# lvxianwei/DeepMerge

Hardware: AMD Instinct MI355X
Metric: superpixel-pairs/sec (train step) (higher is better)
Workload: dtype bf16; 1 GPU; ShfitScaleFormer_v3 depth [3, 2, 1], scales [32, 64, 128, 256] x 4ch (256x256x4 patches), 32 pairs/GPU/step, fwd+loss+bwd+allreduce+Adam (BASELINE configs[1]); pairs_per_gpu=32, global_batch=32, parallelism=dp1

## Files before the change

deepmerge_amd/_lib.py:

```python
from __future__ import annotations

import ctypes as C
import os
import re
import threading

HERE = os.path.dirname(os.path.abspath(__file__))
ROOT = os.path.dirname(HERE)
LIB_PATH = os.path.join(HERE, "libdeepmerge_hip.so")
HEADER_PATH = os.path.join(ROOT, "include", "deepmerge_hip.h")

DM_F32, DM_BF16 = 0, 1
DM_NT, DM_NN, DM_TN = 0, 1, 2
DM_BF16_PAIR = 2
DM_F64 = 3
DM_EPI_NONE, DM_EPI_GELU, DM_EPI_DGELU, DM_EPI_GELU_GRAD, DM_EPI_MUL = 0, 1, 2, 3, 4

_STATUS = {-1: "bad shape", -2: "bad dtype", -3: "bad alignment", -4: "workspace", -5: "HIP error", -6: "unsupported"}


class DeepMergeLibraryError(RuntimeError):
    pass


class DmGemmArgs(C.Structure):
    _fields_ = [
        ("layout", C.c_int32), ("ab_dtype", C.c_int32), ("c_dtype", C.c_int32), ("aux_dtype", C.c_int32),
        ("M", C.c_int32), ("N", C.c_int32), ("K", C.c_int32),
        ("epilogue", C.c_int32), ("accumulate", C.c_int32), ("split_k", C.c_int32),
        ("A", C.c_void_p), ("lda", C.c_int64),
        ("B", C.c_void_p), ("ldb", C.c_int64),
        ("C", C.c_void_p), ("ldc", C.c_int64),
        ("bias", C.c_void_p),
        ("residual", C.c_void_p), ("ldr", C.c_int64),
        ("aux", C.c_void_p), ("ldaux", C.c_int64),
        ("rows_per_group", C.c_int32), ("group_stride", C.c_int64),
        ("workspace", C.c_void_p), ("workspace_bytes", C.c_int64),
        ("colsum_a", C.c_void_p), ("colsum_accumulate", C.c_int32),
        ("k_fold", C.c_int32), ("a_fold", C.c_int64 * 3), ("b_fold", C.c_int64 * 3),
        ("c_plane", C.c_int64),
    ]


class DmReduceItem(C.Structure):
    _fields_ = [("partial", C.c_void_p), ("out0", C.c_void_p), ("out1", C.c_void_p),
                ("nrows", C.c_int32), ("width", C.c_int32), ("split", C.c_int32), ("accumulate", C.c_int32)]


class DmPairDraw(C.Structure):
    _fields_ = [("pairs", C.c_void_p), ("pair_flag", C.c_void_p), ("poly_off", C.c_void_p), ("poly_pts", C.c_void_p),
                ("pt_tile", C.c_void_p), ("pt_xy", C.c_void_p), ("pt_inner", C.c_void_p), ("pt_obj", C.c_void_p),
                ("pt_region", C.c_void_p),
                ("tile_id", C.c_void_p), ("xy", C.c_void_p), ("inner", C.c_void_p), ("obj", C.c_void_p),
                ("region", C.c_void_p), ("flag", C.c_void_p),
                ("point_id", C.c_void_p),
                ("seed", C.c_uint64),
                ("n_pairs", C.c_int32), ("n_poly", C.c_int32), ("n_poly_pts", C.c_int32), ("n_pts", C.c_int32),
                ("epoch", C.c_int32), ("batch", C.c_int32)]


class DmMergeFold(C.Structure):
    _fields_ = [("ptr", C.c_void_p), ("idx", C.c_void_p), ("edges", C.c_void_p), ("root", C.c_void_p), ("pick", C.c_void_p),
                ("rep", C.c_void_p), ("region_of", C.c_void_p),
                ("simi", C.c_void_p), ("weights", C.c_void_p),
                ("count", C.c_void_p), ("sum", C.c_void_p), ("sumsq", C.c_void_p), ("bbox", C.c_void_p), ("peri", C.c_void_p),
                ("new_id", C.c_void_p), ("hist_rank", C.c_void_p), ("new_ptr", C.c_void_p), ("new_idx", C.c_void_p),
                ("new_rep", C.c_void_p), ("new_region_of", C.c_void_p), ("n_regions", C.c_void_p),
                ("new_count", C.c_void_p), ("new_sum", C.c_void_p), ("new_sumsq", C.c_void_p), ("new_bbox", C.c_void_p),
                ("new_peri", C.c_void_p),
                ("history", C.c_void_p), ("history_simi", C.c_void_p),
                ("C", C.c_int32), ("P", C.c_int32), ("E", C.c_int32), ("S0", C.c_int32), ("bands", C.c_int32), ("round", C.c_int32),
                ("hist_base", C.c_int32), ("hist_cap", C.c_int32)]


class DmVectorTrace(C.Structure):
    _fields_ = [("dart", C.c_void_p), ("next", C.c_void_p), ("lab", C.c_void_p), ("other", C.c_void_p), ("flags", C.c_void_p),
                ("key", C.c_void_p), ("sum", C.c_void_p), ("ring_of_slot", C.c_void_p), ("ring_ptr", C.c_void_p),
                ("arc_base", C.c_void_p), ("xy", C.c_void_p), ("area2", C.c_void_p),
                ("arc_first", C.c_void_p), ("arc_left", C.c_void_p), ("arc_right", C.c_void_p), ("arc_vstart", C.c_void_p),
                ("arc_count", C.c_void_p), ("arc_pos", C.c_void_p), ("arc_ptr", C.c_void_p), ("arc_xy", C.c_void_p),
                ("W", C.c_int32), ("D", C.c_int32), ("R", C.c_int32), ("n_arcs", C.c_int32)]


class DmSceneVectorTrace(C.Structure):
    _fields_ = [("dart", C.c_void_p), ("next", C.c_void_p), ("lab", C.c_void_p), ("other", C.c_void_p), ("flags", C.c_void_p),
                ("key", C.c_void_p), ("sum", C.c_void_p), ("ring_of_slot", C.c_void_p), ("ring_ptr", C.c_void_p),
                ("arc_base", C.c_void_p), ("xy", C.c_void_p), ("area2", C.c_void_p),
                ("arc_first", C.c_void_p), ("arc_left", C.c_void_p), ("arc_right", C.c_void_p), ("arc_vstart", C.c_void_p),
                ("arc_count", C.c_void_p), ("arc_pos", C.c_void_p), ("arc_ptr", C.c_void_p), ("arc_xy", C.c_void_p),
                ("W", C.c_int64), ("D", C.c_int32), ("R", C.c_int32), ("n_arcs", C.c_int32)]


class DmSceneSimplifyRings(C.Structure):
    _fields_ = [("xy", C.c_void_p), ("ring_ptr", C.c_void_p), ("vert_ring", C.c_void_p), ("node_row", C.c_void_p), ("node_col", C.c_void_p),
                ("kept_row", C.c_void_p), ("status", C.c_void_p),
                ("n_nodes", C.c_int64), ("n_kept", C.c_int64), ("scene_h", C.c_int64), ("scene_w", C.c_int64),
                ("V", C.c_int32), ("R", C.c_int32)]


class DmSimplifyTopology(C.Structure):
    _fields_ = [("arc_xy", C.c_void_p), ("arc_ptr", C.c_void_p), ("new_ptr", C.c_void_p), ("keep", C.c_void_p),
                ("point_count", C.c_void_p), ("point_fill", C.c_void_p), ("point_ptr", C.c_void_p), ("point_xy", C.c_void_p),
                ("seg", C.c_void_p), ("kind", C.c_void_p), ("cell_count", C.c_void_p), ("cell_fill", C.c_void_p),
                ("cell_ptr", C.c_void_p), ("cell_seg", C.c_void_p), ("stack", C.c_void_p), ("status", C.c_void_p),
                ("Va", C.c_int64), ("cap", C.c_int64), ("A", C.c_int32), ("H", C.c_int32), ("W", C.c_int32), ("q", C.c_int32)]


class DmSceneSimplifyTopology(C.Structure):
    _fields_ = [("arc_xy", C.c_void_p), ("arc_ptr", C.c_void_p), ("new_ptr", C.c_void_p), ("arc_keep", C.c_void_p),
                ("point_count", C.c_void_p), ("point_fill", C.c_void_p), ("point_ptr", C.c_void_p), ("point_xy", C.c_void_p),
                ("seg", C.c_void_p), ("kind", C.c_void_p), ("cell_count", C.c_void_p), ("cell_fill", C.c_void_p),
                ("cell_ptr", C.c_void_p), ("cell_seg", C.c_void_p), ("stack", C.c_void_p), ("status", C.c_void_p),
                ("Va", C.c_int64), ("cap", C.c_int64), ("A", C.c_int32), ("H", C.c_int32), ("W", C.c_int32), ("q", C.c_int32),
                ("cell_log2", C.c_int32)]


class DmProfRow(C.Structure):
    _fields_ = [("name", C.c_char * 64), ("launches", C.c_int64), ("total_ms", C.c_double),
                ("total_flops", C.c_double), ("total_bytes", C.c_double)]


_P, _I, _L, _F, _D = C.c_void_p, C.c_int32, C.c_int64, C.c_float, C.c_double

SIGNATURES = {
    "dm_abi_version": (_I, []),
    "dm_last_error": (C.c_char_p, []),
    "dm_arch": (C.c_char_p, []),
    "dm_gemm": (_I, [C.POINTER(DmGemmArgs), _P]),
    "dm_gemm_workspace_bytes": (_L, [_I, _I, _I, _I]),
    "dm_gemm_grouped": (_I, [C.POINTER(DmGemmArgs), _I, _P]),
    "dm_attention_fwd": (_I, [_P, _P, _P, _P, _I, _I, _I, _I, _F, _I, _P]),
    "dm_attention_relpos_inkernel": (_I, [_I, _I, _I, _I, _I, _I, _I, _I]),
    "dm_attention_fwd_relpos": (_I, [_P, _P, _I, _I, _I, _P, _P, _I, _I, _I, _I, _F, _I, _P]),
    "dm_attention_split_ok": (_I, [_I, _I, _I, _I, _I, _I, _I, _I]),
    "dm_attention_split_fwd": (_I, [_P, _P, _P, _P, _I, _I, _I, _P, _P, _I, _I, _I, _I, _F, _P]),
    "dm_attention_split_fwd_pair": (_I, [_P, _P, _P, _P, _I, _I, _I, _P, _P, _P, _I, _I, _I, _I, _F, _P]),
    "dm_attention_split_bwd_chunks": (_I, [_I, _I, _I]),
    "dm_attention_split_bwd": (_I, [_P, _P, _P, _I, _I, _I, _P, _P, _P, _P, _P, _P, _P, _P, _I, _I, _I, _I, _F, _P]),
    "dm_attention_split_bwd_pair": (_I, [_P, _P, _P, _I, _I, _I, _P, _P, _P, _P, _P, _P, _P, _P, _I, _I, _I, _I, _F, _P]),
    "dm_attention_bwd_relpos": (_I, [_P, _P, _I, _I, _I, _P, _P, _P, _P, _P, _P, _P, _P, _I, _I, _I, _I, _F, _I, _P]),
    "dm_attention_bwd": (_I, [_P, _P, _P, _P, _P, _P, _P, _P, _P, _I, _I, _I, _I, _F, _I, _P]),
    "dm_attention_bwd_batch_chunks": (_I, [_I, _I, _I, _I]),
    "dm_relpos_bias_gather": (_I, [_P, _P, _P, _P, _I, _I, _I, _P]),
    "dm_relpos_bias_reduce": (_I, [_P, _P, _P, _P, _I, _I, _I, _I, _I, _P]),
    "dm_layernorm_fwd": (_I, [_P, _P, _P, _P, _I, _P, _P, _I, _I, _F, _P]),
    "dm_layernorm_bwd": (_I, [_P, _I, _P, _P, _P, _P, _P, _P, _P, _P, _P, _I, _P, _I, _I, _P]),
    "dm_layernorm_bwd_partials": (_I, [_P, _I, _P, _P, _P, _P, _P, _P, _P, _P, _I, _I, C.POINTER(C.c_int32), _P]),
    "dm_layernorm_bwd_partials_pair": (_I, [_P, _I, _P, _P, _P, _P, _P, _P, _P, _P, _I, _I, C.POINTER(C.c_int32), _P]),
    "dm_layernorm_bwd_partials_regroup": (_I, [_P, _I, _P, _P, _P, _P, _P, _P, _P, _P, _I, _I, _I, _I, C.POINTER(C.c_int32), _P]),
    "dm_pool_layernorm_ok": (_I, [_I]),
    "dm_pool_layernorm_fwd": (_I, [_P, _P, _P, _P, _P, _P, _P, _I, _I, _I, _I, _F, _P]),
    "dm_pool_layernorm_bwd": (_I, [_P, _P, _P, _P, _P, _P, _P, _P, _P, _I, _P, C.POINTER(C.c_int32), _I, _I, _I, _I, _P]),
    "dm_partial_reduce_batch": (_I, [C.POINTER(DmReduceItem), _I, _P]),
    "dm_layernorm_bwd_partial_floats": (_L, [_I]),
    "dm_token_pool_fwd": (_I, [_P, _P, _I, _I, _I, _I, _P]),
    "dm_token_pool_bwd": (_I, [_P, _P, _I, _I, _I, _I, _P]),
    "dm_group_mean_fwd": (_I, [_P, _P, _I, _I, _I, _P]),
    "dm_group_mean_bwd": (_I, [_P, _P, _I, _I, _I, _P]),
    "dm_colsum": (_I, [_P, _I, _L, _P, _I, _I, _I, _P, _P]),
    "dm_colsum_partial_floats": (_L, [_I]),
    "dm_cast": (_I, [_P, _P, _I, _L, _P]),
    "dm_split_bf16": (_I, [_P, _L, _L, _L, _P, _I, _I, _P]),
    "dm_split_colsum_partial_floats": (_L, [_L, _L]),
    "dm_split_bf16_colsum": (_I, [_P, _L, _L, _L, _P, _I, _I, _P, _P, _P]),
    "dm_split_bf16_planes": (_I, [_P, _L, _L, _L, _P, _P, _P, _P]),
    "dm_patchify": (_I, [_P, _P, _I, _I, _I, _I, _I, _P]),
    "dm_contrastive_loss": (_I, [_P, _P, _P, _F, _F, _P, _P, _P, _I, _I, _P]),
    "dm_cross_entropy": (_I, [_P, _P, _P, _F, _P, _P, _I, _I, _P]),
    "dm_batchnorm_workspace_bytes": (_L, [_I, _I]),
    "dm_batchnorm_fwd": (_I, [_P, _P, _P, _P, _P, _P, _I, _P, _P, _P, _I, _I, _F, _F, _I, _I, _P, _P]),
    "dm_batchnorm_bwd": (_I, [_P, _P, _P, _P, _P, _I, _P, _P, _P, _P, _P, _I, _I, _I, _I, _I, _P, _P]),
    "dm_adam_step": (_I, [_P, _P, _P, _P, _P, _L, _I, _D, _D, _D, _D, _D, _P]),
    "dm_adam_hyper": (_I, [_I, _D, _D, _D, _P]),
    "dm_adam_step_dev": (_I, [_P, _P, _P, _P, _P, _L, _P, _D, _D, _D, _D, _P]),
    "dm_adam_step_dev_pair": (_I, [_P, _P, _P, _P, _P, _P, _L, _P, _D, _D, _D, _D, _P]),
    "dm_segment_mean": (_I, [_P, _P, _P, _P, _I, _I, _P]),
    "dm_edge_similarity": (_I, [_P, _P, _P, _P, _I, _I, _F, _P]),
    "dm_pairwise_distance": (_I, [_P, _P, _P, _I, _I, _I, _I, _P]),
    "dm_patch_pyramid": (_I, [_P, _I, _I, _I, _P, _P, _I, _I, _I, _I, _P, _P]),
    "dm_patch_pyramid_cols": (_I, [_P, _I, _I, _I, _P, _P, _I, _I, _I, _I, _I, _P, _I, _P]),
    "dm_pair_batch_gather": (_I, [_P, _I, _I, _I, _I, _P, _P, _P, _P, _I, _I, _I, _I, _I, _I, _P, _I, _P, _P, _P, _P]),
    "dm_pair_batch_gather_oriented": (_I, [_P, _I, _I, _I, _I, _P, _P, _P, _P, _P, _I, _I, _I, _I, _I, _I, _P, _I, _P, _P, _P, _P]),
    "dm_pair_batch_gather_augmented": (_I, [_P, _I, _I, _I, _I, _P, _P, _P, _P, _P, _P, _I, _I, _I, _I, _I, _I, _P, _I, _P, _P, _P, _P]),
    "dm_pair_epoch_draw": (_I, [C.POINTER(DmPairDraw), _P]),
    "dm_pair_epoch_orient": (_I, [C.c_uint64, _I, _I, _I, _I, _P, _P]),
    "dm_pair_epoch_radiometric": (_I, [C.c_uint64, _I, _I, _I, _I, _I, _I, _I, _P, _P]),
    "dm_contrastive_terms": (_I, [_P, _P, _P, _F, _P, _P, _I, _I, _P]),
    "dm_pair_eval_workspace_bytes": (_L, [_L, _I]),
    "dm_pair_eval_summary": (_I, [_P, _P, _P, _L, _P, _I, _P, _P, _P, _P, _P]),
    "dm_label_stats": (_I, [_P, _P, _I, _I, _I, _I, _P, _P, _P, _P, _P, _P]),
    "dm_label_features": (_I, [_P, _P, _P, _P, _P, _I, _I, _P, _P]),
    "dm_rag_edges": (_I, [_P, _I, _I, _I, _P, _P, _I, _P, _P, _I, _P, _P, _P]),
    "dm_seam_stitch": (_I, [_P, _P, _L, _L, _P, _P, _P, _I, _P, _P, _I, _P, _P, _P]),
    "dm_merge_round": (_I, [_P, _P, _I, _I, _P, _P, _I, _P]),
    "dm_merge_best": (_I, [_P, _P, _I, _I, _F, _P, _P]),
    "dm_merge_best_small": (_I, [_P, _P, _I, _I, _P, _L, _P, _P]),
    "dm_merge_accept": (_I, [_P, _P, _I, _I, _P, _L, _P, _P]),
    "dm_merge_match": (_I, [_P, _P, _I, _I, _P, _P, _P, _P, _P]),
    "dm_merge_fold_regions": (_I, [C.POINTER(DmMergeFold), _P]),
    "dm_merge_edge_keys": (_I, [_P, _P, _P, _I, _I, _P, _P]),
    "dm_merge_fold_edges": (_I, [_P, _P, _P, _I, _P, _P, _P, _P]),
    "dm_relabel_raster": (_I, [_P, _P, _P, _L, _I, _P]),
    "dm_region_merge_cost": (_I, [_P, _P, _P, _P, _P, _P, _P, _I, _I, _I, _D, _D, _D, _D, _D, _P, _P]),
    "dm_pixel_regions": (_I, [_P, _I, _I, _I, _P, _P, _P, _P, _P, _P, _P, _P]),
    "dm_label_clearance": (_I, [_P, _I, _I, _I, _P, _P, _P, _P]),
    "dm_point_select_round": (_I, [_P, _P, _I, _I, _I, _I, _I, _P, _P, _P, _P, _P, _P]),
    "dm_point_emit": (_I, [_P, _P, _P, _P, _I, _I, _I, _I, _P, _P, _P, _P, _P, _P, _P]),
    "dm_scene_point_init": (_I, [_P, _P, _P, _I, _P]),
    "dm_scene_point_select": (_I, [_P, _P, _I, _I, _I, _I, _I, _I, _L, _L, _L, _L, _I, _I, _I, _P, _P, _P, _P, _P]),
    "dm_scene_point_commit": (_I, [_P, _L, _L, _I, _I, _P, _P, _P, _P]),
    "dm_label_overlap": (_I, [_P, _P, _I, _I, _L, _L, _P, _P, _I, _P, _P, _I, _P, _P, _P]),
    "dm_overlap_reduce": (_I, [_P, _P, _I, _L, _L, _P, _P, _P, _P, _P, _P, _P, _P, _P]),
    "dm_pair_flags": (_I, [_P, _I, _P, _P, _P, _I, _I, _P, _P]),
    "dm_boundary_bits": (_I, [_P, _I, _I, _I, _P, _P, _P, _P]),
    "dm_boundary_counts": (_I, [_P, _P, _P, _I, _I, _I, _I, _I, _I, _I, _P, _P]),
    "dm_slic_iterate": (_I, [_P, _I, _I, _I, _I, _I, _I, _P, _P, _P, _P]),
    "dm_connected_labels": (_I, [_P, _I, _I, _I, _I, _P, _P, _P, _P, _P]),
    "dm_label_area": (_I, [_P, _I, _I, _I, _P, _P]),
    "dm_slic_absorb_pick": (_I, [_P, _P, _I, _P, _I, _I, _P, _P, _P, _P]),
    "dm_scene_slic_init": (_I, [_P, _I, _I, _I, _I, _I, _I, _I, _I, _P, _P, _P]),
    "dm_scene_slic_pass": (_I, [_P, _I, _I, _I, _I, _I, _I, _I, _I, _I, _P, _P, _P, _P]),
    "dm_scene_slic_update": (_I, [_I, _P, _P, _P]),
    "dm_vector_count": (_I, [_P, _I, _I, _P, _P, _P, _P]),
    "dm_vector_emit": (_I, [_P, _P, _I, _I, _P, _P, _P]),
    "dm_vector_link": (_I, [_P, _P, _P, _P, _I, _I, _I, _P, _P, _P, _P, _P, _P]),
    "dm_vector_head_round": (_I, [_P, _P, _P, _P, _I, _P, _P]),
    "dm_vector_rank_init": (_I, [_P, _P, _P, _P, _I, _P, _P, _P, _P, _P, _I, _P]),
    "dm_vector_rank_round": (_I, [_P, _P, _P, _P, _I, _P, _P]),
    "dm_vector_ring_emit": (_I, [C.POINTER(DmVectorTrace), _P]),
    "dm_vector_arc_emit": (_I, [C.POINTER(DmVectorTrace), _P]),
    "dm_scene_vector_count": (_I, [_P, _I, _I, _I, _I, _I, _I, _P, _P, _P, _P, _P]),
    "dm_scene_vector_link": (_I, [_P, _P, _P, _I, _I, _I, _L, _L, _L, _L, _P, _P, _P, _P, _P, _P]),
    "dm_scene_vector_ring_emit": (_I, [C.POINTER(DmSceneVectorTrace), _P]),
    "dm_scene_vector_arc_emit": (_I, [C.POINTER(DmSceneVectorTrace), _P]),
    "dm_rasterize_count": (_I, [_P, _P, _P, _I, _I, _I, _I, _P, _P]),
    "dm_rasterize_emit": (_I, [_P, _P, _P, _P, _P, _I, _I, _L, _I, _I, _L, _P, _P]),
    "dm_rasterize_fill": (_I, [_P, _L, _I, _I, _I, _P, _P, _P]),
    "dm_rasterize_count_rows": (_I, [_P, _P, _P, _I, _I, _I, _I, _I, _I, _P, _P]),
    "dm_rasterize_emit_rows": (_I, [_P, _P, _P, _P, _P, _I, _I, _L, _I, _I, _I, _I, _L, _P, _P]),
    "dm_rasterize_fill_window": (_I, [_P, _L, _I, _I, _I, _I, _I, _I, _I, _P, _P, _P]),
    "dm_simplify_nodes": (_I, [_P, _I, _I, _P, _P]),
    "dm_simplify_chains": (_I, [_P, _P, _I, _L, _I, _I, _I, _P, _P, _P]),
    "dm_simplify_arc_count": (_I, [_P, _P, _I, _L, _I, _I, _P, _P, _P]),
    "dm_simplify_arc_emit": (_I, [_P, _P, _P, _I, _L, _L, _I, _I, _P, _P, _P]),
    "dm_simplify_ring_count": (_I, [_P, _P, _P, _I, _I, _I, _I, _P, _P, _P]),
    "dm_simplify_ring_emit": (_I, [_P, _P, _P, _P, _P, _I, _I, _L, _I, _I, _P, _P, _P, _P]),
    "dm_simplify_topology_point_count": (_I, [C.POINTER(DmSimplifyTopology), _P]),
    "dm_simplify_topology_point_fill": (_I, [C.POINTER(DmSimplifyTopology), _P]),
    "dm_simplify_topology_segments": (_I, [C.POINTER(DmSimplifyTopology), _P]),
    "dm_simplify_topology_bin_count": (_I, [C.POINTER(DmSimplifyTopology), _P]),
    "dm_simplify_topology_bin_fill": (_I, [C.POINTER(DmSimplifyTopology), _P]),
    "dm_simplify_topology_pairs": (_I, [C.POINTER(DmSimplifyTopology), _P]),
    "dm_simplify_topology_jumps": (_I, [C.POINTER(DmSimplifyTopology), _P]),
    "dm_simplify_topology_refine": (_I, [C.POINTER(DmSimplifyTopology), _I, _P]),
    "dm_scene_simplify_node_count": (_I, [_P, _I, _I, _I, _I, _I, _I, _L, _L, _L, _L, _P, _P, _P]),
    "dm_scene_simplify_node_emit": (_I, [_P, _I, _I, _I, _I, _I, _I, _L, _L, _L, _L, _P, _I, _P, _P]),
    "dm_scene_simplify_chains": (_I, [_P, _P, _I, _L, _L, _L, _I, _P, _P, _P]),
    "dm_scene_simplify_arc_count": (_I, [_P, _P, _I, _L, _L, _L, _P, _P, _P]),
    "dm_scene_simplify_arc_emit": (_I, [_P, _P, _P, _I, _L, _L, _L, _L, _P, _P, _P]),
    "dm_scene_simplify_ring_count": (_I, [C.POINTER(DmSceneSimplifyRings), _P, _P]),
    "dm_scene_simplify_ring_emit": (_I, [C.POINTER(DmSceneSimplifyRings), _P, _P, _L, _P, _P, _P]),
    "dm_scene_simplify_topology_point_count": (_I, [C.POINTER(DmSceneSimplifyTopology), _P]),
    "dm_scene_simplify_topology_point_fill": (_I, [C.POINTER(DmSceneSimplifyTopology), _P]),
    "dm_scene_simplify_topology_segments": (_I, [C.POINTER(DmSceneSimplifyTopology), _P]),
    "dm_scene_simplify_topology_bin_count": (_I, [C.POINTER(DmSceneSimplifyTopology), _P]),
    "dm_scene_simplify_topology_bin_fill": (_I, [C.POINTER(DmSceneSimplifyTopology), _P]),
    "dm_scene_simplify_topology_pairs": (_I, [C.POINTER(DmSceneSimplifyTopology), _P]),
    "dm_scene_simplify_topology_jumps": (_I, [C.POINTER(DmSceneSimplifyTopology), _P]),
    "dm_scene_simplify_topology_refine": (_I, [C.POINTER(DmSceneSimplifyTopology), _I, _P]),
    "dm_gru_cell_fwd": (_I, [_P, _L, _P, _P, _P, _P, _I, _I, _P]),
    "dm_gru_cell_bwd": (_I, [_P, _P, _P, _P, _P, _P, _I, _I, _P]),
    "dm_prof_enable": (_I, [_I]),
    "dm_prof_collect": (_I, [C.POINTER(DmProfRow), _I]),
}

_lock = threading.Lock()
_lib = None


def declared_symbols(header_path: str = HEADER_PATH):
    text = open(header_path).read()
    text = re.sub(r"/\*.*?\*/", "", text, flags=re.S)
    return sorted(set(re.findall(r"\b(dm_[a-z0-9_]+)\s*\(", text)))


def lib() -> C.CDLL:
    global _lib
    if _lib is not None:
        return _lib
    with _lock:
        if _lib is not None:
            return _lib
        if not os.path.exists(LIB_PATH):
            raise DeepMergeLibraryError(
                f"{LIB_PATH} not found: build the HIP kernels first "
                f"(`python -c 'import __graft_entry__ as g; g.build()'` or `make -C deepmerge_amd/csrc`). "
                f"deepmerge_amd has no CPU fallback.")
        try:
            handle = C.CDLL(LIB_PATH)
        except OSError as e:
            raise DeepMergeLibraryError(f"cannot load {LIB_PATH}: {e}") from e
        for name, (res, args) in SIGNATURES.items():
            try:
                fn = getattr(handle, name)
            except AttributeError as e:
                raise DeepMergeLibraryError(f"{LIB_PATH} does not export {name}") from e
            fn.restype = res
            fn.argtypes = args
        if handle.dm_abi_version() != 7:
            raise DeepMergeLibraryError(f"ABI version mismatch: library {handle.dm_abi_version()} != 7")
        _lib = handle
        return _lib


def check(rc: int, what: str):
    if rc == 0:
        return
    msg = lib().dm_last_error().decode("utf-8", "replace")
    text = f"{what} failed ({_STATUS.get(rc, rc)}): {msg}"
    if rc in (-1, -2, -3, -6):
        raise ValueError(text)
    raise RuntimeError(text)
```

deepmerge_amd/csrc/dm_attention.hip:

```cpp
#include "dm_common.h"
#include "dm_mfma.h"
#include "dm_attention_pipe.h"
#include "dm_attention_x3.h"
#include "dm_prof.h"

namespace {

constexpr int HD = 64;
constexpr int QB = 64;

template <typename T> struct AL {
  static constexpr int RB = HD * (int)sizeof(T);
  static constexpr int CPRW = RB / 16;
  static constexpr int KBD = RB / 64;
  static constexpr int EPC = 16 / (int)sizeof(T);
  static constexpr int TPB = (sizeof(T) == 2) ? 2 : 1;
};

template <typename T> __device__ __forceinline__ int swz(int row);
template <> __device__ __forceinline__ int swz<bf16_t>(int row) {
  const int t0 = (row >> 1) & 1, t1 = (row >> 2) & 1, t2 = (row >> 3) & 1;
  return ((t1 ^ t2) << 2) | (t0 << 1) | t1;
}
template <> __device__ __forceinline__ int swz<float>(int row) { return row & 15; }

template <typename T> __device__ __forceinline__ int img_off(int row, int chunk) {
  return row * AL<T>::RB + ((chunk ^ swz<T>(row)) << 4);
}

template <typename T>
__device__ __forceinline__ void tile_to_lds(char *lds, const T *g, long long ld, int nvalid, int nrows, int t) {
  using L = AL<T>;
  const int c = t % L::CPRW;
  constexpr int RPI = 256 / L::CPRW;
  for (int row = t / L::CPRW; row < nrows; row += RPI) {
    u32x4 v = {0u, 0u, 0u, 0u};
    if (row < nvalid) v = *reinterpret_cast<const u32x4 *>(g + (long long)row * ld + c * L::EPC);
    *reinterpret_cast<u32x4 *>(lds + img_off<T>(row, c)) = v;
  }
}

template <typename T> __device__ __forceinline__ u32x4 frag_row(const char *lds, int row, int kb, int lane) {
  return *reinterpret_cast<const u32x4 *>(lds + img_off<T>(row, kb * 4 + (lane >> 4)));
}
template <typename T> __device__ __forceinline__ u32x4 frag_tr(const char *lds, int d0, int m, int lane);
template <> __device__ __forceinline__ u32x4 frag_tr<bf16_t>(const char *lds, int d0, int m, int lane) {
  const int g = lane >> 4, q = (lane >> 2) & 3, p = lane & 3;
  const int d = d0 + 4 * p;
  u32x4 out;
#pragma unroll
  for (int half = 0; half < 2; ++half) {
    const int k = 32 * m + 4 * g + 16 * half + q;
    const u32x2 w = dm_ds_read_tr16(lds + img_off<bf16_t>(k, d >> 3) + ((d & 7) << 1));
    out[2 * half] = w[0];
    out[2 * half + 1] = w[1];
  }
  return out;
}
template <> __device__ __forceinline__ u32x4 frag_tr<float>(const char *lds, int d0, int m, int lane) {
  const int g = lane >> 4, d = d0 + (lane & 15);
  u32x4 out;
#pragma unroll
  for (int j = 0; j < 4; ++j) {
    const int k = 16 * m + 4 * g + j;
    out[j] = *reinterpret_cast<const unsigned int *>(lds + img_off<float>(k, d >> 2) + ((d & 3) << 2));
  }
  return out;
}
template <typename T> __device__ __forceinline__ u32x4 gl_frag(const T *rowp, bool valid, int kb, int lane) {
  u32x4 v = {0u, 0u, 0u, 0u};
  if (valid) v = *reinterpret_cast<const u32x4 *>(rowp + (kb * 4 + (lane >> 4)) * AL<T>::EPC);
  return v;
}

template <typename T, int NKT> __device__ __forceinline__ u32x4 acc_frag(const f32x4 (&s)[NKT], int m) {
  if constexpr (sizeof(T) == 2) {
    const f32x4 lo = s[2 * m], hi = s[2 * m + 1];
    bf16x8 r = {(bf16_t)lo[0], (bf16_t)lo[1], (bf16_t)lo[2], (bf16_t)lo[3], (bf16_t)hi[0], (bf16_t)hi[1], (bf16_t)hi[2], (bf16_t)hi[3]};
    return __builtin_bit_cast(u32x4, r);
  } else {
    return __builtin_bit_cast(u32x4, s[m]);
  }
}

template <typename T, int NKT>
__device__ __forceinline__ void contract_tokens(f32x4 (&o)[4], const f32x4 (&s)[NKT], const char *img, int lane) {
#pragma unroll
  for (int m = 0; m < NKT / AL<T>::TPB; ++m) {
    const u32x4 fp = acc_frag<T, NKT>(s, m);
#pragma unroll
    for (int dt = 0; dt < 4; ++dt) mma<T>(o[dt], fp, frag_tr<T>(img, dt * 16, m, lane));
    if ((m & 1) == 1) __builtin_amdgcn_sched_barrier(0);
  }
}

__device__ __forceinline__ float row_max(float v) {
  v = fmaxf(v, __shfl_xor(v, 16, 64));
  return fmaxf(v, __shfl_xor(v, 32, 64));
}
__device__ __forceinline__ float row_sum(float v) {
  v += __shfl_xor(v, 16, 64);
  return v + __shfl_xor(v, 32, 64);
}

template <typename T> __device__ __forceinline__ float fast_exp(float x);
template <> __device__ __forceinline__ float fast_exp<float>(float x) { return expf(x); }
template <> __device__ __forceinline__ float fast_exp<bf16_t>(float x) { return __expf(x); }

__device__ __forceinline__ f32x4 load4_guard(const float *p, int i, int n, bool vec) {
  if (vec) return (i < n) ? dm_load4(p + i) : (f32x4){0.f, 0.f, 0.f, 0.f};
  f32x4 r;
#pragma unroll
  for (int e = 0; e < 4; ++e) r[e] = (i + e < n) ? p[i + e] : 0.f;
  return r;
}

struct AttnParams {
  const void *qkv;
  const float *bias;
  const float *bias_t;
  const void *out;
  const void *dout;
  float *lse;
  float *delta;
  void *dqkv;
  float *slab;
  int B, N, H, bchunk;
  float scale;
};

template <bool FAST, bool STRIDED>
__device__ __forceinline__ f32x4 bias_tile(const float *bias_rows, int N, int row, int lane, int kt) {
  const int col = kt * 16 + 4 * (lane >> 4);
  f32x4 bv = {0.f, 0.f, 0.f, 0.f};
  if (bias_rows && row < N) {
    if constexpr (!STRIDED) {
      bv = load4_guard(bias_rows + (long long)row * N, col, N, FAST);
    } else {
#pragma unroll
      for (int r = 0; r < 4; ++r) bv[r] = (col + r < N) ? bias_rows[(long long)(col + r) * N + row] : 0.f;
    }
  }
  return bv;
}
template <typename T>
__device__ __forceinline__ f32x4 score_tile(const u32x4 (&fa)[AL<T>::KBD], const char *img, const f32x4 bv,
                                            int N, int row, float scale, int lane, int kt) {
  using L = AL<T>;
  const int g = lane >> 4, li = lane & 15;
  f32x4 a = {0.f, 0.f, 0.f, 0.f};
#pragma unroll
  for (int kb = 0; kb < L::KBD; ++kb) mma<T>(a, fa[kb], frag_row<T>(img, kt * 16 + li, kb, lane));
  const int col = kt * 16 + 4 * g;
#pragma unroll
  for (int r = 0; r < 4; ++r) a[r] = (row < N && col + r < N) ? a[r] * scale + bv[r] : -INFINITY;
  return a;
}

template <typename T> __device__ __forceinline__ u32x4 pack_tiles(const f32x4 (&tl)[AL<T>::TPB]) {
  if constexpr (sizeof(T) == 2) {
    bf16x8 r = {(bf16_t)tl[0][0], (bf16_t)tl[0][1], (bf16_t)tl[0][2], (bf16_t)tl[0][3],
                (bf16_t)tl[1][0], (bf16_t)tl[1][1], (bf16_t)tl[1][2], (bf16_t)tl[1][3]};
    return __builtin_bit_cast(u32x4, r);
  } else {
    return __builtin_bit_cast(u32x4, tl[0]);
  }
}

template <typename T, int NB>
__device__ __forceinline__ void contract_frags(f32x4 (&o)[4], const u32x4 (&f)[NB], const char *img, int lane) {
#pragma unroll
  for (int m = 0; m < NB; ++m) {
#pragma unroll
    for (int dt = 0; dt < 4; ++dt) mma<T>(o[dt], f[m], frag_tr<T>(img, dt * 16, m, lane));
    if ((m & 1) == 1) __builtin_amdgcn_sched_barrier(0);
  }
}

template <typename T, int NKT, bool FAST>
__global__ __launch_bounds__(256, 2) void attn_fwd_kernel(const AttnParams p) {
  using L = AL<T>;
  constexpr int NK = NKT * 16;
  constexpr int IMG = NK * L::RB;
  __shared__ __attribute__((aligned(16))) char smem[2 * IMG];
  char *kimg = smem, *vimg = smem + IMG;
  const int t = threadIdx.x, lane = t & 63, wave = t >> 6, g = lane >> 4, li = lane & 15;
  const int qblk = blockIdx.x, h = blockIdx.y, b = blockIdx.z;
  const int N = p.N, H = p.H;

  const long long tok_stride = 3LL * H * HD;
  const T *base = reinterpret_cast<const T *>(p.qkv) + (long long)b * N * tok_stride + (long long)h * HD;
  const int q = qblk * QB + wave * 16 + li;

  tile_to_lds<T>(kimg, base + (long long)H * HD, tok_stride, N, NK, t);
  tile_to_lds<T>(vimg, base + 2LL * H * HD, tok_stride, N, NK, t);
  u32x4 fq[L::KBD];
#pragma unroll
  for (int kb = 0; kb < L::KBD; ++kb) fq[kb] = gl_frag<T>(base + (long long)q * tok_stride, q < N, kb, lane);
  __syncthreads();

  f32x4 s[NKT];
  const float *brows = p.bias ? p.bias + (long long)h * N * N : nullptr;
#pragma unroll
  for (int kt = 0; kt < NKT; ++kt) s[kt] = score_tile<T>(fq, kimg, bias_tile<FAST, false>(brows, N, q, lane, kt), N, q, p.scale, lane, kt);

  float m = -INFINITY;
#pragma unroll
  for (int kt = 0; kt < NKT; ++kt)
#pragma unroll
    for (int r = 0; r < 4; ++r) m = fmaxf(m, s[kt][r]);
  m = row_max(m);
  const float msafe = (m == -INFINITY) ? 0.f : m;
  float l = 0.f;
#pragma unroll
  for (int kt = 0; kt < NKT; ++kt)
#pragma unroll
    for (int r = 0; r < 4; ++r) {
      const float e = fast_exp<T>(s[kt][r] - msafe);
      s[kt][r] = e;
      l += e;
    }
  l = row_sum(l);
  const float inv = (l > 0.f) ? 1.f / l : 0.f;
  if (g == 0 && q < N) p.lse[((long long)b * H + h) * N + q] = msafe + logf(l);
#pragma unroll
  for (int kt = 0; kt < NKT; ++kt) s[kt] *= inv;

  f32x4 o[4];
#pragma unroll
  for (int dt = 0; dt < 4; ++dt) o[dt] = (f32x4){0.f, 0.f, 0.f, 0.f};
  contract_tokens<T, NKT>(o, s, vimg, lane);
  if (q < N) {
    T *orow = reinterpret_cast<T *>(const_cast<void *>(p.out)) + ((long long)b * N + q) * H * HD + (long long)h * HD;
#pragma unroll
    for (int dt = 0; dt < 4; ++dt) dm_store4(orow + dt * 16 + 4 * g, o[dt]);
  }
}

template <typename T, int NKT, bool FAST>
__global__ __launch_bounds__(256, 2) void attn_bwd_dq_kernel(const AttnParams p) {
  using L = AL<T>;
  constexpr int NK = NKT * 16;
  constexpr int IMG = NK * L::RB;
  constexpr int NB = NKT / L::TPB;
  __shared__ __attribute__((aligned(16))) char smem[2 * IMG];
  char *kimg = smem, *vimg = smem + IMG;
  const int t = threadIdx.x, lane = t & 63, wave = t >> 6, g = lane >> 4, li = lane & 15;
  const int qblk = blockIdx.x, h = blockIdx.y, chunk = blockIdx.z;
  const int N = p.N, H = p.H;
  const long long tok_stride = 3LL * H * HD;
  const int q = qblk * QB + wave * 16 + li;
  const bool qok = q < N;
  const float *brows = p.bias ? p.bias + (long long)h * N * N : nullptr;
  const bool want_bins = p.slab != nullptr;
  f32x4 hacc[NKT];
#pragma unroll
  for (int kt = 0; kt < NKT; ++kt) hacc[kt] = (f32x4){0.f, 0.f, 0.f, 0.f};

  const int b_end = min(p.B, (chunk + 1) * p.bchunk);
  for (int b = chunk * p.bchunk; b < b_end; ++b) {
    const T *base = reinterpret_cast<const T *>(p.qkv) + (long long)b * N * tok_stride + (long long)h * HD;
    const long long orow = ((long long)b * N + q) * H * HD + (long long)h * HD;
    const T *Og = reinterpret_cast<const T *>(p.out) + orow;
    const T *dOg = reinterpret_cast<const T *>(p.dout) + orow;
    __syncthreads();
    tile_to_lds<T>(kimg, base + (long long)H * HD, tok_stride, N, NK, t);
    tile_to_lds<T>(vimg, base + 2LL * H * HD, tok_stride, N, NK, t);
    u32x4 fq[L::KBD], fdo[L::KBD];
#pragma unroll
    for (int kb = 0; kb < L::KBD; ++kb) {
      fq[kb] = gl_frag<T>(base + (long long)q * tok_stride, qok, kb, lane);
      fdo[kb] = gl_frag<T>(dOg, qok, kb, lane);
    }
    float dl = 0.f;
    if (qok) {
#pragma unroll
      for (int c = 0; c < 4; ++c) {
        const f32x4 a = dm_load4(Og + 16 * g + 4 * c), d = dm_load4(dOg + 16 * g + 4 * c);
        dl += (a[0] * d[0] + a[1] * d[1]) + (a[2] * d[2] + a[3] * d[3]);
      }
    }
    dl = row_sum(dl);
    const long long rowid = ((long long)b * H + h) * N + q;
    if (g == 0 && qok) p.delta[rowid] = dl;
    const float lse = qok ? p.lse[rowid] : 0.f;
    __syncthreads();

    u32x4 fds[NB];
    f32x4 bnext[L::TPB];
#pragma unroll
    for (int u = 0; u < L::TPB; ++u) bnext[u] = bias_tile<FAST, false>(brows, N, q, lane, u);
#pragma unroll
    for (int m = 0; m < NB; ++m) {
      f32x4 bcur[L::TPB];
#pragma unroll
      for (int u = 0; u < L::TPB; ++u) bcur[u] = bnext[u];
      if (m + 1 < NB) {
#pragma unroll
        for (int u = 0; u < L::TPB; ++u) bnext[u] = bias_tile<FAST, false>(brows, N, q, lane, (m + 1) * L::TPB + u);
      }
      f32x4 tl[L::TPB];
#pragma unroll
      for (int u = 0; u < L::TPB; ++u) {
        const int kt = m * L::TPB + u;
        const f32x4 sc = score_tile<T>(fq, kimg, bcur[u], N, q, p.scale, lane, kt);
        f32x4 a = {0.f, 0.f, 0.f, 0.f};
#pragma unroll
        for (int kb = 0; kb < L::KBD; ++kb) mma<T>(a, fdo[kb], frag_row<T>(vimg, kt * 16 + li, kb, lane));
        f32x4 dsv;
#pragma unroll
        for (int r = 0; r < 4; ++r) dsv[r] = fast_exp<T>(sc[r] - lse) * (a[r] - dl);
        if (want_bins) hacc[kt] += dsv;
        tl[u] = dsv;
      }
      fds[m] = pack_tiles<T>(tl);
      asm volatile("" : "+v"(fds[m]));
      __builtin_amdgcn_sched_barrier(0);
    }

    f32x4 o[4];
#pragma unroll
    for (int dt = 0; dt < 4; ++dt) o[dt] = (f32x4){0.f, 0.f, 0.f, 0.f};
    contract_frags<T, NB>(o, fds, kimg, lane);
    if (qok) {
      T *dq = reinterpret_cast<T *>(p.dqkv) + ((long long)b * N + q) * tok_stride + (long long)h * HD;
#pragma unroll
      for (int dt = 0; dt < 4; ++dt) dm_store4(dq + dt * 16 + 4 * g, o[dt] * p.scale);
    }
  }

  if (want_bins && qok) {
    float *srow = p.slab + (((long long)chunk * H + h) * N + q) * N;
#pragma unroll
    for (int kt = 0; kt < NKT; ++kt) {
      const int key = kt * 16 + 4 * g;
      if constexpr (FAST) {
        if (key < N) dm_store4(srow + key, hacc[kt]);
      } else {
#pragma unroll
        for (int r = 0; r < 4; ++r)
          if (key + r < N) srow[key + r] = hacc[kt][r];
      }
    }
  }
}

template <typename T, int NKT, bool FAST>
__global__ __launch_bounds__(256, 2) void attn_bwd_dkv_kernel(const AttnParams p) {
  using L = AL<T>;
  constexpr int NK = NKT * 16;
  constexpr int IMG = NK * L::RB;
  __shared__ __attribute__((aligned(16))) char smem[2 * IMG];
  char *qimg = smem, *doimg = smem + IMG;
  const int t = threadIdx.x, lane = t & 63, wave = t >> 6, g = lane >> 4, li = lane & 15;
  const int kblk = blockIdx.x, h = blockIdx.y, b = blockIdx.z;
  const int N = p.N, H = p.H;

  const long long tok_stride = 3LL * H * HD;
  const T *base = reinterpret_cast<const T *>(p.qkv) + (long long)b * N * tok_stride + (long long)h * HD;
  const long long o_stride = (long long)H * HD;
  const T *dOg = reinterpret_cast<const T *>(p.dout) + (long long)b * N * o_stride + (long long)h * HD;
  const int key = kblk * QB + wave * 16 + li;
  const bool kok = key < N;
  const T *krow = base + (long long)key * tok_stride + (long long)H * HD;
  const T *vrow = krow + (long long)H * HD;
  const float *lse = p.lse + ((long long)b * H + h) * N;
  const float *delta = p.delta + ((long long)b * H + h) * N;

  tile_to_lds<T>(qimg, base, tok_stride, N, NK, t);
  tile_to_lds<T>(doimg, dOg, o_stride, N, NK, t);
  u32x4 fk[L::KBD], fvv[L::KBD];
#pragma unroll
  for (int kb = 0; kb < L::KBD; ++kb) {
    fk[kb] = gl_frag<T>(krow, kok, kb, lane);
    fvv[kb] = gl_frag<T>(vrow, kok, kb, lane);
  }
  __syncthreads();

  constexpr int NB = NKT / L::TPB;
  u32x4 fpt[NB], fds[NB];
  const float *bsrc = FAST ? p.bias_t : p.bias;
  const float *brows = bsrc ? bsrc + (long long)h * N * N : nullptr;
  f32x4 bnext[L::TPB], lnext[L::TPB], dnext[L::TPB];
  auto fetch = [&](int m) {
#pragma unroll
    for (int u = 0; u < L::TPB; ++u) {
      const int qt = m * L::TPB + u;
      bnext[u] = bias_tile<FAST, !FAST>(brows, N, key, lane, qt);
      lnext[u] = load4_guard(lse, qt * 16 + 4 * g, N, FAST);
      dnext[u] = load4_guard(delta, qt * 16 + 4 * g, N, FAST);
    }
  };
  fetch(0);
#pragma unroll
  for (int m = 0; m < NB; ++m) {
    f32x4 bcur[L::TPB], lcur[L::TPB], dcur[L::TPB];
#pragma unroll
    for (int u = 0; u < L::TPB; ++u) { bcur[u] = bnext[u]; lcur[u] = lnext[u]; dcur[u] = dnext[u]; }
    if (m + 1 < NB) fetch(m + 1);
    f32x4 tp[L::TPB], td[L::TPB];
#pragma unroll
    for (int u = 0; u < L::TPB; ++u) {
      const int qt = m * L::TPB + u;
      const int q0 = qt * 16 + 4 * g;
      const f32x4 sc = score_tile<T>(fk, qimg, bcur[u], N, key, p.scale, lane, qt);
      f32x4 a = {0.f, 0.f, 0.f, 0.f};
#pragma unroll
      for (int kb = 0; kb < L::KBD; ++kb) mma<T>(a, fvv[kb], frag_row<T>(doimg, qt * 16 + li, kb, lane));
#pragma unroll
      for (int r = 0; r < 4; ++r) {
        const float pv = (q0 + r < N) ? fast_exp<T>(sc[r] - lcur[u][r]) : 0.f;
        tp[u][r] = pv;
        td[u][r] = pv * (a[r] - dcur[u][r]);
      }
    }
    fpt[m] = pack_tiles<T>(tp);
    fds[m] = pack_tiles<T>(td);
    asm volatile("" : "+v"(fpt[m]), "+v"(fds[m]));
    __builtin_amdgcn_sched_barrier(0);
  }
  f32x4 o[4];
  T *dk = reinterpret_cast<T *>(p.dqkv) + ((long long)b * N + key) * tok_stride + (long long)H * HD + (long long)h * HD;
  T *dvp = dk + (long long)H * HD;
#pragma unroll
  for (int dt = 0; dt < 4; ++dt) o[dt] = (f32x4){0.f, 0.f, 0.f, 0.f};
  contract_frags<T, NB>(o, fpt, doimg, lane);
  if (kok) {
#pragma unroll
    for (int dt = 0; dt < 4; ++dt) dm_store4(dvp + dt * 16 + 4 * g, o[dt]);
  }
#pragma unroll
  for (int dt = 0; dt < 4; ++dt) o[dt] = (f32x4){0.f, 0.f, 0.f, 0.f};
  contract_frags<T, NB>(o, fds, qimg, lane);
  if (kok) {
#pragma unroll
    for (int dt = 0; dt < 4; ++dt) dm_store4(dk + dt * 16 + 4 * g, o[dt] * p.scale);
  }
}

template <typename T, int NKT, bool FAST> void launch3(int which, const AttnParams &p, dim3 grid, hipStream_t s) {
  if (which == 0) hipLaunchKernelGGL((attn_fwd_kernel<T, NKT, FAST>), grid, dim3(256), 0, s, p);
  else if (which == 1) hipLaunchKernelGGL((attn_bwd_dq_kernel<T, NKT, FAST>), grid, dim3(256), 0, s, p);
  else hipLaunchKernelGGL((attn_bwd_dkv_kernel<T, NKT, FAST>), grid, dim3(256), 0, s, p);
}
template <typename T, bool FAST> void dispatch_nkt(int which, const AttnParams &p, hipStream_t s) {
  const dim3 grid((p.N + QB - 1) / QB, p.H, which == 1 ? (p.B + p.bchunk - 1) / p.bchunk : p.B);
  const int nkt = (p.N + 15) / 16;
  if (nkt <= 2) launch3<T, 2, FAST>(which, p, grid, s);
  else if (nkt <= 4) launch3<T, 4, FAST>(which, p, grid, s);
  else if (nkt <= 8) launch3<T, 8, FAST>(which, p, grid, s);
  else if (nkt <= 12) launch3<T, 12, FAST>(which, p, grid, s);
  else if (nkt <= 14) launch3<T, 14, FAST>(which, p, grid, s);
  else launch3<T, 16, FAST>(which, p, grid, s);
}
template <typename T> int dispatch(int which, const AttnParams &p, hipStream_t s) {
  const bool fast = (p.N % 4 == 0) && (which != 2 || p.bias == nullptr || p.bias_t != nullptr);
  if (fast) dispatch_nkt<T, true>(which, p, s);
  else dispatch_nkt<T, false>(which, p, s);
  return 0;
}

int check_common(const char *who, int B, int N, int H, int D, int dtype) {
  DM_REQUIRE(B > 0 && H > 0 && N > 0 && N <= 256, DM_ERR_BAD_SHAPE, "%s: need 0 < N <= 4096 tokens and head dim <= 256 (got N=%d, D=%d, B=%d, H=%d)", who, N, D, B, H);
  DM_REQUIRE(D == HD, DM_ERR_BAD_SHAPE, "%s: head dim must be in 1..256 (got %d)", who, D);
  DM_REQUIRE(dtype == DM_F32 || dtype == DM_BF16, DM_ERR_BAD_DTYPE, "%s: bad dtype %d", who, dtype);
  DM_REQUIRE(H <= 65535 && B <= 65535, DM_ERR_BAD_SHAPE, "%s: grid too large", who);
  return DM_OK;
}

}

static int batch_chunk(int B, int N, int H) {
  const int per_sample = ((N + QB - 1) / QB) * H;
  for (int c = 8; c > 1; c >>= 1)
    if ((long long)per_sample * ((B + c - 1) / c) >= 300) return c;
  return 1;
}

const AttnSwitches &attn_switches() {
// ... 340 lines not shown
```

deepmerge_amd/ops.py:

```python
from __future__ import annotations

import os

import ctypes as C
from dataclasses import dataclass
from typing import Optional, Tuple

import torch

from . import _lib
from ._lib import DM_BF16, DM_EPI_DGELU, DM_EPI_GELU, DM_EPI_GELU_GRAD, DM_EPI_MUL, DM_EPI_NONE, DM_F32, DM_NN, DM_NT, DM_TN, DmGemmArgs, check

_NUMERICS = "bf16"


NUMERICS_MODES = ("bf16", "fp32", "bf16x3")
_FP32_PRODUCTS = "mfma_f32"
_SPLIT_MIN_WORK = 1 << 24
_PAIR_LN_MAX_COLS = 1024


def set_numerics(mode: str) -> None:
    global _NUMERICS
    _NUMERICS = check_numerics(mode)
# ... 158 lines not shown

def _fold_planes(layout: int, A: Planes, B: Planes, M: int, N: int, K: int):
    (a_rows, a_cols), (b_rows, b_cols) = _operand_shapes(layout, M, N, K)
    if (A.rows, A.cols) != (a_rows, a_cols) or (B.rows, B.cols) != (b_rows, b_cols):
        raise ValueError(f"plane pair shapes {(A.rows, A.cols)} / {(B.rows, B.cols)} do not match the product {(a_rows, a_cols)} / {(b_rows, b_cols)}")
    return A.t, B.t, a_cols, b_cols, 3 * K, (K, A.t.stride(0), B.t.stride(0))


def gemm(layout: int, A: torch.Tensor, B: torch.Tensor, C_out: torch.Tensor, M: int, N: int, K: int, *,
         lda: Optional[int] = None, ldb: Optional[int] = None, ldc: Optional[int] = None,
         bias: Optional[torch.Tensor] = None, residual: Optional[torch.Tensor] = None, ldr: Optional[int] = None,
         epilogue: int = DM_EPI_NONE, aux: Optional[torch.Tensor] = None, ldaux: Optional[int] = None,
         accumulate: bool = False, split_k: int = 0, rows_per_group: int = 0, group_stride: int = 0,
         colsum_out: Optional[torch.Tensor] = None, colsum_accumulate: bool = False, ws_slot: str = "gemm") -> torch.Tensor:
    c_pair = C_out if isinstance(C_out, Planes) else None
    if c_pair is not None:
        if (c_pair.rows, c_pair.cols) != (M, N) or ldc not in (None, N):
            raise ValueError("a plane-pair result is a dense [2, M, N] tensor")
        C_out = c_pair.t
    fold = None
    if isinstance(A, Planes) or isinstance(B, Planes) or (
            _FP32_PRODUCTS == "bf16x3" and A.dtype == torch.float32 and M * N * K >= _SPLIT_MIN_WORK and planes_ok(M, K) and planes_ok(N, K)
            and (lda is None or lda % 4 == 0) and (ldb is None or ldb % 4 == 0) and A.data_ptr() % 16 == 0 and B.data_ptr() % 16 == 0):
        (a_rows, a_cols), (b_rows, b_cols) = _operand_shapes(layout, M, N, K)
        if not isinstance(A, Planes):
            A = split_planes(torch.as_strided(A, (a_rows, a_cols), (lda if lda is not None else a_cols, 1)), colsum_out, colsum_accumulate)
            colsum_out = None
        if not isinstance(B, Planes):
            B = split_planes(torch.as_strided(B, (b_rows, b_cols), (ldb if ldb is not None else b_cols, 1)))
        A, B, lda, ldb, K, fold = _fold_planes(layout, A, B, M, N, K)
    _need_cuda(A, B, C_out, bias, residual, aux, colsum_out)
    if A.dtype != B.dtype:
        raise ValueError(f"A/B dtype mismatch: {A.dtype} vs {B.dtype}")
    if lda is None:
        lda = A.stride(-2) if A.dim() >= 2 else K
    if ldb is None:
        ldb = B.stride(-2) if B.dim() >= 2 else K
    if (_FP32_PRODUCTS == "bf16x3" and A.dtype == torch.float32 and M * N * K >= _SPLIT_MIN_WORK
            and M % 8 == 0 and N % 8 == 0 and K % 8 == 0 and lda % 4 == 0 and ldb % 4 == 0):
        (a_rows, a_cols), (b_rows, b_cols) = _operand_shapes(layout, M, N, K)
        a_stack, b_stack = int(layout == DM_TN), int(layout != DM_NT)
        A3 = workspace(6 * a_rows * a_cols, A.device, ws_slot + ".split_a").view(torch.bfloat16)
        B3 = workspace(6 * b_rows * b_cols, A.device, ws_slot + ".split_b").view(torch.bfloat16)
        fused_ok = colsum_out is not None and a_cols % 8 == 0 and A.data_ptr() % 16 == 0 and (a_rows * a_cols) % 8 == 0
        n_part = _lib.lib().dm_split_colsum_partial_floats(a_rows, a_cols) if fused_ok else 0
        if n_part > 0:
            part = workspace(4 * n_part, A.device, ws_slot + ".partial").view(torch.float32)
            rows_out = C.c_int32(0)
            check(_lib.lib().dm_split_bf16_colsum(A.data_ptr(), lda, a_rows, a_cols, A3.data_ptr(), a_stack, 0b100, part.data_ptr(),
                                                  C.byref(rows_out), _stream()), "dm_split_bf16_colsum")
            _reduce(part, colsum_out, colsum_out, rows_out.value, a_cols, a_cols, colsum_accumulate)
        else:
            check(_lib.lib().dm_split_bf16(A.data_ptr(), lda, a_rows, a_cols, A3.data_ptr(), a_stack, 0b100, _stream()), "dm_split_bf16")
            if colsum_out is not None:
                colsum(torch.as_strided(A, (a_rows, a_cols), (lda, 1)), colsum_out, accumulate=colsum_accumulate, ws_slot=ws_slot + ".partial")
        check(_lib.lib().dm_split_bf16(B.data_ptr(), ldb, b_rows, b_cols, B3.data_ptr(), b_stack, 0b010, _stream()), "dm_split_bf16")
        return gemm(layout, A3, B3, C_out, M, N, 3 * K, lda=(a_cols if a_stack else 3 * a_cols), ldb=(b_cols if b_stack else 3 * b_cols),
                    ldc=ldc, bias=bias, residual=residual, ldr=ldr, epilogue=epilogue, aux=aux, ldaux=ldaux, accumulate=accumulate,
                    split_k=split_k, rows_per_group=rows_per_group, group_stride=group_stride, ws_slot=ws_slot)
    a = _gemm_args(layout, A, B, C_out, M, N, K, lda, ldb, ldc, bias, residual, ldr, epilogue, aux, ldaux, accumulate, split_k,
                   rows_per_group, group_stride, colsum_out, colsum_accumulate, ws_slot, c_pair, fold)
    check(_lib.lib().dm_gemm(C.byref(a), _stream()), "dm_gemm")
    return c_pair if c_pair is not None else C_out


def _gemm_args(layout, A, B, C_out, M, N, K, lda, ldb, ldc, bias, residual, ldr, epilogue, aux, ldaux, accumulate, split_k,
               rows_per_group, group_stride, colsum_out, colsum_accumulate, ws_slot, c_pair=None, fold=None, min_slabs: int = 0) -> DmGemmArgs:
    a = DmGemmArgs()
    a.layout, a.ab_dtype, a.c_dtype = layout, _dt(A), _dt(C_out)
    if c_pair is not None:
        if _dt(A) != DM_BF16:
            raise ValueError("a plane-pair result goes with bf16 / folded operands")
        a.c_dtype, a.c_plane = _lib.DM_BF16_PAIR, M * N
    a.aux_dtype = _dt(aux) if aux is not None else DM_F32
    a.M, a.N, a.K = M, N, K
    a.epilogue, a.accumulate, a.split_k = epilogue, int(accumulate), split_k
    a.A, a.lda = A.data_ptr(), lda
    a.B, a.ldb = B.data_ptr(), ldb
    a.C, a.ldc = C_out.data_ptr(), (ldc if ldc is not None else N)
    a.bias = _ptr(bias)
    if bias is not None and (bias.dtype != torch.float32 or bias.numel() < N):
        raise ValueError("bias must be fp32 with >= N elements")
    a.residual, a.ldr = _ptr(residual), (ldr if ldr is not None else N)
    if residual is not None and residual.dtype != torch.float32:
        raise ValueError("residual must be fp32")
    a.aux, a.ldaux = _ptr(aux), (ldaux if ldaux is not None else N)
    a.rows_per_group, a.group_stride = rows_per_group, group_stride
    if colsum_out is not None:
        if colsum_out.dtype != torch.float32 or colsum_out.numel() < M or not colsum_out.is_contiguous():
            raise ValueError("colsum_out must be a contiguous fp32 tensor with >= M elements")
        a.colsum_a, a.colsum_accumulate = colsum_out.data_ptr(), int(colsum_accumulate)
    if fold is not None:
        a.k_fold = fold[0]
        a.a_fold[0], a.a_fold[1], a.a_fold[2] = 0, 0, fold[1]
        a.b_fold[0], a.b_fold[1], a.b_fold[2] = 0, fold[2], 0
    ws_bytes = _lib.lib().dm_gemm_workspace_bytes(layout, M, N, K) if (split_k != 1 or colsum_out is not None) else 0
    if split_k > 1:
        ws_bytes = max(ws_bytes, _lib.lib().dm_gemm_workspace_bytes(layout, M, N, K) + split_k * M * N * 4)
    if min_slabs > 0:
        ws_bytes = max(ws_bytes, _lib.lib().dm_gemm_workspace_bytes(layout, M, N, K) + min_slabs * M * N * 4)
    if ws_bytes > 0:
        ws = workspace(ws_bytes, A.device, ws_slot)
        a.workspace, a.workspace_bytes = ws.data_ptr(), ws.numel()
    return a


def gemm_grouped(calls) -> None:
    if not calls:
        return
    plain = len(calls) > 1
    for args, kw in calls:
        A, B = args[1], args[2]
        pair = isinstance(A, Planes) and isinstance(B, Planes)
        plain = plain and not isinstance(args[3], Planes) and (pair or (not isinstance(A, Planes) and not isinstance(B, Planes) and A.dtype == torch.bfloat16))
    if not plain:
        for args, kw in calls:
            gemm(*args, **kw)
        return
    arr = (DmGemmArgs * len(calls))()
    for i, (args, kw) in enumerate(calls):
        layout, A, B, C_out, M, N, K = args
        lda, ldb, fold = kw.get("lda"), kw.get("ldb"), None
        if isinstance(A, Planes):
            A, B, lda, ldb, K, fold = _fold_planes(layout, A, B, M, N, K)
        _need_cuda(A, B, C_out, kw.get("colsum_out"))
        if A.dtype != B.dtype:
            raise ValueError(f"A/B dtype mismatch: {A.dtype} vs {B.dtype}")
        lda = lda if lda is not None else (A.stride(-2) if A.dim() >= 2 else K)
        ldb = ldb if ldb is not None else (B.stride(-2) if B.dim() >= 2 else K)
        arr[i] = _gemm_args(layout, A, B, C_out, M, N, K, lda, ldb, kw.get("ldc"), kw.get("bias"), kw.get("residual"), kw.get("ldr"),
                            kw.get("epilogue", DM_EPI_NONE), kw.get("aux"), kw.get("ldaux"), kw.get("accumulate", False), kw.get("split_k", 0),
                            kw.get("rows_per_group", 0), kw.get("group_stride", 0), kw.get("colsum_out"), kw.get("colsum_accumulate", False),
                            f"{kw.get('ws_slot', 'gemm')}.g{i}", None, fold, min_slabs=16 if layout == DM_TN else 0)
    check(_lib.lib().dm_gemm_grouped(arr, len(calls), _stream()), "dm_gemm_grouped")


def cast(src: torch.Tensor, dtype: torch.dtype) -> torch.Tensor:
    if src.dtype == dtype:
        return src
    _need_cuda(src)
    if src.dtype != torch.float32:
        raise ValueError("dm_cast source must be fp32")
    src = src.contiguous()
    dst = torch.empty(src.shape, dtype=dtype, device=src.device)
    check(_lib.lib().dm_cast(src.data_ptr(), dst.data_ptr(), _dt(dst), src.numel(), _stream()), "dm_cast")
    return dst


def colsum(X: torch.Tensor, out: torch.Tensor, accumulate: bool = False, ws_slot: str = "partial") -> torch.Tensor:
    _need_cuda(X, out)
    M, N = X.shape
    part = workspace(_lib.lib().dm_colsum_partial_floats(N) * 4, X.device, ws_slot)
    check(_lib.lib().dm_colsum(X.data_ptr(), _dt(X), X.stride(0), out.data_ptr(), M, N, int(accumulate), part.data_ptr(), _stream()), "dm_colsum")
    return out


def layernorm_fwd(x: torch.Tensor, gamma, beta, eps: float, out_dtype: torch.dtype, pair: bool = False):
    _need_cuda(x, gamma, beta)
    rows, cols = x.numel() // x.shape[-1], x.shape[-1]
    mean = torch.empty(rows, dtype=torch.float32, device=x.device)
    rstd = torch.empty(rows, dtype=torch.float32, device=x.device)
    if pair:
        yp = torch.empty((2, rows, cols), dtype=torch.bfloat16, device=x.device)
        check(_lib.lib().dm_layernorm_fwd(x.data_ptr(), gamma.data_ptr(), beta.data_ptr(), yp.data_ptr(), _lib.DM_BF16_PAIR, mean.data_ptr(),
                                          rstd.data_ptr(), rows, cols, eps, _stream()), "dm_layernorm_fwd")
        return Planes(yp), mean, rstd
    y = torch.empty(x.shape, dtype=out_dtype, device=x.device)
    check(_lib.lib().dm_layernorm_fwd(x.data_ptr(), gamma.data_ptr(), beta.data_ptr(), y.data_ptr(), _dt(y), mean.data_ptr(),
                                      rstd.data_ptr(), rows, cols, eps, _stream()), "dm_layernorm_fwd")
    return y, mean, rstd


_pending_reduce = []
_pending_out = set()
_flush_queued = False
_flush_task = -1


def _in_backward() -> bool:
    return torch._C._current_graph_task_id() != -1


def flush_reductions() -> None:
    global _flush_queued
    _flush_queued = False
    if not _pending_reduce:
        return
    items = (_lib.DmReduceItem * len(_pending_reduce))()
    for i, (f, _keep) in enumerate(_pending_reduce):
        items[i].partial, items[i].out0, items[i].out1, items[i].nrows, items[i].width, items[i].split, items[i].accumulate = f
    n = len(_pending_reduce)
    keep = list(_pending_reduce)
    _pending_reduce.clear()
    _pending_out.clear()
    check(_lib.lib().dm_partial_reduce_batch(items, n, _stream()), "dm_partial_reduce_batch")
    del keep


def _queue_reduce(part, out0, out1, nrows, width, split, accumulate) -> None:
    global _flush_queued, _flush_task
    task = torch._C._current_graph_task_id()
    if task != _flush_task:
        _pending_reduce.clear()
        _pending_out.clear()
        _flush_queued = False
        _flush_task = task
    keys = (out0.data_ptr(), out1.data_ptr())
    if keys[0] in _pending_out or keys[1] in _pending_out:
        flush_reductions()
    _pending_reduce.append(((part.data_ptr(), keys[0], keys[1], int(nrows), int(width), int(split), int(bool(accumulate))), (part, out0, out1)))
    _pending_out.update(keys)
    if not _flush_queued:
        torch.autograd.Variable._execution_engine.queue_callback(flush_reductions)
        _flush_queued = True


def _deferred(defer: bool) -> bool:
    return bool(defer and _DEFER_REDUCTIONS and _in_backward())


def _reduce(part, out0, out1, nrows, width, split, accumulate, deferred=False) -> None:
    if deferred:
        _queue_reduce(part, out0, out1, nrows, width, split, accumulate)
        return
    item = (_lib.DmReduceItem * 1)()
    item[0].partial, item[0].out0, item[0].out1 = part.data_ptr(), out0.data_ptr(), out1.data_ptr()
    item[0].nrows, item[0].width, item[0].split, item[0].accumulate = nrows, width, split, int(bool(accumulate))
    check(_lib.lib().dm_partial_reduce_batch(item, 1, _stream()), "dm_partial_reduce_batch")


def _partial_rows(cols: int, device, deferred: bool) -> torch.Tensor:
    n = _lib.lib().dm_layernorm_bwd_partial_floats(cols)
    return torch.empty(n, dtype=torch.float32, device=device) if deferred else workspace(n * 4, device, "partial").view(torch.float32)


def layernorm_bwd(dy, x, gamma, mean, rstd, dres=None, dgamma=None, dbeta=None, accumulate=False, want_lp=False, defer=False, want_pair=False,
                  regroup=None):
    _need_cuda(dy, x)
    if not (dy.is_contiguous() and x.is_contiguous()) or dy.numel() != x.numel():
        raise ValueError("layernorm_bwd: dy and x must be contiguous and of the same size (an expanded gradient has no rows to read)")
    rows, cols = x.numel() // x.shape[-1], x.shape[-1]
    dx = torch.empty(x.shape, dtype=torch.float32, device=x.device)
    if want_pair:
        lp_out = Planes(torch.empty((2, rows, cols), dtype=torch.bfloat16, device=x.device))
    elif regroup is not None:
        S, T = regroup
        if not want_lp or rows % (S * T) or cols > _PAIR_LN_MAX_COLS:
            raise ValueError("layernorm_bwd: regroup needs want_lp, rows in whole (S, T) groups and a register-resident width")
        lp_out = torch.empty((S, rows // (S * T), T, cols), dtype=torch.bfloat16, device=x.device)
    else:
        lp_out = torch.empty(x.shape, dtype=torch.bfloat16, device=x.device) if want_lp else None
    if dgamma is None:
        dgamma = torch.empty(cols, dtype=torch.float32, device=x.device)
        dbeta = torch.empty(cols, dtype=torch.float32, device=x.device)
        accumulate = False
        defer = False
    result = (dx, lp_out, dgamma, dbeta) if (want_lp or want_pair) else (dx, dgamma, dbeta)
    deferred = _deferred(defer)
    part = _partial_rows(cols, x.device, deferred)
    head = (dy.data_ptr(), _dt(dy), x.data_ptr(), gamma.data_ptr(), mean.data_ptr(), rstd.data_ptr(), _ptr(dres), dx.data_ptr())
    if not (want_pair or regroup is not None or deferred):
        check(_lib.lib().dm_layernorm_bwd(*head, _ptr(lp_out), dgamma.data_ptr(), dbeta.data_ptr(), int(accumulate), part.data_ptr(), rows, cols,
                                          _stream()), "dm_layernorm_bwd")
        return result
    n_part = C.c_int32(0)
    if want_pair:
        check(_lib.lib().dm_layernorm_bwd_partials_pair(*head, lp_out.t.data_ptr(), part.data_ptr(), rows, cols, C.byref(n_part), _stream()),
              "dm_layernorm_bwd_partials_pair")
    elif regroup is not None:
        check(_lib.lib().dm_layernorm_bwd_partials_regroup(*head, lp_out.data_ptr(), part.data_ptr(), rows, cols, S, T, C.byref(n_part), _stream()),
              "dm_layernorm_bwd_partials_regroup")
    else:
        check(_lib.lib().dm_layernorm_bwd_partials(*head, _ptr(lp_out), part.data_ptr(), rows, cols, C.byref(n_part), _stream()),
              "dm_layernorm_bwd_partials")
    _reduce(part, dgamma, dbeta, n_part.value, 2 * cols, cols, accumulate, deferred)
    return result


_DEFER_REDUCTIONS = os.environ.get("DM_DEFER_REDUCTIONS", "1") != "0"
_FUSED_GLUE = os.environ.get("DM_FUSED_GLUE", "1") != "0"


def relpos_bias_gather(table: torch.Tensor, index32: torch.Tensor, N: int, transposed: bool = False):
    _need_cuda(table, index32)
    n_bins, H = table.shape
    bias = torch.empty((H, N, N), dtype=torch.float32, device=table.device)
    bias_t = torch.empty_like(bias) if transposed else None
    check(_lib.lib().dm_relpos_bias_gather(table.data_ptr(), index32.data_ptr(), bias.data_ptr(), _ptr(bias_t), N, H, n_bins, _stream()),
          "dm_relpos_bias_gather")
    return (bias, bias_t) if transposed else bias


def attention_fwd(qkv: torch.Tensor, bias: Optional[torch.Tensor], B: int, N: int, H: int, D: int, scale: float):
    _need_cuda(qkv, bias)
    out = torch.empty((B, N, H * D), dtype=qkv.dtype, device=qkv.device)
    lse = torch.empty((B, H, N), dtype=torch.float32, device=qkv.device)
    check(_lib.lib().dm_attention_fwd(qkv.data_ptr(), _ptr(bias), out.data_ptr(), lse.data_ptr(), B, N, H, D, scale, _dt(qkv), _stream()),
          "dm_attention_fwd")
    return out, lse


_SPLIT_ATTENTION = os.environ.get("DM_ATTN_X3", "1") != "0"
_INKERNEL_TABLE = os.environ.get("DM_ATTN_TABLE_IN_KERNEL", "1") != "0"


class _AttnRoute:
    __slots__ = ("kind", "cube")

    def __init__(self, table, index32, dtype, B, N, H, D):
        cube = None if table is None else getattr(index32, "_dm_cube", None)
        self.kind, self.cube = "dense", None
        if (dtype == torch.float32 and _FP32_PRODUCTS == "bf16x3" and _SPLIT_ATTENTION and (table is None or cube is not None)
                and attention_split_ok(B, N, H, D, cube)):
            self.kind, self.cube = "split", cube
        elif cube is not None and _INKERNEL_TABLE and relpos_inkernel(B, N, H, D, cube, dtype):
            self.kind, self.cube = "table", cube


def _attention_forward(qkv, table, index32, route: _AttnRoute, B, N, H, D, scale, out_pair: bool = False):
    table = None if table is None else table.contiguous()
    if route.kind == "split":
        r = attention_fwd_split(qkv, table, route.cube, B, N, H, D, scale, out_pair=out_pair)
        return r[0], r[1], (r[2], r[3]), (r[4] if out_pair else None)
    if route.kind == "table":
        return attention_fwd_relpos(qkv, table, route.cube, B, N, H, D, scale) + ((None, None), None)
    keep = (None, None) if table is None else relpos_bias_gather(table, index32, N, transposed=True)
    return attention_fwd(qkv, keep[0], B, N, H, D, scale) + (keep, None)


def _attention_backward(route: _AttnRoute, qkv, keep, table, out, dout, lse, index32, n_bins, B, N, H, D, scale, pair: bool = False):
    table = None if (table is None or route.kind == "dense") else table.contiguous()
    if route.kind == "split":
        return attention_bwd_split(keep[0], keep[1], table, route.cube, out, dout, lse, B, N, H, D, scale, index32, n_bins or 0, pair=pair)
    return attention_bwd(qkv, keep[0], out, dout, lse, B, N, H, D, scale, index32, n_bins or 0, bias_t=keep[1], table=table, cube=route.cube)


def relpos_inkernel(B: int, N: int, H: int, D: int, cube, dtype: torch.dtype) -> bool:
    if cube is None or len(cube) != 3:
        return False
    return bool(_lib.lib().dm_attention_relpos_inkernel(B, N, H, D, int(cube[0]), int(cube[1]), int(cube[2]),
                                                        DM_BF16 if dtype == torch.bfloat16 else DM_F32))


def attention_fwd_relpos(qkv: torch.Tensor, table: torch.Tensor, cube, B: int, N: int, H: int, D: int, scale: float):
    _need_cuda(qkv, table)
    if table.dtype != torch.float32 or not table.is_contiguous() or tuple(table.shape) != ((2 * cube[0] - 1) * (2 * cube[1] - 1) * (2 * cube[2] - 1), H):
        raise ValueError(f"attention_fwd_relpos: table must be contiguous fp32 [(2s-1)(2h-1)(2w-1), H], got {tuple(table.shape)} {table.dtype}")
    out = torch.empty((B, N, H * D), dtype=qkv.dtype, device=qkv.device)
    lse = torch.empty((B, H, N), dtype=torch.float32, device=qkv.device)
    check(_lib.lib().dm_attention_fwd_relpos(qkv.data_ptr(), table.data_ptr(), int(cube[0]), int(cube[1]), int(cube[2]), out.data_ptr(),
                                             lse.data_ptr(), B, N, H, D, scale, _dt(qkv), _stream()), "dm_attention_fwd_relpos")
    return out, lse


def attention_split_ok(B: int, N: int, H: int, D: int, cube=None) -> bool:
    c = (0, 0, 0) if cube is None else tuple(int(v) for v in cube)
    return bool(_lib.lib().dm_attention_split_ok(B, N, H, D, int(cube is not None), c[0], c[1], c[2]))


def attention_fwd_split(qkv: torch.Tensor, table: Optional[torch.Tensor], cube, B: int, N: int, H: int, D: int, scale: float, out_pair: bool = False):
    if table is not None and (table.dtype != torch.float32 or not table.is_contiguous()):
        raise ValueError("attention_fwd_split: table must be contiguous fp32")
    if isinstance(qkv, Planes):
        _need_cuda(qkv.t, table)
        hi, lo, src, dev = qkv.t[0], qkv.t[1], None, qkv.t.device
    else:
        _need_cuda(qkv, table)
        if qkv.dtype != torch.float32 or not qkv.is_contiguous():
            raise ValueError("attention_fwd_split: qkv must be a contiguous fp32 tensor")
        hi = torch.empty(qkv.shape, dtype=torch.bfloat16, device=qkv.device)
        lo = torch.empty(qkv.shape, dtype=torch.bfloat16, device=qkv.device)
        src, dev = qkv.data_ptr(), qkv.device
    out = torch.empty((B, N, H * D), dtype=torch.float32, device=dev)
    lse = torch.empty((B, H, N), dtype=torch.float32, device=dev)
    c = (0, 0, 0) if cube is None else tuple(int(v) for v in cube)
    if out_pair:
        op = torch.empty((2, B * N, H * D), dtype=torch.bfloat16, device=dev)
        check(_lib.lib().dm_attention_split_fwd_pair(src, hi.data_ptr(), lo.data_ptr(), _ptr(table), c[0], c[1], c[2], out.data_ptr(), op.data_ptr(),
                                                     lse.data_ptr(), B, N, H, D, scale, _stream()), "dm_attention_split_fwd_pair")
        return out, lse, hi, lo, Planes(op)
    check(_lib.lib().dm_attention_split_fwd(src, hi.data_ptr(), lo.data_ptr(), _ptr(table), c[0], c[1], c[2], out.data_ptr(),
                                            lse.data_ptr(), B, N, H, D, scale, _stream()), "dm_attention_split_fwd")
    return out, lse, hi, lo


def attention_bwd_split(hi, lo, table, cube, out, dout, lse, B, N, H, D, scale, index32=None, n_bins=0, pair=False):
    _need_cuda(hi, lo, table, out, dout, lse, index32)
    if out.dtype != torch.float32 or dout.dtype != torch.float32 or not (out.is_contiguous() and dout.is_contiguous()):
        raise ValueError("attention_bwd_split: out / dout must be contiguous fp32")
    dqkv = (torch.empty((2, B * N, 3 * H * D), dtype=torch.bfloat16, device=hi.device) if pair
            else torch.empty(hi.shape, dtype=torch.float32, device=hi.device))
    delta = torch.empty((B, H, N), dtype=torch.float32, device=hi.device)
    dhi = torch.empty(dout.shape, dtype=torch.bfloat16, device=hi.device)
    dlo = torch.empty(dout.shape, dtype=torch.bfloat16, device=hi.device)
    slab, info = None, None
    if index32 is not None and table is not None:
        chunks = _lib.lib().dm_attention_split_bwd_chunks(B, N, H)
        slab = torch.empty((chunks, H, N, N), dtype=torch.float32, device=hi.device)
        info = (chunks, N, relpos_index_csr(index32, n_bins))
    c = (0, 0, 0) if cube is None else tuple(int(v) for v in cube)
    fn = _lib.lib().dm_attention_split_bwd_pair if pair else _lib.lib().dm_attention_split_bwd
    check(fn(hi.data_ptr(), lo.data_ptr(), _ptr(table), c[0], c[1], c[2], out.data_ptr(), dout.data_ptr(),
             dhi.data_ptr(), dlo.data_ptr(), lse.data_ptr(), dqkv.data_ptr(), delta.data_ptr(), _ptr(slab),
             B, N, H, D, scale, _stream()), "dm_attention_split_bwd")
    return (Planes(dqkv) if pair else dqkv), slab, info


def relpos_index_csr(index32: torch.Tensor, n_bins: int):
    key = (index32._version, n_bins)
    hit = getattr(index32, "_dm_csr", None)
    if hit is None or hit[0] != key:
        flat = index32.reshape(-1).to(torch.int64)
        ok = (flat >= 0) & (flat < n_bins)
        where = torch.nonzero(ok).reshape(-1)
        order = torch.argsort(flat[where], stable=True)
        positions = where[order].to(torch.int32).contiguous()
        counts = torch.bincount(flat[where], minlength=n_bins)
        offsets = torch.zeros(n_bins + 1, dtype=torch.int64, device=index32.device)
        offsets[1:] = torch.cumsum(counts, 0)
        hit = index32._dm_csr = (key, positions, offsets.to(torch.int32).contiguous())
    return hit[1], hit[2]


def attention_bwd(qkv, bias, out, dout, lse, B, N, H, D, scale, index32=None, n_bins=0, bias_t=None, table=None, cube=None):
    _need_cuda(qkv, bias, out, dout, lse, index32, bias_t, table)
    dqkv = torch.empty_like(qkv)
    delta = torch.empty((B, H, N), dtype=torch.float32, device=qkv.device)
    slab, info = None, None
    if index32 is not None:
        if D != 64 or N > 256:
            raise ValueError(f"the relative-position bias gradient needs head dim 64 and N <= 256 (got D={D}, N={N})")
        chunks = _lib.lib().dm_attention_bwd_batch_chunks(B, N, H, _dt(qkv))
        slab = torch.empty((chunks, H, N, N), dtype=torch.float32, device=qkv.device)
        info = (chunks, N, relpos_index_csr(index32, n_bins))
    if table is not None and cube is not None:
        check(_lib.lib().dm_attention_bwd_relpos(qkv.data_ptr(), table.data_ptr(), int(cube[0]), int(cube[1]), int(cube[2]), _ptr(bias),
                                                 _ptr(bias_t), out.data_ptr(), dout.data_ptr(), lse.data_ptr(), dqkv.data_ptr(),
                                                 delta.data_ptr(), _ptr(slab), B, N, H, D, scale, _dt(qkv), _stream()),
              "dm_attention_bwd_relpos")
        return dqkv, slab, info
    check(_lib.lib().dm_attention_bwd(qkv.data_ptr(), _ptr(bias), _ptr(bias_t), out.data_ptr(), dout.data_ptr(), lse.data_ptr(), dqkv.data_ptr(),
                                      delta.data_ptr(), _ptr(slab), B, N, H, D, scale, _dt(qkv), _stream()),
          "dm_attention_bwd")
    return dqkv, slab, info


def relpos_bias_scatter(slab, dtable, B, H, info, n_bins, accumulate=False):
    _need_cuda(slab, dtable)
    chunks, N, (positions, offsets) = info
    check(_lib.lib().dm_relpos_bias_reduce(slab.data_ptr(), positions.data_ptr(), offsets.data_ptr(), dtable.data_ptr(), chunks, H, N,
                                           n_bins, int(accumulate), _stream()), "dm_relpos_bias_reduce")
    return dtable


def patchify(x: torch.Tensor, patch: int, dtype: torch.dtype) -> torch.Tensor:
    _need_cuda(x)
    B, Cc, H, W = x.shape
    if H != W:
        raise ValueError("square images only")
    x = x.contiguous()
    g = H // patch
    cols = torch.empty((B * g * g, Cc * patch * patch), dtype=dtype, device=x.device)
    check(_lib.lib().dm_patchify(x.data_ptr(), cols.data_ptr(), _dt(cols), B, Cc, H, patch, _stream()), "dm_patchify")
    return cols


RESIZE_RULES = {"opencv": 0, "exact_area": 1}


def _resize_rule(resize: str) -> int:
    if resize not in RESIZE_RULES:
        raise ValueError(f"resize must be one of {tuple(RESIZE_RULES)}, got {resize!r}")
    return RESIZE_RULES[resize]


def patch_pyramid(tile: torch.Tensor, xy: torch.Tensor, windows: torch.Tensor, target: int, max_window: Optional[int] = None,
                  resize: str = "opencv") -> torch.Tensor:
    _need_cuda(tile, xy, windows)
    if tile.dtype != torch.uint8:
        raise ValueError("tile must be uint8")
    bands, H, W = tile.shape
    P = xy.shape[0]
    if max_window is None:
        max_window = int(windows.max().item())
    out = torch.empty((P, bands, target, target), dtype=torch.float32, device=tile.device)
    check(_lib.lib().dm_patch_pyramid(tile.contiguous().data_ptr(), bands, H, W, xy.to(torch.int32).contiguous().data_ptr(),
                                      windows.to(torch.int32).contiguous().data_ptr(), max_window, P, target, _resize_rule(resize),
                                      out.data_ptr(), _stream()), "dm_patch_pyramid")
    return out


class PatchCols:

    def __init__(self, cols: torch.Tensor, batch: int, side: int, patch: int, bands: int):
        self.cols, self.batch, self.side, self.patch, self.bands = cols, batch, side, patch, bands

    @property
    def shape(self):
        return (self.batch, self.bands, self.side, self.side)

    def __getitem__(self, sl):
        g2 = (self.side // self.patch) ** 2
        if not isinstance(sl, slice) or sl.step not in (None, 1):
            raise TypeError("PatchCols supports contiguous batch slices only")
        a, b, _ = sl.indices(self.batch)
        return PatchCols(self.cols[a * g2:b * g2], b - a, self.side, self.patch, self.bands)

    def to(self, *_a, **_k):
        return self

    @staticmethod
    def cat(a: "PatchCols", b: "PatchCols") -> "PatchCols":
        if (a.side, a.patch, a.bands, a.cols.dtype) != (b.side, b.patch, b.bands, b.cols.dtype):
            raise ValueError("PatchCols.cat: the two sides were built for different scales / dtypes")
        ca, cb = a.cols, b.cols
        if (ca.is_contiguous() and cb.is_contiguous() and ca.untyped_storage().data_ptr() == cb.untyped_storage().data_ptr()
                and cb.data_ptr() == ca.data_ptr() + ca.numel() * ca.element_size()):
            both = ca.as_strided((ca.shape[0] + cb.shape[0], ca.shape[1]), (ca.shape[1], 1), ca.storage_offset())
        else:
            both = torch.cat((ca, cb), 0)
        return PatchCols(both, a.batch + b.batch, a.side, a.patch, a.bands)


def cat_batch(a, b):
    if isinstance(a, PatchCols) or isinstance(b, PatchCols):
        return PatchCols.cat(a, b)
    return torch.cat((a, b), 0)


def pair_batch_gather(tiles: torch.Tensor, tile_id: Optional[torch.Tensor], xy: torch.Tensor, inner: torch.Tensor, obj: torch.Tensor,
                      scale_index: int, target: int, max_window: int, out: torch.Tensor, grid: int = 0, resize: str = "opencv",
                      region_features: Optional[torch.Tensor] = None, designed: Optional[torch.Tensor] = None,
                      error_flag: Optional[torch.Tensor] = None, orient: Optional[torch.Tensor] = None,
                      radio: Optional[torch.Tensor] = None) -> None:
    _need_cuda(tiles, tile_id, xy, inner, obj, out, region_features, designed, error_flag, orient, radio)
    if tiles.dtype != torch.uint8 or tiles.dim() != 4 or not tiles.is_contiguous():
        raise ValueError("tiles must be a contiguous uint8 [T, bands, H, W] tensor")
    for name, t in (("tile_id", tile_id), ("xy", xy), ("inner", inner), ("obj", obj), ("error_flag", error_flag)):
        if t is not None and (t.dtype != torch.int32 or not t.is_contiguous()):
            raise ValueError(f"{name} must be a contiguous int32 tensor (a per-step cast would be a launch of its own)")
    T, bands, H, W = tiles.shape
    P = xy.shape[0]
    if not out.is_contiguous() or out.numel() != P * bands * target * target:
        raise ValueError(f"out must be contiguous with {P * bands * target * target} elements, got {tuple(out.shape)}")
    if (region_features is None) != (designed is None):
        raise ValueError("designed rows need the region features (and vice versa)")
    if designed is not None and (designed.dtype != torch.float32 or designed.numel() != P * 19 or not designed.is_contiguous()
                                 or region_features.dtype != torch.float32 or region_features.numel() != P * 15 or not region_features.is_contiguous()):
        raise ValueError("region_features must be contiguous float32 [P, 15] and designed contiguous float32 [P, 1, 19]")
    if orient is not None and (orient.dtype != torch.int32 or not orient.is_contiguous() or tuple(orient.shape) != (P,)):
        raise ValueError(f"orient must be a contiguous int32 [{P}] tensor, got {orient.dtype} {tuple(orient.shape)}")
    if radio is not None:
        if radio.dtype != torch.int32 or not radio.is_contiguous() or tuple(radio.shape) != (P, bands, 2):
            raise ValueError(f"radio must be a contiguous int32 [{P}, {bands}, 2] tensor, got {radio.dtype} {tuple(radio.shape)}")
        check(_lib.lib().dm_pair_batch_gather_augmented(tiles.data_ptr(), T, bands, H, W, _ptr(tile_id), xy.data_ptr(), inner.data_ptr(),
                                                        obj.data_ptr(), _ptr(orient), radio.data_ptr(), scale_index, max_window, P, target,
                                                        grid, _resize_rule(resize), out.data_ptr(), _dt(out), _ptr(region_features),
                                                        _ptr(designed), _ptr(error_flag), _stream()), "dm_pair_batch_gather_augmented")
        return
    if orient is not None:
        check(_lib.lib().dm_pair_batch_gather_oriented(tiles.data_ptr(), T, bands, H, W, _ptr(tile_id), xy.data_ptr(), inner.data_ptr(),
                                                       obj.data_ptr(), orient.data_ptr(), scale_index, max_window, P, target, grid,
                                                       _resize_rule(resize), out.data_ptr(), _dt(out), _ptr(region_features), _ptr(designed),
                                                       _ptr(error_flag), _stream()), "dm_pair_batch_gather_oriented")
        return
    check(_lib.lib().dm_pair_batch_gather(tiles.data_ptr(), T, bands, H, W, _ptr(tile_id), xy.data_ptr(), inner.data_ptr(), obj.data_ptr(),
                                          scale_index, max_window, P, target, grid, _resize_rule(resize), out.data_ptr(), _dt(out),
                                          _ptr(region_features), _ptr(designed), _ptr(error_flag), _stream()), "dm_pair_batch_gather")


ORIENT_MASKS = {"flips": 3, "d4": 7}


def pair_epoch_orient(seed: int, epoch: int, n_pairs: int, batch: int, mask: int, out: torch.Tensor) -> None:
    _need_cuda(out)
    if out.dtype != torch.int32 or not out.is_contiguous() or out.numel() != 2 * int(n_pairs):
        raise ValueError(f"pair_epoch_orient: out must be a contiguous int32 tensor of {2 * int(n_pairs)} elements, got {out.dtype} {tuple(out.shape)}")
    with torch.cuda.device(out.device):
        check(_lib.lib().dm_pair_epoch_orient(int(seed) & 0xFFFFFFFFFFFFFFFF, int(epoch), int(n_pairs), int(batch), int(mask), out.data_ptr(),
                                              _stream()), "dm_pair_epoch_orient")


@dataclass(frozen=True)
class Radiometric:
    contrast: float = 0.2
    brightness: float = 0.1
    colour: float = 0.05

    def __post_init__(self):
        for name, top in (("contrast", 0.5), ("brightness", 0.25), ("colour", 0.25)):
            v = getattr(self, name)
            if isinstance(v, bool) or not isinstance(v, (int, float)) or not 0.0 <= float(v) <= top:
                raise ValueError(f"Radiometric: {name} must be a number in 0 .. {top}, got {v!r}")

    def spans(self) -> Tuple[int, int, int]:
        return int(round(256 * self.contrast)), int(round(256 * self.colour)), int(round(255 * 256 * self.brightness))

    @staticmethod
    def of(value) -> Optional["Radiometric"]:
        if value is None or isinstance(value, Radiometric):
            return value
        if isinstance(value, (tuple, list)) and len(value) == 3:
            return Radiometric(*value)
        raise ValueError(f"radiometric must be None, an ops.Radiometric or a (contrast, brightness, colour) triple, got {value!r}")


def pair_epoch_radiometric(seed: int, epoch: int, n_pairs: int, batch: int, bands: int, gain_span: int, band_span: int, offset_span: int,
                           out: torch.Tensor) -> None:
    _need_cuda(out)
    if out.dtype != torch.int32 or not out.is_contiguous() or out.numel() != 4 * int(n_pairs) * int(bands):
        raise ValueError(f"pair_epoch_radiometric: out must be a contiguous int32 tensor of {4 * int(n_pairs) * int(bands)} elements "
                         f"([2 n_pairs, bands, 2]), got {out.dtype} {tuple(out.shape)}")
    with torch.cuda.device(out.device):
        check(_lib.lib().dm_pair_epoch_radiometric(int(seed) & 0xFFFFFFFFFFFFFFFF, int(epoch), int(n_pairs), int(batch), int(bands),
                                                   int(gain_span), int(band_span), int(offset_span), out.data_ptr(), _stream()),
              "dm_pair_epoch_radiometric")


def pair_epoch_draw(pairs: torch.Tensor, pair_flag: torch.Tensor, poly_off: torch.Tensor, poly_pts: torch.Tensor, pt_tile: torch.Tensor,
                    pt_xy: torch.Tensor, pt_inner: torch.Tensor, pt_obj: torch.Tensor, pt_region: torch.Tensor, seed: int, epoch: int, batch: int,
                    tile_id: torch.Tensor, xy: torch.Tensor, inner: torch.Tensor, obj: torch.Tensor, region: torch.Tensor, flag: torch.Tensor,
                    point_id: Optional[torch.Tensor] = None) -> None:
    if pairs.dim() != 2 or pairs.shape[1] != 2:
        raise ValueError(f"pair_epoch_draw: pairs must be [N, 2], got {tuple(pairs.shape)}")
    N, n_pts = pairs.shape[0], pt_tile.numel()
    cols = {"pairs": (pairs, torch.int32, 2 * N), "pair_flag": (pair_flag, torch.int32, N), "poly_off": (poly_off, torch.int32, poly_off.numel()),
            "poly_pts": (poly_pts, torch.int32, poly_pts.numel()), "pt_tile": (pt_tile, torch.int32, n_pts), "pt_xy": (pt_xy, torch.int32, 2 * n_pts),
            "pt_inner": (pt_inner, torch.int32, n_pts), "pt_obj": (pt_obj, torch.int32, n_pts), "pt_region": (pt_region, torch.float32, 15 * n_pts),
            "tile_id": (tile_id, torch.int32, 2 * N), "xy": (xy, torch.int32, 4 * N), "inner": (inner, torch.int32, 2 * N),
            "obj": (obj, torch.int32, 2 * N), "region": (region, torch.float32, 30 * N), "flag": (flag, torch.float32, N),
            "point_id": (point_id, torch.int32, 2 * N)}
    _need_cuda(*(t for t, _, _ in cols.values()))
    for name, (t, dtype, numel) in cols.items():
        if t is not None and (t.dtype != dtype or not t.is_contiguous() or t.numel() != numel):
            raise ValueError(f"pair_epoch_draw: {name} must be a contiguous {dtype} tensor of {numel} elements, got {t.dtype} {tuple(t.shape)}")
    a = _lib.DmPairDraw()
    for name, (t, _, _) in cols.items():
        setattr(a, name, _ptr(t))
    a.seed = int(seed) & 0xFFFFFFFFFFFFFFFF
    a.n_pairs, a.n_poly, a.n_poly_pts, a.n_pts = N, poly_off.numel() - 1, poly_pts.numel(), n_pts
    a.epoch, a.batch = int(epoch), int(batch)
    with torch.cuda.device(pairs.device):
        check(_lib.lib().dm_pair_epoch_draw(C.byref(a), _stream()), "dm_pair_epoch_draw")


def patch_pyramid_cols(tile: torch.Tensor, xy: torch.Tensor, windows: torch.Tensor, target: int, grid: int = 8,
                       dtype: torch.dtype = torch.bfloat16, max_window: Optional[int] = None, resize: str = "opencv") -> PatchCols:
    _need_cuda(tile, xy, windows)
    if tile.dtype != torch.uint8:
        raise ValueError("tile must be uint8")
    bands, H, W = tile.shape
    P = xy.shape[0]
    if target % grid:
        raise ValueError(f"target {target} is not a multiple of the token grid {grid}")
    ps = target // grid
    if max_window is None:
        max_window = int(windows.max().item())
    cols = torch.empty((P * grid * grid, bands * ps * ps), dtype=dtype, device=tile.device)
    check(_lib.lib().dm_patch_pyramid_cols(tile.contiguous().data_ptr(), bands, H, W, xy.to(torch.int32).contiguous().data_ptr(),
                                           windows.to(torch.int32).contiguous().data_ptr(), max_window, P, target, grid, _resize_rule(resize),
                                           cols.data_ptr(), _dt(cols), _stream()), "dm_patch_pyramid_cols")
    return PatchCols(cols, P, target, ps, bands)


def adam_step(param, grad, m, v, step, lr=1e-4, beta1=0.9, beta2=0.999, eps=1e-8, grad_scale=1.0, param_lp=None):
    _need_cuda(param, grad, m, v)
    check(_lib.lib().dm_adam_step(param.data_ptr(), grad.data_ptr(), m.data_ptr(), v.data_ptr(), _ptr(param_lp), param.numel(), step,
                                  lr, beta1, beta2, eps, grad_scale, _stream()), "dm_adam_step")


def adam_hyper(step: int, lr: float, beta1: float = 0.9, beta2: float = 0.999) -> torch.Tensor:
    h = torch.empty(2, dtype=torch.float32).pin_memory() if torch.cuda.is_available() else torch.empty(2, dtype=torch.float32)
    check(_lib.lib().dm_adam_hyper(step, lr, beta1, beta2, h.data_ptr()), "dm_adam_hyper")
    return h


def adam_step_dev(param, grad, m, v, hyper_dev, beta1=0.9, beta2=0.999, eps=1e-8, grad_scale=1.0, param_lp=None, param_lo=None):
    _need_cuda(param, grad, m, v, hyper_dev)
    if param_lo is not None:
        check(_lib.lib().dm_adam_step_dev_pair(param.data_ptr(), grad.data_ptr(), m.data_ptr(), v.data_ptr(), param_lp.data_ptr(), param_lo.data_ptr(),
                                               param.numel(), hyper_dev.data_ptr(), beta1, beta2, eps, grad_scale, _stream()), "dm_adam_step_dev_pair")
        return
    check(_lib.lib().dm_adam_step_dev(param.data_ptr(), grad.data_ptr(), m.data_ptr(), v.data_ptr(), _ptr(param_lp), param.numel(),
                                      hyper_dev.data_ptr(), beta1, beta2, eps, grad_scale, _stream()), "dm_adam_step_dev")


def segment_mean(F: torch.Tensor, ptr: torch.Tensor, idx: torch.Tensor, validate: bool = True) -> torch.Tensor:
    _need_cuda(F, ptr, idx)
    S, D = ptr.numel() - 1, F.shape[1]
    if validate and S > 0:
        bad = (ptr[1:] < ptr[:-1]).any() | (ptr[0] != 0) | (ptr[-1] > idx.numel())
        if idx.numel():
            bad = bad | (idx.min() < 0) | (idx.max() >= F.shape[0])
        if bool(bad):
            raise ValueError("segment_mean: ptr must be non-decreasing from 0 to <= len(idx) and idx must index rows of F")
    pooled = torch.empty((S, D), dtype=torch.float32, device=F.device)
    check(_lib.lib().dm_segment_mean(F.data_ptr(), ptr.data_ptr(), idx.data_ptr(), pooled.data_ptr(), S, D, _stream()), "dm_segment_mean")
    return pooled


def edge_similarity(pooled: torch.Tensor, edges: torch.Tensor, margin: float = 1.0, validate: bool = True):
    _need_cuda(pooled, edges)
    E, D = edges.shape[0], pooled.shape[1]
    if validate and E > 0 and int(edges.max()) >= pooled.shape[0]:
        raise ValueError(f"edge_similarity: edge endpoint {int(edges.max())} is not a row of pooled (S = {pooled.shape[0]}); negative ids mean 'no polygon'")
    simi = torch.empty(E, dtype=torch.float32, device=pooled.device)
    merge = torch.empty(E, dtype=torch.uint8, device=pooled.device)
    check(_lib.lib().dm_edge_similarity(pooled.data_ptr(), edges.data_ptr(), simi.data_ptr(), merge.data_ptr(), E, D, margin, _stream()),
          "dm_edge_similarity")
    return simi, merge


def contrastive_terms(a: torch.Tensor, b: torch.Tensor, flag: torch.Tensor, margin: float = 1.0,
                      d2: Optional[torch.Tensor] = None, term: Optional[torch.Tensor] = None):
    _need_cuda(a, b, flag, d2, term)
    if a.dim() != 2 or tuple(a.shape) != tuple(b.shape) or a.shape[0] < 1 or a.shape[1] < 1:
        raise ValueError(f"contrastive_terms: a and b must be the same non-empty [B, D], got {tuple(a.shape)} and {tuple(b.shape)}")
    B = a.shape[0]
    for name, t, shape in (("a", a, tuple(a.shape)), ("b", b, tuple(a.shape)), ("flag", flag, (B,)), ("d2", d2, (B,)), ("term", term, (B,))):
        if t is not None and (t.dtype != torch.float32 or not t.is_contiguous() or tuple(t.shape) != shape):
            raise ValueError(f"contrastive_terms: {name} must be a contiguous float32 tensor of shape {shape}, got {t.dtype} {tuple(t.shape)}")
    d2 = torch.empty(B, dtype=torch.float32, device=a.device) if d2 is None else d2
    term = torch.empty(B, dtype=torch.float32, device=a.device) if term is None else term
    with torch.cuda.device(a.device):
        check(_lib.lib().dm_contrastive_terms(a.data_ptr(), b.data_ptr(), flag.data_ptr(), float(margin), d2.data_ptr(), term.data_ptr(),
                                              B, a.shape[1], _stream()), "dm_contrastive_terms")
    return d2, term


PAIR_EVAL_MAX_THRESHOLDS = 1024


def pair_eval_summary(term: torch.Tensor, simi: torch.Tensor, flag: torch.Tensor, thresholds: torch.Tensor, validate: bool = True,
                      out: Optional[torch.Tensor] = None) -> torch.Tensor:
    _need_cuda(term, simi, flag, thresholds, out)
    N = term.numel()
    for name, t in (("term", term), ("simi", simi), ("flag", flag)):
        if t.dtype != torch.float32 or not t.is_contiguous() or t.dim() != 1 or t.numel() != N:
            raise ValueError(f"pair_eval_summary: {name} must be a contiguous float32 [N] tensor (N = {N}), got {t.dtype} {tuple(t.shape)}")
    if not 1 <= N <= 2 ** 31 - 1:
        raise ValueError(f"pair_eval_summary: N = {N} pairs (1 .. 2^31 - 1)")
    T = thresholds.numel()
    if thresholds.dtype != torch.float32 or not thresholds.is_contiguous() or thresholds.dim() != 1 or not 1 <= T <= PAIR_EVAL_MAX_THRESHOLDS:
        raise ValueError(f"pair_eval_summary: thresholds must be a contiguous float32 [T] tensor with 1 <= T <= {PAIR_EVAL_MAX_THRESHOLDS}, "
                         f"got {thresholds.dtype} {tuple(thresholds.shape)}")
    if validate:
        th = thresholds.cpu()
        if not bool(torch.isfinite(th).all()) or (T > 1 and not bool((th[1:] > th[:-1]).all())):
            raise ValueError("pair_eval_summary: thresholds must be finite and strictly ascending")
    if out is None:
        out = torch.empty(2 * T + 2, dtype=torch.int64, device=term.device)
    elif out.dtype != torch.int64 or not out.is_contiguous() or out.numel() != 2 * T + 2:
        raise ValueError(f"pair_eval_summary: out must be a contiguous int64 tensor of {2 * T + 2} elements")
    lib = _lib.lib()
    ws = workspace(lib.dm_pair_eval_workspace_bytes(N, T), term.device, slot="eval")
    with torch.cuda.device(term.device):
        check(lib.dm_pair_eval_summary(term.data_ptr(), simi.data_ptr(), flag.data_ptr(), N, thresholds.data_ptr(), T, ws.data_ptr(),
                                       out.data_ptr(), out.data_ptr() + 16, out.data_ptr() + 8, _stream()), "dm_pair_eval_summary")
    return out


_DIST_DTYPES = {torch.float32: DM_F32, torch.float64: _lib.DM_F64}


def pairwise_distance(X: torch.Tensor, Y: torch.Tensor) -> torch.Tensor:
    _need_cuda(X, Y)
    if X.dim() != 2 or Y.dim() != 2:
        raise ValueError(f"pairwise_distance: X and Y must be 2-D, got {tuple(X.shape)} and {tuple(Y.shape)}")
    if X.shape[1] != Y.shape[1]:
        raise ValueError(f"pairwise_distance: feature widths differ ({X.shape[1]} != {Y.shape[1]})")
    if X.dtype != Y.dtype or X.dtype not in _DIST_DTYPES:
        raise ValueError(f"pairwise_distance: X and Y must both be float32 or float64, got {X.dtype} and {Y.dtype}")
    if X.device != Y.device:
        raise ValueError(f"pairwise_distance: X on {X.device}, Y on {Y.device}")
    n, m, p = X.shape[0], Y.shape[0], X.shape[1]
    if n == 0 or m == 0:
        return torch.empty((n, m), dtype=X.dtype, device=X.device)
    if p == 0:
        return torch.zeros((n, m), dtype=X.dtype, device=X.device)
    X, Y = X.detach().contiguous(), Y.detach().contiguous()
    D = torch.empty((n, m), dtype=X.dtype, device=X.device)
    with torch.cuda.device(X.device):
        check(_lib.lib().dm_pairwise_distance(X.data_ptr(), Y.data_ptr(), D.data_ptr(), n, m, p, _DIST_DTYPES[X.dtype], _stream()),
              "dm_pairwise_distance")
    return D


def _as_operand(t: torch.Tensor, dtype: torch.dtype) -> torch.Tensor:
    t = t.contiguous()
    if t.dtype == dtype:
        return t
    if t.dtype == torch.float32:
        return cast(t, dtype)
    raise ValueError(f"cannot use a {t.dtype} gradient with {dtype} operands")


class _GradSlot:
    __slots__ = ("param", "out", "direct")

    def __init__(self, param, shape, device, use_sink: bool = True):
        sink = getattr(param, "_dm_grad_sink", None) if use_sink else None
        self.param, self.direct = param, sink is not None
        self.out = sink.view(shape) if self.direct else torch.empty(shape, dtype=torch.float32, device=device)

    def acc(self) -> bool:
        if not self.direct:
            return False
        st = getattr(self.param, "_dm_gw", None)
        if st is None or st[0]:
            return True
        st[0] = True
        return False

    def grad(self):
        if self.direct:
            return None
        return self.out if self.out.shape == self.param.shape else self.out.view(self.param.shape)


def _norm_slots(gamma, beta, cols: int, device, need: bool = True):
    g = _GradSlot(gamma, (cols,), device, use_sink=need)
    b = _GradSlot(beta, (cols,), device, use_sink=g.direct)
    if b.direct != g.direct:
        g = _GradSlot(gamma, (cols,), device, use_sink=False)
    acc = g.acc()
    b.acc()
    return g, b, acc


def attach(g: torch.Tensor, name: str, payload, *extra) -> None:
    setattr(g, name, (payload, _grad_tag(g)) + extra)


def attached(g: torch.Tensor, name: str, *extra):
    rider = getattr(g, name, None)
    if rider is None or rider[1] != _grad_tag(g) or tuple(rider[2:]) != extra:
        return None
    return rider[0]


def _linear_backward(x, w, dy, need_dx, need_dw, need_db, wparam, bparam):
    M, K = x.shape
    N = w.shape[0]
    dx = None
    if need_dx:
        dx = torch.empty((M, K), dtype=x.dtype, device=x.device)
        gemm(DM_NN, dy, w, dx, M, K, N, lda=N, ldb=K, ldc=K)
    bs = _GradSlot(bparam, (N,), x.device) if need_db else None
    ws = _GradSlot(wparam, (N, K), x.device) if need_dw else None
    if need_dw:
        gemm(DM_TN, dy, x, ws.out, N, K, M, lda=N, ldb=K, ldc=K, accumulate=ws.acc(),
             colsum_out=bs.out if need_db else None, colsum_accumulate=bs.acc() if need_db else False)
    elif need_db:
        colsum(dy, bs.out, accumulate=bs.acc())
    return dx, (ws.grad() if need_dw else None), (bs.grad() if need_db else None)


class LinearFn(torch.autograd.Function):

    @staticmethod
    def forward(ctx, x, weight, bias, residual, out_dtype):
        _save_products(ctx)
        x = x.contiguous()
        M, K = x.shape
        N = weight.shape[0]
        w = lp_weight(weight, x.dtype, (N, K))
        y = torch.empty((M, N), dtype=out_dtype, device=x.device)
        gemm(DM_NT, x, w, y, M, N, K, lda=K, ldb=K, ldc=N, bias=bias,
             residual=None if residual is None else residual.contiguous())
        ctx.save_for_backward(x, w)
        ctx.has_bias = bias is not None
        ctx.params = (weight, bias)
        return y

    @staticmethod
    @_replay_products
    def backward(ctx, dy):
        x, w = ctx.saved_tensors
        dres = dy if ctx.needs_input_grad[3] else None
        dyo = _as_operand(dy, x.dtype)
        dx, dw, db = _linear_backward(x, w, dyo, ctx.needs_input_grad[0], ctx.needs_input_grad[1],
                                      ctx.has_bias and ctx.needs_input_grad[2], *ctx.params)
        return dx, dw, db, dres, None


class PatchEmbedCatFn(torch.autograd.Function):

    @staticmethod
    def forward(ctx, S, T, *args):
        _save_products(ctx)
        cols, weights, biases = args[:S], args[S:2 * S], args[2 * S:3 * S]
        B = cols[0].shape[0] // T
        Cc = weights[0].shape[0]
        cube = torch.empty((B, S * T, Cc), dtype=torch.float32, device=cols[0].device)
        flat = cube.view(-1)
        ws = []
        for i in range(S):
            c = cols[i].contiguous()
            K = c.shape[1]
            w = lp_weight(weights[i], c.dtype, (Cc, K))
            ws.append(w)
            gemm(DM_NT, c, w, flat[i * T * Cc:], B * T, Cc, K, lda=K, ldb=K, ldc=Cc, bias=biases[i], rows_per_group=T, group_stride=S * T * Cc)
        ctx.save_for_backward(*cols, *ws)
        ctx.cfg = (S, T, B, Cc)
        ctx.params = (weights, biases)
        if _FUSED_GLUE:
            cube._dm_lp_rows = (S, T)
        return cube

    @staticmethod
    @_replay_products
    def backward(ctx, dcube):
        S, T, B, Cc = ctx.cfg
        saved = ctx.saved_tensors
        cols, ws = saved[:S], saved[S:]
        weights, biases = ctx.params
        grads_w, grads_b = [], []
        same = all(c.dtype == cols[0].dtype for c in cols)
        rg = attached(dcube, "_dm_lp_regrouped", (S, T))
        if rg is not None and same and rg.dtype == cols[0].dtype and tuple(rg.shape) == (S, B, T, Cc) and tuple(dcube.shape) == (B, S * T, Cc):
            dys = rg
        else:
            dys = torch.empty((S, B, T, Cc), dtype=cols[0].dtype, device=dcube.device).copy_(dcube.contiguous().view(B, S, T, Cc).transpose(0, 1)) if same else None
        for i in range(S):
            c = cols[i]
            K = c.shape[1]
            dy = dys[i].view(B * T, Cc) if same else dcube[:, i * T:(i + 1) * T, :].to(c.dtype).reshape(B * T, Cc)
            need_w, need_b = ctx.needs_input_grad[2 + S + i], ctx.needs_input_grad[2 + 2 * S + i]
            _, dw, db = _linear_backward(c, ws[i], dy, False, need_w, need_b and biases[i] is not None, weights[i], biases[i])
            grads_w.append(dw)
            grads_b.append(db)
        return (None, None) + (None,) * S + tuple(grads_w) + tuple(grads_b)


class MlpFn(torch.autograd.Function):

    @staticmethod
    def forward(ctx, x, w1, b1, w2, b2, residual, out_dtype):
        _save_products(ctx)
        x = x.contiguous()
        M, K = x.shape
        Hd, N = w1.shape[0], w2.shape[0]
        w1c = cast(w1.reshape(Hd, K), x.dtype)
        w2c = cast(w2.reshape(N, Hd), x.dtype)
        pre = torch.empty((M, Hd), dtype=x.dtype, device=x.device)
        h = torch.empty((M, Hd), dtype=x.dtype, device=x.device)
        gemm(DM_NT, x, w1c, h, M, Hd, K, lda=K, ldb=K, ldc=Hd, bias=b1, epilogue=DM_EPI_GELU_GRAD, aux=pre, ldaux=Hd)
        y = torch.empty((M, N), dtype=out_dtype, device=x.device)
        gemm(DM_NT, h, w2c, y, M, N, Hd, lda=Hd, ldb=Hd, ldc=N, bias=b2,
             residual=None if residual is None else residual.contiguous())
        ctx.save_for_backward(x, w1c, w2c, pre, h)
        ctx.params = (w1, b1, w2, b2)
        return y

    @staticmethod
    @_replay_products
    def backward(ctx, dy):
        x, w1c, w2c, pre, h = ctx.saved_tensors
        M, K = x.shape
        Hd, N = w1c.shape[0], w2c.shape[0]
        need = ctx.needs_input_grad
        dres = dy if need[5] else None
        dyo = _as_operand(dy, x.dtype)
        w1, b1, w2, b2 = ctx.params
        _, dw2, db2 = _linear_backward(h, w2c, dyo, False, need[3], need[4], w2, b2)
        dpre = torch.empty((M, Hd), dtype=x.dtype, device=x.device)
        gemm(DM_NN, dyo, w2c, dpre, M, Hd, N, lda=N, ldb=Hd, ldc=Hd, epilogue=DM_EPI_MUL, aux=pre, ldaux=Hd)
        dx, dw1, db1 = _linear_backward(x, w1c, dpre, need[0], need[1], need[2], w1, b1)
        return dx, dw1, db1, dw2, db2, dres, None


class LayerNormFn(torch.autograd.Function):

    @staticmethod
    def forward(ctx, x, gamma, beta, eps, out_dtype, grad_lp=None):
        x = x.contiguous()
        y, mean, rstd = layernorm_fwd(x, gamma, beta, eps, out_dtype)
        ctx.save_for_backward(x, gamma, mean, rstd)
        ctx.params = (gamma, beta)
        ctx.want_lp = grad_lp == torch.bfloat16 and _FUSED_GLUE
        return y

    @staticmethod
    def backward(ctx, dy):
        x, gamma, mean, rstd = ctx.saved_tensors
        g, b, acc = _norm_slots(*ctx.params, gamma.numel(), x.device, need=ctx.needs_input_grad[1] and ctx.needs_input_grad[2])
        r = layernorm_bwd(dy.contiguous(), x, gamma, mean, rstd, dgamma=g.out, dbeta=b.out, accumulate=acc, want_lp=ctx.want_lp)
        dx = r[0]
        if ctx.want_lp:
            attach(dx, "_dm_lp_copy", r[1])
        return dx, g.grad(), b.grad(), None, None, None


class AttentionFn(torch.autograd.Function):

    @staticmethod
    def forward(ctx, qkv, table, index32, B, N, H, D, scale):
        qkv = qkv.contiguous()
        route = _AttnRoute(table, index32, qkv.dtype, B, N, H, D)
        out, lse, keep, _ = _attention_forward(qkv, table, index32, route, B, N, H, D, scale)
        ctx.save_for_backward(None if route.kind == "split" else qkv, out, lse, *keep, index32, None if route.kind == "dense" else table)
        ctx.dims = (B, N, H, D, scale, None if table is None else table.shape[0])
        ctx.route = route
        return out

    @staticmethod
    def backward(ctx, dout):
        B, N, H, D, scale, n_bins = ctx.dims
        qkv, out, lse, k0, k1, index32, table = ctx.saved_tensors
        want_table = n_bins is not None and ctx.needs_input_grad[1]
        dout = dout.contiguous().float() if ctx.route.kind == "split" else _as_operand(dout, qkv.dtype)
        dqkv, slab, info = _attention_backward(ctx.route, qkv, (k0, k1), table, out, dout, lse, index32 if want_table else None, n_bins,
                                               B, N, H, D, scale)
        dtable = None
        if want_table:
            dtable = torch.empty((n_bins, H), dtype=torch.float32, device=out.device)
            relpos_bias_scatter(slab, dtable, B, H, info, n_bins)
        return dqkv, dtable, None, None, None, None, None, None


class GRUCellFn(torch.autograd.Function):

    @staticmethod
    def forward(ctx, gi, gh, h):
        _need_cuda(gi, gh, h)
        B, H = h.shape
        if gi.shape != (B, 3 * H) or gh.shape != (B, 3 * H) or gi.stride(1) != 1:
            raise ValueError(f"GRUCellFn: gi {tuple(gi.shape)} / gh {tuple(gh.shape)} do not fit h {tuple(h.shape)}")
        gh, h = gh.contiguous(), h.contiguous()
        h_new = torch.empty_like(h)
        saved = torch.empty((B, 4 * H), dtype=torch.float32, device=h.device)
        check(_lib.lib().dm_gru_cell_fwd(gi.data_ptr(), gi.stride(0), gh.data_ptr(), h.data_ptr(), h_new.data_ptr(), saved.data_ptr(), B, H,
                                         _stream()), "dm_gru_cell_fwd")
        ctx.save_for_backward(saved, h)
        return h_new

    @staticmethod
    def backward(ctx, dh_new):
        saved, h = ctx.saved_tensors
        B, H = h.shape
        dh_new = dh_new.contiguous()
        dgi = torch.empty((B, 3 * H), dtype=torch.float32, device=h.device)
        dgh, dh = torch.empty_like(dgi), torch.empty_like(h)
        check(_lib.lib().dm_gru_cell_bwd(dh_new.data_ptr(), saved.data_ptr(), h.data_ptr(), dgi.data_ptr(), dgh.data_ptr(), dh.data_ptr(), B, H,
                                         _stream()), "dm_gru_cell_bwd")
        return dgi, dgh, dh


class BatchNormReluFn(torch.autograd.Function):

    @staticmethod
    def forward(ctx, x, gamma, beta, running_mean, running_var, mask, rows_per_sample, eps, momentum, training, relu):
        _need_cuda(x, gamma, beta, running_mean, running_var, mask)
        x = x.float().contiguous()
        M, Cc = x.shape
        if training and M <= 1:
            raise ValueError(f"Expected more than 1 value per channel when training, got input size {tuple(x.shape)}")
        y = torch.empty_like(x)
        mean = torch.empty(Cc, dtype=torch.float32, device=x.device)
        rstd = torch.empty(Cc, dtype=torch.float32, device=x.device)
        if mask is not None:
            mask = mask.float().contiguous()
            if mask.shape != (M // rows_per_sample, Cc):
                raise ValueError(f"mask must be [samples, C] = {(M // rows_per_sample, Cc)}, got {tuple(mask.shape)}")
        ws = workspace(_lib.lib().dm_batchnorm_workspace_bytes(M, Cc), x.device, "bn")
        check(_lib.lib().dm_batchnorm_fwd(x.data_ptr(), gamma.data_ptr(), beta.data_ptr(), _ptr(running_mean), _ptr(running_var), _ptr(mask),
                                          rows_per_sample, y.data_ptr(), mean.data_ptr(), rstd.data_ptr(), M, Cc, eps, momentum, int(training),
                                          int(relu), ws.data_ptr(), _stream()), "dm_batchnorm_fwd")
        ctx.save_for_backward(x, y, gamma, mask, mean, rstd)
        ctx.cfg = (rows_per_sample, bool(training), bool(relu))
        ctx.params = (gamma, beta)
        return y

    @staticmethod
    def backward(ctx, dy):
        x, y, gamma, mask, mean, rstd = ctx.saved_tensors
        rows_per_sample, training, relu = ctx.cfg
        M, Cc = x.shape
        dx = torch.empty_like(x)
        g, b, acc = _norm_slots(*ctx.params, Cc, x.device)
        ws = workspace(_lib.lib().dm_batchnorm_workspace_bytes(M, Cc), x.device, "bn")
        check(_lib.lib().dm_batchnorm_bwd(dy.float().contiguous().data_ptr(), x.data_ptr(), y.data_ptr(), gamma.data_ptr(), _ptr(mask), rows_per_sample,
                                          mean.data_ptr(), rstd.data_ptr(), dx.data_ptr(), g.out.data_ptr(), b.out.data_ptr(), int(acc), M, Cc,
                                          int(training), int(relu), ws.data_ptr(), _stream()), "dm_batchnorm_bwd")
        return dx, g.grad(), b.grad(), None, None, None, None, None, None, None, None


class TokenPoolFn(torch.autograd.Function):

    @staticmethod
    def forward(ctx, x, S, side):
        x = x.contiguous()
        B, N, Cc = x.shape
        y = torch.empty((B, S * (side // 2) ** 2, Cc), dtype=torch.float32, device=x.device)
        check(_lib.lib().dm_token_pool_fwd(x.data_ptr(), y.data_ptr(), B, S, side, Cc, _stream()), "dm_token_pool_fwd")
        ctx.dims = (B, S, side, Cc)
        return y

    @staticmethod
    def backward(ctx, dy):
        B, S, side, Cc = ctx.dims
        dy = dy.contiguous()
        dx = torch.empty((B, S * side * side, Cc), dtype=torch.float32, device=dy.device)
        check(_lib.lib().dm_token_pool_bwd(dy.data_ptr(), dx.data_ptr(), B, S, side, Cc, _stream()), "dm_token_pool_bwd")
        return dx, None, None


def pool_norm_fused(x: torch.Tensor, numerics: str) -> bool:
    return (_FUSED_GLUE and numerics != "bf16x3" and x.is_cuda and x.dtype == torch.float32
            and bool(_lib.lib().dm_pool_layernorm_ok(x.shape[-1])))


def pool_norm(x, gamma, beta, eps, S, side, numerics):
    if pool_norm_fused(x, numerics):
        return PoolNormFn.apply(x, gamma, beta, eps, S, side, act_dtype(numerics))
    return LayerNormFn.apply(TokenPoolFn.apply(x, S, side), gamma, beta, eps, torch.float32)


class PoolNormFn(torch.autograd.Function):

    @staticmethod
    def forward(ctx, x, gamma, beta, eps, S, side, grad_lp):
        x = x.contiguous()
        B, N, Cc = x.shape
        if N != S * side * side:
            raise ValueError(f"PoolNormFn: {N} tokens are not {S} scales of {side} x {side}")
        n = S * (side // 2) ** 2
        pooled = torch.empty((B, n, Cc), dtype=torch.float32, device=x.device)
        y = torch.empty((B, n, Cc), dtype=torch.float32, device=x.device)
        mean = torch.empty(B * n, dtype=torch.float32, device=x.device)
        rstd = torch.empty(B * n, dtype=torch.float32, device=x.device)
        check(_lib.lib().dm_pool_layernorm_fwd(x.data_ptr(), gamma.data_ptr(), beta.data_ptr(), pooled.data_ptr(), y.data_ptr(), mean.data_ptr(),
                                               rstd.data_ptr(), B, S, side, Cc, eps, _stream()), "dm_pool_layernorm_fwd")
        ctx.save_for_backward(pooled, gamma, mean, rstd)
        ctx.dims = (B, S, side, Cc)
        ctx.params = (gamma, beta)
        ctx.want_lp = grad_lp == torch.bfloat16
        return y

    @staticmethod
    def backward(ctx, dy):
        pooled, gamma, mean, rstd = ctx.saved_tensors
        B, S, side, Cc = ctx.dims
        dy = dy.contiguous()
        if dy.dtype != torch.float32 or dy.numel() != pooled.numel():
            raise ValueError("PoolNormFn.backward: the gradient must be fp32 and of the pooled rows' size")
        dev = dy.device
        dx = torch.empty((B, S * side * side, Cc), dtype=torch.float32, device=dev)
        dx_lp = torch.empty(dx.shape, dtype=torch.bfloat16, device=dev) if ctx.want_lp else None
        g, b, acc = _norm_slots(*ctx.params, Cc, dev, need=ctx.needs_input_grad[1] and ctx.needs_input_grad[2])
        deferred = _deferred(g.direct)
        part = _partial_rows(Cc, dev, deferred)
        n_part = C.c_int32(0)
        sums = (None, None, 0, part.data_ptr(), C.byref(n_part)) if deferred else (g.out.data_ptr(), b.out.data_ptr(), int(acc), part.data_ptr(), None)
        check(_lib.lib().dm_pool_layernorm_bwd(dy.data_ptr(), pooled.data_ptr(), gamma.data_ptr(), mean.data_ptr(), rstd.data_ptr(), dx.data_ptr(),
                                               _ptr(dx_lp), *sums, B, S, side, Cc, _stream()), "dm_pool_layernorm_bwd")
        if deferred:
            _reduce(part, g.out, b.out, n_part.value, 2 * Cc, Cc, acc, deferred)
        if dx_lp is not None:
            attach(dx, "_dm_lp_copy", dx_lp)
        return dx, g.grad(), b.grad(), None, None, None, None


class GroupMeanFn(torch.autograd.Function):

    @staticmethod
    def forward(ctx, x, g):
        x = x.contiguous()
        rows, Cc = x.numel() // (x.shape[-1] * g), x.shape[-1]
        y = torch.empty((rows, Cc), dtype=torch.float32, device=x.device)
        check(_lib.lib().dm_group_mean_fwd(x.data_ptr(), y.data_ptr(), rows, g, Cc, _stream()), "dm_group_mean_fwd")
        ctx.dims = (rows, g, Cc, x.shape)
        return y

    @staticmethod
    def backward(ctx, dy):
        rows, g, Cc, xshape = ctx.dims
        dy = dy.contiguous()
        dx = torch.empty(xshape, dtype=torch.float32, device=dy.device)
        check(_lib.lib().dm_group_mean_bwd(dy.data_ptr(), dx.data_ptr(), rows, g, Cc, _stream()), "dm_group_mean_bwd")
        return dx, None


class ContrastiveLossFn(torch.autograd.Function):

    @staticmethod
    def forward(ctx, a, b, flag, margin):
        a, b = a.contiguous(), b.contiguous()
        B, D = a.shape
        flag = flag.to(torch.float32).contiguous()
        loss = torch.empty(1, dtype=torch.float32, device=a.device)
        da, db = torch.empty_like(a), torch.empty_like(b)
        check(_lib.lib().dm_contrastive_loss(a.data_ptr(), b.data_ptr(), flag.data_ptr(), margin, 1.0, loss.data_ptr(),
                                             da.data_ptr(), db.data_ptr(), B, D, _stream()), "dm_contrastive_loss")
        ctx.save_for_backward(da, db)
        return loss.reshape(())

    @staticmethod
    def backward(ctx, g):
        da, db = ctx.saved_tensors
        if is_unit_grad(g):
            return da, db, None, None
        return da * g, db * g, None, None


_unit_grads = {}


def unit_grad(device) -> torch.Tensor:
    key = torch.device(device)
    t = _unit_grads.get(key)
    if t is None:
        t = _unit_grads[key] = torch.ones((), dtype=torch.float32, device=key)
    return t


def is_unit_grad(g: torch.Tensor) -> bool:
    t = _unit_grads.get(g.device)
    return t is not None and g.data_ptr() == t.data_ptr() and g.dim() == 0


def split_halves(f: torch.Tensor):
    B = f.shape[0] // 2
    a, b = f[:B], f[B:]
    a._dm_pair, b._dm_pair = f, f
    return a, b


def stacked_halves(a: torch.Tensor, b: torch.Tensor):
    f = getattr(a, "_dm_pair", None)
    if f is None or f is not getattr(b, "_dm_pair", None) or f.dim() != 2 or not f.is_contiguous() or a.shape != b.shape:
        return None
    B, D = a.shape
    if tuple(f.shape) != (2 * B, D) or a.data_ptr() != f.data_ptr() or b.data_ptr() != f.data_ptr() + B * D * f.element_size():
        return None
    return f


class ContrastivePairLossFn(torch.autograd.Function):

    @staticmethod
    def forward(ctx, both, flag, margin):
        B, D = both.shape[0] // 2, both.shape[1]
        flag = flag.to(torch.float32).contiguous()
        loss = torch.empty(1, dtype=torch.float32, device=both.device)
        d = torch.empty_like(both)
        check(_lib.lib().dm_contrastive_loss(both.data_ptr(), both[B:].data_ptr(), flag.data_ptr(), margin, 1.0, loss.data_ptr(),
                                             d.data_ptr(), d[B:].data_ptr(), B, D, _stream()), "dm_contrastive_loss")
        ctx.save_for_backward(d)
        return loss.reshape(())

    @staticmethod
    def backward(ctx, g):
        d, = ctx.saved_tensors
        return (d if is_unit_grad(g) else d * g), None, None


def contrastive_loss(a: torch.Tensor, b: torch.Tensor, flag: torch.Tensor, margin: float) -> torch.Tensor:
    both = stacked_halves(a, b) if (a.dtype == torch.float32 and b.dtype == torch.float32) else None
    if both is not None:
        return ContrastivePairLossFn.apply(both, flag, margin)
    return ContrastiveLossFn.apply(a, b, flag, margin)


class CrossEntropyFn(torch.autograd.Function):

    @staticmethod
    def forward(ctx, logits, target):
        _need_cuda(logits, target)
        x = logits.float().contiguous()
        B, K = x.shape
        loss = torch.empty(1, dtype=torch.float32, device=x.device)
        dl = torch.empty_like(x)
        if target.dtype.is_floating_point:
            if target.shape != x.shape:
                raise ValueError(f"probability targets must be [B,K] = {tuple(x.shape)}, got {tuple(target.shape)}")
            t = target.float().contiguous()
            ti, tp = 0, t.data_ptr()
        else:
            if target.shape != (B,):
                raise ValueError(f"index targets must be [B] = ({B},), got {tuple(target.shape)}")
            t = target.to(torch.int64).contiguous()
            if B and (int(t.min()) < 0 or int(t.max()) >= K):
                raise IndexError(f"Target {int(t.max())} is out of bounds.")
            ti, tp = t.data_ptr(), 0
        check(_lib.lib().dm_cross_entropy(x.data_ptr(), ti, tp, 1.0, loss.data_ptr(), dl.data_ptr(), B, K, _stream()), "dm_cross_entropy")
        ctx.save_for_backward(dl)
        return loss.reshape(())

    @staticmethod
    def backward(ctx, g):
        (dl,) = ctx.saved_tensors
        return dl * g, None




def lp_weight(weight: torch.Tensor, dtype: torch.dtype, shape2d) -> torch.Tensor:
    if dtype == torch.float32:
        return weight.reshape(shape2d)
    lp = getattr(weight, "_dm_lp", None)
    if lp is not None and lp.dtype == dtype:
        return lp.reshape(shape2d)
    return cast(weight.reshape(shape2d), dtype)


def pair_weight(weight: torch.Tensor, w2d: torch.Tensor) -> Planes:
    src = getattr(weight, "_dm_pair_src", None)
    if src is not None and _PLANES:
        flat, off = src
        rows, cols = w2d.shape
        if rows * cols == weight.numel() and off % 8 == 0 and flat.shape[1] % 8 == 0:
            return Planes(torch.as_strided(flat, (2, rows, cols), (flat.shape[1], cols, 1), off))
    return split_planes(w2d)


def _grad_tag(g: torch.Tensor):
    return (g.data_ptr(), g._version)


def _operand_grad(dy: torch.Tensor, dtype: torch.dtype, lp: Optional[torch.Tensor] = None) -> torch.Tensor:
    if dy.dtype == dtype and dy.is_contiguous():
        return dy
    if lp is not None and lp.dtype == dtype and lp.numel() == dy.numel():
        return lp.reshape(dy.shape)
    return _as_operand(dy, dtype)


_WGRAD_GROUP_TOKENS = int(os.environ.get("DM_WGRAD_GROUP", "12288"))
_WGRAD_PAIR = os.environ.get("DM_WGRAD_PAIR", "1") != "0"


class _WgradQueue:

    def __init__(self, fused: bool, M: int):
        self.grouped = [] if (fused and 0 < M <= _WGRAD_GROUP_TOKENS) else None
        self.late = [] if (self.grouped is None and fused and _WGRAD_PAIR) else None

    def add(self, *a, pair: bool = False, **kw) -> None:
        if self.grouped is not None:
            self.grouped.append((a, kw))
        elif self.late is not None and pair:
            self.late.append((a, kw))
        else:
            gemm(*a, **kw)

    def flush(self) -> None:
        for calls in (self.grouped, self.late):
            if calls:
                gemm_grouped(calls)


class BlockFn(torch.autograd.Function):

    @staticmethod
    def forward(ctx, x, n1w, n1b, table, index32, qkv_w, qkv_b, proj_w, proj_b, n2w, n2b, fc1_w, fc1_b, fc2_w, fc2_b,
                heads, eps, scale, dtype):
        _save_products(ctx)
        lp_rows = getattr(x, "_dm_lp_rows", None)
        ctx.lp_rows = lp_rows if (lp_rows is not None and x.dim() == 3 and lp_rows[0] * lp_rows[1] == x.shape[1]) else None
        x = x.contiguous()
        B, N, Cc = x.shape
        M, Hd, D = B * N, fc1_w.shape[0], Cc // heads
        dev = x.device
        wq, wp = lp_weight(qkv_w, dtype, (3 * Cc, Cc)), lp_weight(proj_w, dtype, (Cc, Cc))
        w1, w2 = lp_weight(fc1_w, dtype, (Hd, Cc)), lp_weight(fc2_w, dtype, (Cc, Hd))
        x2d = x.view(M, Cc)
        planes = (dtype == torch.float32 and _FP32_PRODUCTS == "bf16x3" and planes_ok(M, Cc) and planes_ok(M, Hd) and planes_ok(Hd, Cc)
                  and Cc <= _PAIR_LN_MAX_COLS and M * Cc * Cc >= _SPLIT_MIN_WORK)
        if planes:
            wq, wp, w1, w2 = (pair_weight(P, w) for P, w in ((qkv_w, wq), (proj_w, wp), (fc1_w, w1), (fc2_w, w2)))
        y1, mean1, rstd1 = layernorm_fwd(x2d, n1w, n1b, eps, dtype, pair=planes)
        route = _AttnRoute(table, index32, dtype, B, N, heads, D)
        split = route.kind == "split"
        qkv = (Planes(torch.empty((2, M, 3 * Cc), dtype=torch.bfloat16, device=dev)) if (planes and split)
               else torch.empty((M, 3 * Cc), dtype=dtype, device=dev))
        gemm(DM_NT, y1, wq, qkv, M, 3 * Cc, Cc, lda=Cc, ldb=Cc, ldc=3 * Cc, bias=qkv_b)
        o, lse, keep, o_op = _attention_forward(qkv, table, index32, route, B, N, heads, D, scale, out_pair=planes and split)
        bias, bias_t = (None, None) if split else keep
        x1 = torch.empty((M, Cc), dtype=torch.float32, device=dev)
        if o_op is None:
            o_op = split_planes(o.view(M, Cc)) if planes else o.view(M, Cc)
        gemm(DM_NT, o_op, wp, x1, M, Cc, Cc, lda=Cc, ldb=Cc, ldc=Cc, bias=proj_b, residual=x2d)
        y2, mean2, rstd2 = layernorm_fwd(x1, n2w, n2b, eps, dtype, pair=planes)
        h = Planes(torch.empty((2, M, Hd), dtype=torch.bfloat16, device=dev)) if planes else torch.empty((M, Hd), dtype=dtype, device=dev)
        if any(ctx.needs_input_grad):
            pre = torch.empty((M, Hd), dtype=dtype, device=dev)
            gemm(DM_NT, y2, w1, h, M, Hd, Cc, lda=Cc, ldb=Cc, ldc=Hd, bias=fc1_b, epilogue=DM_EPI_GELU_GRAD, aux=pre, ldaux=Hd)
        else:
            pre = None
            gemm(DM_NT, y2, w1, h, M, Hd, Cc, lda=Cc, ldb=Cc, ldc=Hd, bias=fc1_b, epilogue=DM_EPI_GELU)
        x2 = torch.empty((M, Cc), dtype=torch.float32, device=dev)
        gemm(DM_NT, h, w2, x2, M, Cc, Hd, lda=Hd, ldb=Hd, ldc=Cc, bias=fc2_b, residual=x1)
        if planes:
            y1, y2, h, wq, wp, w1, w2, o_op = y1.t, y2.t, h.t, wq.t, wp.t, w1.t, w2.t, o_op.t
            if isinstance(qkv, Planes):
                qkv = qkv.t
        ctx.planes = planes
        ctx.save_for_backward(x2d, mean1, rstd1, y1, qkv, o, lse, bias, bias_t, index32, x1, mean2, rstd2, y2, pre, h,
                              wq, wp, w1, w2, n1w, n2w, o_op if planes else None)
        ctx.dims = (B, N, Cc, heads, D, Hd, scale, None if table is None else table.shape[0])
        ctx.route = route
        ctx.split_imgs = keep if split else None
        ctx.params = (n1w, n1b, table, qkv_w, qkv_b, proj_w, proj_b, n2w, n2b, fc1_w, fc1_b, fc2_w, fc2_b)
        return x2.view(B, N, Cc)

    _PARAMS = ("n1w", "n1b", "table", "qkv_w", "qkv_b", "proj_w", "proj_b", "n2w", "n2b", "fc1_w", "fc1_b", "fc2_w", "fc2_b")

    @staticmethod
    @_replay_products
    def backward(ctx, dx2):
        (x, mean1, rstd1, y1, qkv, o, lse, bias, bias_t, index32, x1, mean2, rstd2, y2, pre, h,
         wq, wp, w1, w2, n1w, n2w, o_op) = ctx.saved_tensors
        planes = ctx.planes
        if planes:
            y1, y2, h, wq, wp, w1, w2, o_op = (Planes(t_) for t_ in (y1, y2, h, wq, wp, w1, w2, o_op))
        P = dict(zip(BlockFn._PARAMS, ctx.params))
        B, N, Cc, heads, D, Hd, scale, n_bins = ctx.dims
        M = B * N
        dtype, dev = (torch.float32 if planes else y1.dtype), x.device
        lp = dtype != torch.float32
        slots = {}
        wgrads = _WgradQueue(lp or planes, M)

        def linear_grads(name, g2d, inp, n_out, n_in, pair=False):
            w = slots[name + "_w"] = _GradSlot(P[name + "_w"], (n_out, n_in), dev)
            b = slots[name + "_b"] = _GradSlot(P[name + "_b"], (n_out,), dev)
            if planes and not isinstance(g2d, Planes):
                g2d = split_planes(g2d)
            wgrads.add(DM_TN, g2d, inp, w.out, n_out, n_in, M, lda=n_out, ldb=n_in, ldc=n_in, accumulate=w.acc(),
                       colsum_out=b.out, colsum_accumulate=b.acc(), pair=pair)
            return g2d

        def norm_grads(name, dy_, x_, gamma, mean, rstd, dres, regroup=None):
            g, b, acc = _norm_slots(P[name + "w"], P[name + "b"], Cc, dev)
            slots[name + "w"], slots[name + "b"] = g, b
            return layernorm_bwd(dy_, x_, gamma, mean, rstd, dres=dres, dgamma=g.out, dbeta=b.out, accumulate=acc, want_lp=lp, defer=g.direct,
                                 want_pair=planes, regroup=regroup)

        lp_copy, dy_pair = attached(dx2, "_dm_lp_copy"), attached(dx2, "_dm_planes")
        dx2 = dx2.contiguous().view(M, Cc)
        dy = _operand_grad(dx2, dtype, lp_copy)
        if planes and isinstance(dy_pair, Planes) and (dy_pair.rows, dy_pair.cols) == (M, Cc):
            dy = dy_pair
        dy = linear_grads("fc2", dy, h, Cc, Hd)
        dpre = Planes(torch.empty((2, M, Hd), dtype=torch.bfloat16, device=dev)) if planes else torch.empty((M, Hd), dtype=dtype, device=dev)
        gemm(DM_NN, dy, w2, dpre, M, Hd, Cc, lda=Cc, ldb=Hd, ldc=None if planes else Hd, epilogue=DM_EPI_MUL, aux=pre, ldaux=Hd)
        dpre = linear_grads("fc1", dpre, y2, Hd, Cc)
        dy2 = torch.empty((M, Cc), dtype=dtype, device=dev)
        gemm(DM_NN, dpre, w1, dy2, M, Cc, Hd, lda=Hd, ldb=Cc, ldc=Cc)
        r = norm_grads("n2", dy2, x1, n2w, mean2, rstd2, dx2)
        dx1, dx1_op = r[0], (r[1] if (lp or planes) else r[0])
        dx1_op = linear_grads("proj", dx1_op, o_op if planes else o.view(M, Cc), Cc, Cc, pair=True)
        do = torch.empty((M, Cc), dtype=dtype, device=dev)
        gemm(DM_NN, dx1_op, wp, do, M, Cc, Cc, lda=Cc, ldb=Cc, ldc=Cc)
        keep = ctx.split_imgs if ctx.route.kind == "split" else (bias, bias_t)
        ctx.split_imgs = None
        want_table = P["table"] is not None
        dqkv, slab, info = _attention_backward(ctx.route, qkv, keep, P["table"].detach() if want_table else None, o, do.view(B, N, Cc), lse,
                                               index32 if want_table else None, n_bins, B, N, heads, D, scale, pair=planes)
        if want_table:
            t = slots["table"] = _GradSlot(P["table"], (n_bins, heads), dev)
            relpos_bias_scatter(slab, t.out, B, heads, info, n_bins, accumulate=t.acc())
        dqkv = linear_grads("qkv", dqkv if isinstance(dqkv, Planes) else dqkv.view(M, 3 * Cc), y1, 3 * Cc, Cc, pair=True)
        dy1 = torch.empty((M, Cc), dtype=dtype, device=dev)
        gemm(DM_NN, dqkv, wq, dy1, M, Cc, 3 * Cc, lda=3 * Cc, ldb=Cc, ldc=Cc)
        regroup = ctx.lp_rows if (lp and dtype == torch.bfloat16 and _FUSED_GLUE and Cc <= _PAIR_LN_MAX_COLS) else None
        r = norm_grads("n1", dy1, x, n1w, mean1, rstd1, dx1, regroup=regroup)
        wgrads.flush()
        dx = r[0].view(B, N, Cc)
        if regroup is not None:
            attach(dx, "_dm_lp_regrouped", r[1], regroup)
        elif lp:
            attach(dx, "_dm_lp_copy", r[1])
        if planes:
            attach(dx, "_dm_planes", r[1])
        grads = [slots[n].grad() if n in slots else None for n in BlockFn._PARAMS]
        return (dx, *grads[:3], None, *grads[3:], None, None, None, None)
```

include/deepmerge_hip.h:

```cpp
#ifndef DEEPMERGE_HIP_H
#define DEEPMERGE_HIP_H

#include <stdint.h>

#ifdef __cplusplus
extern "C" {
#endif

typedef enum { DM_F32 = 0, DM_BF16 = 1,
               DM_BF16_PAIR = 2,
               DM_F64 = 3
} DmDtype;

typedef enum {
  DM_OK = 0,
  DM_ERR_BAD_SHAPE = -1,
  DM_ERR_BAD_DTYPE = -2,
  DM_ERR_BAD_ALIGN = -3,
  DM_ERR_WORKSPACE = -4,
  DM_ERR_HIP = -5,
  DM_ERR_UNSUPPORTED = -6
} DmStatus;

int dm_abi_version(void);
const char *dm_last_error(void);
const char *dm_arch(void);

typedef enum { DM_NT = 0, DM_NN = 1, DM_TN = 2 } DmGemmLayout;
typedef enum { DM_EPI_NONE = 0, DM_EPI_GELU = 1, DM_EPI_DGELU = 2, DM_EPI_GELU_GRAD = 3, DM_EPI_MUL = 4 } DmEpilogue;

typedef struct {
  int32_t layout;
  int32_t ab_dtype;
  int32_t c_dtype;
  int32_t aux_dtype;
  int32_t M, N, K;
  int32_t epilogue;
  int32_t accumulate;
  int32_t split_k;
  const void *A; int64_t lda;
  const void *B; int64_t ldb;
  void *C; int64_t ldc;
  const float *bias;
  const float *residual; int64_t ldr;
  void *aux; int64_t ldaux;
  int32_t rows_per_group; int64_t group_stride;
  void *workspace; int64_t workspace_bytes;
  float *colsum_a; int32_t colsum_accumulate;
  int32_t k_fold;
  int64_t a_fold[3], b_fold[3];
  int64_t c_plane;
} DmGemmArgs;

int dm_gemm(const DmGemmArgs *args, void *stream);
int64_t dm_gemm_workspace_bytes(int32_t layout, int32_t M, int32_t N, int32_t K);
int dm_gemm_grouped(const DmGemmArgs *args, int32_t n, void *stream);

int dm_attention_fwd(const void *qkv, const float *bias, void *out, float *lse,
                     int32_t B, int32_t N, int32_t H, int32_t D, float scale, int32_t dtype, void *stream);
int32_t dm_attention_relpos_inkernel(int32_t B, int32_t N, int32_t H, int32_t D, int32_t cube_s, int32_t cube_h,
                                     int32_t cube_w, int32_t dtype);
int dm_attention_fwd_relpos(const void *qkv, const float *table, int32_t cube_s, int32_t cube_h, int32_t cube_w,
                            void *out, float *lse, int32_t B, int32_t N, int32_t H, int32_t D, float scale,
                            int32_t dtype, void *stream);
int dm_attention_bwd(const void *qkv, const float *bias, const float *bias_t, const void *out, const void *dout,
                     const float *lse, void *dqkv, float *delta, float *dbias_slab, int32_t B, int32_t N, int32_t H,
                     int32_t D, float scale, int32_t dtype, void *stream);
int dm_attention_bwd_relpos(const void *qkv, const float *table, int32_t cube_s, int32_t cube_h, int32_t cube_w,
                            const float *bias, const float *bias_t, const void *out, const void *dout, const float *lse,
                            void *dqkv, float *delta, float *dbias_slab, int32_t B, int32_t N, int32_t H, int32_t D,
                            float scale, int32_t dtype, void *stream);
int32_t dm_attention_split_ok(int32_t B, int32_t N, int32_t H, int32_t D, int32_t has_table, int32_t cube_s, int32_t cube_h,
                              int32_t cube_w);
int dm_attention_split_fwd(const float *qkv, void *qkv_hi, void *qkv_lo, const float *table, int32_t cube_s, int32_t cube_h,
                           int32_t cube_w, float *out, float *lse, int32_t B, int32_t N, int32_t H, int32_t D, float scale,
                           void *stream);
int dm_attention_split_fwd_pair(const float *qkv, void *qkv_hi, void *qkv_lo, const float *table, int32_t cube_s, int32_t cube_h,
                                int32_t cube_w, float *out, void *out_pair, float *lse, int32_t B, int32_t N, int32_t H, int32_t D,
                                float scale, void *stream);
int32_t dm_attention_split_bwd_chunks(int32_t B, int32_t N, int32_t H);
int dm_attention_split_bwd(const void *qkv_hi, const void *qkv_lo, const float *table, int32_t cube_s, int32_t cube_h,
                           int32_t cube_w, const float *out, const float *dout, void *dout_hi, void *dout_lo,
                           const float *lse, float *dqkv, float *delta, float *dbias_slab, int32_t B, int32_t N,
                           int32_t H, int32_t D, float scale, void *stream);
int dm_attention_split_bwd_pair(const void *qkv_hi, const void *qkv_lo, const float *table, int32_t cube_s, int32_t cube_h,
                                int32_t cube_w, const float *out, const float *dout, void *dout_hi, void *dout_lo,
                                const float *lse, void *dqkv_pair, float *delta, float *dbias_slab, int32_t B, int32_t N,
                                int32_t H, int32_t D, float scale, void *stream);
int32_t dm_attention_bwd_batch_chunks(int32_t B, int32_t N, int32_t H, int32_t dtype);

int dm_relpos_bias_gather(const float *table, const int32_t *index, float *bias, float *bias_t,
                          int32_t N, int32_t H, int32_t n_bins, void *stream);
int dm_relpos_bias_reduce(float *dbias_slab, const int32_t *positions, const int32_t *offsets, float *dtable,
                          int32_t chunks, int32_t H, int32_t N, int32_t n_bins, int32_t accumulate, void *stream);

int dm_layernorm_fwd(const float *x, const float *gamma, const float *beta, void *y, int32_t y_dtype,
                     float *mean, float *rstd, int32_t rows, int32_t cols, float eps, void *stream);
int dm_layernorm_bwd(const void *dy, int32_t dy_dtype, const float *x, const float *gamma,
                     const float *mean, const float *rstd, const float *dres, float *dx, void *dx_lp,
                     float *dgamma, float *dbeta, int32_t accumulate_params, float *partial,
                     int32_t rows, int32_t cols, void *stream);
int64_t dm_layernorm_bwd_partial_floats(int32_t cols);
int dm_layernorm_bwd_partials(const void *dy, int32_t dy_dtype, const float *x, const float *gamma,
                              const float *mean, const float *rstd, const float *dres, float *dx, void *dx_lp,
                              float *partial, int32_t rows, int32_t cols, int32_t *n_partial, void *stream);
int dm_layernorm_bwd_partials_pair(const void *dy, int32_t dy_dtype, const float *x, const float *gamma,
                                   const float *mean, const float *rstd, const float *dres, float *dx, void *dx_pair, float *partial,
                                   int32_t rows, int32_t cols, int32_t *n_partial, void *stream);
int dm_layernorm_bwd_partials_regroup(const void *dy, int32_t dy_dtype, const float *x, const float *gamma,
                                      const float *mean, const float *rstd, const float *dres, float *dx, void *dx_lp, float *partial,
                                      int32_t rows, int32_t cols, int32_t S, int32_t T, int32_t *n_partial, void *stream);
typedef struct DmReduceItem {
  const float *partial;
  float *out0, *out1;
  int32_t nrows, width, split, accumulate;
} DmReduceItem;
int dm_partial_reduce_batch(const DmReduceItem *items, int32_t n, void *stream);

int dm_token_pool_fwd(const float *x, float *y, int32_t B, int32_t S, int32_t side, int32_t C, void *stream);
int dm_token_pool_bwd(const float *dy, float *dx, int32_t B, int32_t S, int32_t side, int32_t C, void *stream);
int dm_pool_layernorm_ok(int32_t C);
int dm_pool_layernorm_fwd(const float *x, const float *gamma, const float *beta, float *pooled, float *y, float *mean, float *rstd,
                          int32_t B, int32_t S, int32_t side, int32_t C, float eps, void *stream);
int dm_pool_layernorm_bwd(const float *dy, const float *pooled, const float *gamma, const float *mean, const float *rstd, float *dx,
                          void *dx_lp, float *dgamma, float *dbeta, int32_t accumulate_params, float *partial, int32_t *n_partial,
                          int32_t B, int32_t S, int32_t side, int32_t C, void *stream);
int dm_group_mean_fwd(const float *x, float *y, int32_t rows, int32_t g, int32_t C, void *stream);
int dm_group_mean_bwd(const float *dy, float *dx, int32_t rows, int32_t g, int32_t C, void *stream);

int dm_colsum(const void *X, int32_t dtype, int64_t ldx, float *out, int32_t M, int32_t N,
              int32_t accumulate, float *partial, void *stream);
int64_t dm_colsum_partial_floats(int32_t N);

int dm_cast(const float *src, void *dst, int32_t dst_dtype, int64_t n, void *stream);

int dm_split_bf16(const float *src, int64_t ld, int64_t rows, int64_t cols, void *dst, int32_t stack, int32_t pattern, void *stream);
int64_t dm_split_colsum_partial_floats(int64_t rows, int64_t cols);
int dm_split_bf16_planes(const float *src, int64_t ld, int64_t rows, int64_t cols, void *dst, float *partial, int32_t *n_partial, void *stream);
int dm_split_bf16_colsum(const float *src, int64_t ld, int64_t rows, int64_t cols, void *dst, int32_t stack, int32_t pattern,
                         float *partial, int32_t *n_partial, void *stream);

int dm_patchify(const float *x, void *cols, int32_t dtype, int32_t B, int32_t C, int32_t side, int32_t p, void *stream);

int dm_contrastive_loss(const float *a, const float *b, const float *flag, float margin, float upstream,
                        float *loss, float *da, float *db, int32_t B, int32_t D, void *stream);

int dm_cross_entropy(const float *logits, const int64_t *target_index, const float *target_prob, float upstream,
                     float *loss, float *dlogits, int32_t B, int32_t K, void *stream);

int dm_adam_step(float *param, const float *grad, float *m, float *v, void *param_lp, int64_t n,
                 int32_t step, double lr, double beta1, double beta2, double eps, double grad_scale, void *stream);

int dm_adam_hyper(int32_t step, double lr, double beta1, double beta2, float *hyper_host);
int dm_adam_step_dev(float *param, const float *grad, float *m, float *v, void *param_lp, int64_t n, const float *hyper_dev,
                     double beta1, double beta2, double eps, double grad_scale, void *stream);
int dm_adam_step_dev_pair(float *param, const float *grad, float *m, float *v, void *param_hi, void *param_lo, int64_t n,
                          const float *hyper_dev, double beta1, double beta2, double eps, double grad_scale, void *stream);

int dm_segment_mean(const float *F, const int32_t *ptr, const int32_t *idx, float *pooled,
                    int32_t S, int32_t D, void *stream);
int dm_edge_similarity(const float *pooled, const int32_t *edges, float *simi, uint8_t *merge,
                       int32_t E, int32_t D, float margin, void *stream);
int dm_pairwise_distance(const void *X, const void *Y, void *D, int32_t n, int32_t m, int32_t p, int32_t dtype, void *stream);

#define DM_RESIZE_OPENCV 0
#define DM_RESIZE_EXACT_AREA 1
int dm_patch_pyramid(const uint8_t *tile, int32_t bands, int32_t H, int32_t W, const int32_t *xy, const int32_t *windows,
                     int32_t max_window, int32_t P, int32_t target, int32_t resize_rule, float *out, void *stream);
int dm_patch_pyramid_cols(const uint8_t *tile, int32_t bands, int32_t H, int32_t W, const int32_t *xy, const int32_t *windows,
                          int32_t max_window, int32_t P, int32_t target, int32_t grid, int32_t resize_rule, void *cols, int32_t dtype,
                          void *stream);

int dm_pair_batch_gather(const uint8_t *tiles, int32_t n_tiles, int32_t bands, int32_t H, int32_t W, const int32_t *tile_id,
                         const int32_t *xy, const int32_t *inner, const int32_t *obj, int32_t scale_index, int32_t max_window,
                         int32_t P, int32_t target, int32_t grid, int32_t resize_rule, void *out, int32_t dtype,
                         const float *region_features, float *designed, int32_t *error_flag, void *stream);
int dm_pair_batch_gather_oriented(const uint8_t *tiles, int32_t n_tiles, int32_t bands, int32_t H, int32_t W, const int32_t *tile_id,
                                  const int32_t *xy, const int32_t *inner, const int32_t *obj, const int32_t *orient, int32_t scale_index,
                                  int32_t max_window, int32_t P, int32_t target, int32_t grid, int32_t resize_rule, void *out,
                                  int32_t dtype, const float *region_features, float *designed, int32_t *error_flag, void *stream);
int dm_pair_batch_gather_augmented(const uint8_t *tiles, int32_t n_tiles, int32_t bands, int32_t H, int32_t W, const int32_t *tile_id,
                                   const int32_t *xy, const int32_t *inner, const int32_t *obj, const int32_t *orient,
                                   const int32_t *radio, int32_t scale_index, int32_t max_window, int32_t P, int32_t target, int32_t grid,
                                   int32_t resize_rule, void *out, int32_t dtype, const float *region_features, float *designed,
                                   int32_t *error_flag, void *stream);

typedef struct {
  const int32_t *pairs, *pair_flag, *poly_off, *poly_pts;
  const int32_t *pt_tile, *pt_xy, *pt_inner, *pt_obj;
  const float *pt_region;
  int32_t *tile_id, *xy, *inner, *obj;
  float *region, *flag;
  int32_t *point_id;
  uint64_t seed;
  int32_t n_pairs, n_poly, n_poly_pts, n_pts, epoch, batch;
} DmPairDraw;
int dm_pair_epoch_draw(const DmPairDraw *args, void *stream);
int dm_pair_epoch_orient(uint64_t seed, int32_t epoch, int32_t n_pairs, int32_t batch, int32_t mask, int32_t *orient, void *stream);
#define DM_RADIO_MAX_GAIN_SPAN 128
#define DM_RADIO_MAX_BAND_SPAN 64
#define DM_RADIO_MAX_OFFSET_SPAN 16320
int dm_pair_epoch_radiometric(uint64_t seed, int32_t epoch, int32_t n_pairs, int32_t batch, int32_t bands, int32_t gain_span,
                              int32_t band_span, int32_t offset_span, int32_t *radio, void *stream);

int dm_contrastive_terms(const float *a, const float *b, const float *flag, float margin, float *d2, float *term, int32_t B, int32_t D,
                         void *stream);
int64_t dm_pair_eval_workspace_bytes(int64_t N, int32_t T);
int dm_pair_eval_summary(const float *term, const float *simi, const float *flag, int64_t N, const float *thresholds, int32_t T,
                         void *workspace, double *loss_sum, int64_t *merged, int64_t *n_pos, void *stream);

int dm_label_stats(const int32_t *labels, const uint8_t *tile, int32_t bands, int32_t H, int32_t W, int32_t S,
                   int64_t *count, int64_t *sum, int64_t *sumsq, int32_t *bbox, int64_t *peri, void *stream);
int dm_label_features(const int64_t *count, const int64_t *sum, const int64_t *sumsq, const int32_t *bbox, const int64_t *peri,
                      int32_t S, int32_t bands, float *features, void *stream);
int dm_rag_edges(const int32_t *labels, int32_t H, int32_t W, int32_t S, int64_t *table_keys, int32_t *table_counts,
                 int32_t capacity_log2, int64_t *edge_keys, int32_t *edge_counts, int32_t max_edges, int32_t *n_edges,
                 int32_t *overflow, void *stream);

int dm_seam_stitch(const int32_t *a, const int32_t *b, int64_t n, int64_t S, int64_t *peri, int64_t *table_keys,
                   int32_t *table_counts, int32_t capacity_log2, int64_t *edge_keys, int32_t *edge_counts, int32_t max_edges,
                   int32_t *n_edges, int32_t *overflow, void *stream);

int dm_merge_round(const int32_t *edges, const uint8_t *merge, int32_t E, int32_t S, int32_t *parent, int32_t *changed,
                   int32_t init, void *stream);

typedef struct {
  const int32_t *ptr, *idx, *edges, *root, *pick, *rep, *region_of;
  const float *simi;
  const int32_t *weights;
  const int64_t *count, *sum, *sumsq;
  const int32_t *bbox;
  const int64_t *peri;
  int32_t *new_id, *hist_rank, *new_ptr, *new_idx, *new_rep, *new_region_of, *n_regions;
  int64_t *new_count, *new_sum, *new_sumsq;
  int32_t *new_bbox;
  int64_t *new_peri;
  int32_t *history;
  float *history_simi;
  int32_t C, P, E, S0, bands, round, hist_base, hist_cap;
} DmMergeFold;
int dm_merge_best(const int32_t *edges, const float *simi, int32_t E, int32_t C, float margin, uint64_t *best, void *stream);
int dm_merge_best_small(const int32_t *edges, const float *simi, int32_t E, int32_t C, const int64_t *count, int64_t min_area,
                        uint64_t *best, void *stream);
int dm_merge_accept(const int32_t *edges, const float *simi, int32_t E, int32_t C, const int64_t *count, int64_t min_area,
                    uint64_t *best, void *stream);
int dm_merge_match(const int32_t *edges, const uint64_t *best, int32_t E, int32_t C, uint8_t *picked, int32_t *root, int32_t *pick,
                   int32_t *n_picked, void *stream);
int dm_merge_fold_regions(const DmMergeFold *args, void *stream);
int dm_merge_edge_keys(const int32_t *edges, const int32_t *root, const int32_t *new_id, int32_t E, int32_t C, int64_t *keys,
                       void *stream);
int dm_merge_fold_edges(const int64_t *sorted_keys, const int64_t *order, const int32_t *weights, int32_t E, int32_t *new_edges,
                        int32_t *new_weights, int32_t *n_edges, void *stream);
int dm_relabel_raster(const int32_t *labels, const int32_t *map, int32_t *out, int64_t n, int32_t S, void *stream);

int dm_region_merge_cost(const int64_t *count, const int64_t *sum, const int64_t *sumsq, const int32_t *bbox, const int64_t *peri,
                         const int32_t *edges, const int32_t *weights, int32_t E, int32_t C, int32_t bands, double bw0, double bw1,
                         double bw2, double shape, double compactness, float *cost, void *stream);
int dm_pixel_regions(const uint8_t *tile, int32_t bands, int32_t H, int32_t W, int64_t *count, int64_t *sum, int64_t *sumsq,
                     int32_t *bbox, int64_t *peri, int32_t *edges, int32_t *weights, void *stream);

int dm_label_clearance(const int32_t *labels, int32_t H, int32_t W, int32_t max_window, uint64_t *bits, uint8_t *row_dist,
                       uint16_t *clearance, void *stream);
int dm_point_select_round(const int32_t *labels, const uint16_t *clearance, int32_t H, int32_t W, int32_t S, int32_t k, int32_t round,
                          uint64_t *best, int32_t *points, int32_t *point_clearance, int32_t *counts, int32_t *bbox, void *stream);
int dm_point_emit(const int32_t *counts, const int32_t *points, const int32_t *point_clearance, const int32_t *bbox, int32_t S, int32_t k,
                  int32_t max_window, int32_t capacity, int32_t *ptr, int32_t *xy, int32_t *label, int32_t *inner, int32_t *obj,
                  int32_t *round, void *stream);

#define DM_SCENE_POINTS_MAX_PIXELS (1LL << 48)
int dm_scene_point_init(uint64_t *best, int32_t *counts, int32_t *bbox, int32_t S, void *stream);
int dm_scene_point_select(const int32_t *labels, const uint16_t *clearance, int32_t wh, int32_t ww, int32_t cy0, int32_t cy1,
                          int32_t cx0, int32_t cx1, int64_t oy, int64_t ox, int64_t scene_h, int64_t scene_w, int32_t S, int32_t k,
                          int32_t round, const int32_t *points, const int32_t *counts, uint64_t *best, int32_t *bbox, void *stream);
int dm_scene_point_commit(uint64_t *best, int64_t scene_h, int64_t scene_w, int32_t S, int32_t k, int32_t *points,
                          int32_t *point_clearance, int32_t *counts, void *stream);

int dm_label_overlap(const int32_t *labels, const int32_t *truth, int32_t H, int32_t W, int64_t S, int64_t G, int64_t *table_keys,
                     int32_t *table_counts, int32_t capacity_log2, int64_t *cell_keys, int32_t *cell_counts, int32_t max_cells,
                     int32_t *n_cells, int32_t *overflow, void *stream);
int dm_overlap_reduce(const int64_t *cell_keys, const int32_t *cell_counts, int32_t K, int64_t S, int64_t G, uint64_t *row_best,
                      int64_t *row_labelled, int64_t *area, int32_t *owner, int32_t *owner_count, int64_t *size, int32_t *cover,
                      int64_t *summary, void *stream);
int dm_pair_flags(const int32_t *edges, int32_t E, const int64_t *area, const int32_t *owner, const int32_t *owner_count, int32_t S,
                  int32_t purity_pm, int8_t *flags, void *stream);

#define DM_BOUNDARY_MAX_TOLERANCE 64
int dm_boundary_bits(const int32_t *raster, int32_t H, int32_t W, int32_t n_ids, const int32_t *mapping, uint64_t *edge,
                     uint64_t *valid, void *stream);
int dm_boundary_counts(const uint64_t *label_edge, const uint64_t *truth_edge, const uint64_t *truth_valid, int32_t H, int32_t W,
                       int32_t d, int32_t y0, int32_t y1, int32_t x0, int32_t x1, int64_t *counts, void *stream);

int dm_slic_iterate(const uint8_t *tile, int32_t bands, int32_t H, int32_t W, int32_t cell, int32_t compactness, int32_t iters,
                    int32_t *centres, int64_t *sums, int32_t *labels, void *stream);
int dm_connected_labels(const int32_t *raster, int32_t H, int32_t W, int32_t use_background, int32_t background, int32_t *parent,
                        int32_t *chunk_counts, int32_t *labels, int32_t *n_labels, void *stream);
int dm_label_area(const int32_t *labels, int32_t H, int32_t W, int32_t S, int32_t *area, void *stream);
int dm_slic_absorb_pick(const int32_t *edges, const int32_t *weights, int32_t E, const int32_t *area, int32_t S, int32_t min_size,
                        uint64_t *best, uint8_t *merge, int32_t *n_picked, void *stream);

int dm_scene_slic_init(const uint8_t *core, int32_t bands, int32_t h, int32_t w, int32_t y0, int32_t x0, int32_t H, int32_t W,
                       int32_t cell, int32_t *centres, int64_t *sums, void *stream);
int dm_scene_slic_pass(const uint8_t *core, int32_t bands, int32_t h, int32_t w, int32_t y0, int32_t x0, int32_t H, int32_t W,
                       int32_t cell, int32_t compactness, const int32_t *centres, int64_t *sums, int32_t *labels, void *stream);
int dm_scene_slic_update(int32_t K, int32_t *centres, int64_t *sums, void *stream);

typedef struct DmVectorTrace {
  const int32_t *dart, *next, *lab, *other;
  const uint8_t *flags;
  const int64_t *key, *sum;
  const int32_t *ring_of_slot;
  const int64_t *ring_ptr;
  const int32_t *arc_base;
  int32_t *xy;
  int64_t *area2;
  int32_t *arc_first, *arc_left, *arc_right, *arc_vstart, *arc_count;
  const int32_t *arc_pos;
  const int64_t *arc_ptr;
  int32_t *arc_xy;
  int32_t W, D, R, n_arcs;
} DmVectorTrace;
int dm_vector_count(const int32_t *labels, int32_t H, int32_t W, uint8_t *mask, int32_t *tile_off, int32_t *n_darts, void *stream);
int dm_vector_emit(const uint8_t *mask, const int32_t *tile_off, int32_t H, int32_t W, int32_t *first_slot, int32_t *dart, void *stream);
int dm_vector_link(const int32_t *labels, const uint8_t *mask, const int32_t *first_slot, const int32_t *dart, int32_t H, int32_t W,
                   int32_t D, int32_t *next, int32_t *lab, int32_t *other, uint8_t *flags, int64_t *key, void *stream);
int dm_vector_head_round(const int64_t *key_in, const int32_t *jump_in, int64_t *key_out, int32_t *jump_out, int32_t D, int32_t *changed,
                         void *stream);
int dm_vector_rank_init(const int64_t *key, const int32_t *next, const uint8_t *flags, const int32_t *lab, int32_t D, int64_t *sum,
                        int32_t *nxt, int64_t *ring_key, int32_t *ring_slot, int32_t *n_rings, int32_t max_rings, void *stream);
int dm_vector_rank_round(const int64_t *sum_in, const int32_t *nxt_in, int64_t *sum_out, int32_t *nxt_out, int32_t D, int32_t *changed,
                         void *stream);
int dm_vector_ring_emit(const DmVectorTrace *t, void *stream);
int dm_vector_arc_emit(const DmVectorTrace *t, void *stream);

#define DM_SCENE_VECTOR_MAX_SIDE 2147483647LL
#define DM_SCENE_VECTOR_MAX_PIXELS (1LL << 60)
typedef struct DmSceneVectorTrace {
  const int64_t *dart;
  const int32_t *next, *lab, *other;
  const uint8_t *flags;
  const int64_t *key, *sum;
  const int32_t *ring_of_slot;
  const int64_t *ring_ptr;
  const int32_t *arc_base;
  int32_t *xy;
  int64_t *area2;
  int32_t *arc_first, *arc_left, *arc_right, *arc_vstart, *arc_count;
  const int32_t *arc_pos;
  const int64_t *arc_ptr;
  int32_t *arc_xy;
  int64_t W;
  int32_t D, R, n_arcs;
} DmSceneVectorTrace;
int dm_scene_vector_count(const int32_t *labels, int32_t H, int32_t W, int32_t cy0, int32_t cy1, int32_t cx0, int32_t cx1, uint8_t *mask,
                          uint8_t *core_mask, int32_t *tile_off, int32_t *n_darts, void *stream);
int dm_scene_vector_link(const int32_t *labels, const uint8_t *mask, const int32_t *dart, int32_t H, int32_t W, int32_t D, int64_t oy,
                         int64_t ox, int64_t scene_h, int64_t scene_w, int64_t *id, int64_t *succ, int32_t *lab, int32_t *other,
                         uint8_t *succ_flags, void *stream);
int dm_scene_vector_ring_emit(const DmSceneVectorTrace *t, void *stream);
int dm_scene_vector_arc_emit(const DmSceneVectorTrace *t, void *stream);

#define DM_RASTERIZE_SUBPIXEL 256
int dm_rasterize_count(const int32_t *xy, const int64_t *ring_ptr, const int32_t *vert_ring, int32_t V, int32_t R, int32_t H, int32_t W,
                       int32_t *count, void *stream);
int dm_rasterize_emit(const int32_t *xy, const int64_t *ring_ptr, const int32_t *vert_ring, const int32_t *ring_label, const int64_t *scan,
                      int32_t V, int32_t R, int64_t N, int32_t H, int32_t W, int64_t n_labels, int64_t *keys, void *stream);
int dm_rasterize_fill(const int64_t *keys, int64_t N, int32_t H, int32_t W, int32_t fill, int32_t *out, int32_t *error, void *stream);

int dm_rasterize_count_rows(const int32_t *xy, const int64_t *ring_ptr, const int32_t *vert_ring, int32_t V, int32_t R, int32_t H, int32_t W,
                            int32_t r0, int32_t r1, int32_t *count, void *stream);
int dm_rasterize_emit_rows(const int32_t *xy, const int64_t *ring_ptr, const int32_t *vert_ring, const int32_t *ring_label,
                           const int64_t *scan, int32_t V, int32_t R, int64_t N, int32_t H, int32_t W, int32_t r0, int32_t r1,
                           int64_t n_labels, int64_t *keys, void *stream);
int dm_rasterize_fill_window(const int64_t *keys, int64_t N, int32_t H, int32_t W, int32_t r0, int32_t r1, int32_t x0, int32_t x1,
                             int32_t fill, int32_t *out, int32_t *error, void *stream);

#define DM_SIMPLIFY_MAX_SIDE 32768
#define DM_SIMPLIFY_MAX_Q (1 << 20)
int dm_simplify_nodes(const int32_t *labels, int32_t H, int32_t W, uint8_t *keep, void *stream);
int dm_simplify_chains(const int32_t *arc_xy, const int64_t *arc_ptr, int32_t A, int64_t Va, int32_t H, int32_t W, int32_t q, uint8_t *keep,
                       int64_t *stack, void *stream);
int dm_simplify_arc_count(const int32_t *arc_xy, const int64_t *arc_ptr, int32_t A, int64_t Va, int32_t H, int32_t W, const uint8_t *keep,
                          int32_t *count, void *stream);
int dm_simplify_arc_emit(const int32_t *arc_xy, const int64_t *arc_ptr, const int64_t *new_ptr, int32_t A, int64_t Va, int64_t Vn, int32_t H,
                         int32_t W, const uint8_t *keep, int32_t *out_xy, void *stream);
int dm_simplify_ring_count(const int32_t *xy, const int64_t *ring_ptr, const int32_t *vert_ring, int32_t V, int32_t R, int32_t H, int32_t W,
                           const uint8_t *keep, int32_t *count, void *stream);
int dm_simplify_ring_emit(const int32_t *xy, const int64_t *ring_ptr, const int32_t *vert_ring, const int64_t *scan, const int64_t *new_ring_ptr,
                          int32_t V, int32_t R, int64_t Vn, int32_t H, int32_t W, const uint8_t *keep, int32_t *out_xy, int64_t *area2,
                          void *stream);

#define DM_SIMPLIFY_TOPOLOGY_CELL_LOG2 5
typedef struct DmSimplifyTopology {
  const int32_t *arc_xy;
// ... 106 lines not shown
```

Measured before the change: 6563 pairs/s.

## Add fused small-token attention kernels with in-kernel relpos bias and table grads

```diff
diff --git a/deepmerge_amd/_lib.py b/deepmerge_amd/_lib.py
--- a/deepmerge_amd/_lib.py
+++ b/deepmerge_amd/_lib.py
@@ -141,6 +141,10 @@
     "dm_attention_bwd_relpos": (_I, [_P, _P, _I, _I, _I, _P, _P, _P, _P, _P, _P, _P, _P, _I, _I, _I, _I, _F, _I, _P]),
     "dm_attention_bwd": (_I, [_P, _P, _P, _P, _P, _P, _P, _P, _P, _I, _I, _I, _I, _F, _I, _P]),
     "dm_attention_bwd_batch_chunks": (_I, [_I, _I, _I, _I]),
+    "dm_attention_small_ok": (_I, [_I, _I, _I, _I, _I, _I]),
+    "dm_attention_small_chunks": (_I, [_I, _I, _I]),
+    "dm_attention_small_fwd": (_I, [_P, _P, _P, _P, _P, _I, _I, _I, _I, _I, _F, _P]),
+    "dm_attention_small_bwd": (_I, [_P, _P, _P, _P, _P, _P, _P, _P, _P, _P, _P, _I, _I, _I, _I, _I, _I, _F, _P]),
     "dm_relpos_bias_gather": (_I, [_P, _P, _P, _P, _I, _I, _I, _P]),
     "dm_relpos_bias_reduce": (_I, [_P, _P, _P, _P, _I, _I, _I, _I, _I, _P]),
     "dm_layernorm_fwd": (_I, [_P, _P, _P, _P, _I, _P, _P, _I, _I, _F, _P]),
diff --git a/deepmerge_amd/csrc/dm_attention.hip b/deepmerge_amd/csrc/dm_attention.hip
--- a/deepmerge_amd/csrc/dm_attention.hip
+++ b/deepmerge_amd/csrc/dm_attention.hip
@@ -1,119 +1,11 @@
 #include "dm_common.h"
 #include "dm_mfma.h"
+#include "dm_attention_reg.h"
 #include "dm_attention_pipe.h"
 #include "dm_attention_x3.h"
 #include "dm_prof.h"
 
 namespace {
-
-constexpr int HD = 64;
-constexpr int QB = 64;
-
-template <typename T> struct AL {
-  static constexpr int RB = HD * (int)sizeof(T);
-  static constexpr int CPRW = RB / 16;
-  static constexpr int KBD = RB / 64;
-  static constexpr int EPC = 16 / (int)sizeof(T);
-  static constexpr int TPB = (sizeof(T) == 2) ? 2 : 1;
-};
-
-template <typename T> __device__ __forceinline__ int swz(int row);
-template <> __device__ __forceinline__ int swz<bf16_t>(int row) {
-  const int t0 = (row >> 1) & 1, t1 = (row >> 2) & 1, t2 = (row >> 3) & 1;
-  return ((t1 ^ t2) << 2) | (t0 << 1) | t1;
-}
-template <> __device__ __forceinline__ int swz<float>(int row) { return row & 15; }
-
-template <typename T> __device__ __forceinline__ int img_off(int row, int chunk) {
-  return row * AL<T>::RB + ((chunk ^ swz<T>(row)) << 4);
-}
-
-template <typename T>
-__device__ __forceinline__ void tile_to_lds(char *lds, const T *g, long long ld, int nvalid, int nrows, int t) {
-  using L = AL<T>;
-  const int c = t % L::CPRW;
-  constexpr int RPI = 256 / L::CPRW;
-  for (int row = t / L::CPRW; row < nrows; row += RPI) {
-    u32x4 v = {0u, 0u, 0u, 0u};
-    if (row < nvalid) v = *reinterpret_cast<const u32x4 *>(g + (long long)row * ld + c * L::EPC);
-    *reinterpret_cast<u32x4 *>(lds + img_off<T>(row, c)) = v;
-  }
-}
-
-template <typename T> __device__ __forceinline__ u32x4 frag_row(const char *lds, int row, int kb, int lane) {
-  return *reinterpret_cast<const u32x4 *>(lds + img_off<T>(row, kb * 4 + (lane >> 4)));
-}
-template <typename T> __device__ __forceinline__ u32x4 frag_tr(const char *lds, int d0, int m, int lane);
-template <> __device__ __forceinline__ u32x4 frag_tr<bf16_t>(const char *lds, int d0, int m, int lane) {
-  const int g = lane >> 4, q = (lane >> 2) & 3, p = lane & 3;
-  const int d = d0 + 4 * p;
-  u32x4 out;
-#pragma unroll
-  for (int half = 0; half < 2; ++half) {
-    const int k = 32 * m + 4 * g + 16 * half + q;
-    const u32x2 w = dm_ds_read_tr16(lds + img_off<bf16_t>(k, d >> 3) + ((d & 7) << 1));
-    out[2 * half] = w[0];
-    out[2 * half + 1] = w[1];
-  }
-  return out;
-}
-template <> __device__ __forceinline__ u32x4 frag_tr<float>(const char *lds, int d0, int m, int lane) {
-  const int g = lane >> 4, d = d0 + (lane & 15);
-  u32x4 out;
-#pragma unroll
-  for (int j = 0; j < 4; ++j) {
-    const int k = 16 * m + 4 * g + j;
-    out[j] = *reinterpret_cast<const unsigned int *>(lds + img_off<float>(k, d >> 2) + ((d & 3) << 2));
-  }
-  return out;
-}
-template <typename T> __device__ __forceinline__ u32x4 gl_frag(const T *rowp, bool valid, int kb, int lane) {
-  u32x4 v = {0u, 0u, 0u, 0u};
-  if (valid) v = *reinterpret_cast<const u32x4 *>(rowp + (kb * 4 + (lane >> 4)) * AL<T>::EPC);
-  return v;
-}
-
-template <typename T, int NKT> __device__ __forceinline__ u32x4 acc_frag(const f32x4 (&s)[NKT], int m) {
-  if constexpr (sizeof(T) == 2) {
-    const f32x4 lo = s[2 * m], hi = s[2 * m + 1];
-    bf16x8 r = {(bf16_t)lo[0], (bf16_t)lo[1], (bf16_t)lo[2], (bf16_t)lo[3], (bf16_t)hi[0], (bf16_t)hi[1], (bf16_t)hi[2], (bf16_t)hi[3]};
-    return __builtin_bit_cast(u32x4, r);
-  } else {
-    return __builtin_bit_cast(u32x4, s[m]);
-  }
-}
-
-template <typename T, int NKT>
-__device__ __forceinline__ void contract_tokens(f32x4 (&o)[4], const f32x4 (&s)[NKT], const char *img, int lane) {
-#pragma unroll
-  for (int m = 0; m < NKT / AL<T>::TPB; ++m) {
-    const u32x4 fp = acc_frag<T, NKT>(s, m);
-#pragma unroll
-    for (int dt = 0; dt < 4; ++dt) mma<T>(o[dt], fp, frag_tr<T>(img, dt * 16, m, lane));
-    if ((m & 1) == 1) __builtin_amdgcn_sched_barrier(0);
-  }
-}
-
-__device__ __forceinline__ float row_max(float v) {
-  v = fmaxf(v, __shfl_xor(v, 16, 64));
-  return fmaxf(v, __shfl_xor(v, 32, 64));
-}
-__device__ __forceinline__ float row_sum(float v) {
-  v += __shfl_xor(v, 16, 64);
-  return v + __shfl_xor(v, 32, 64);
-}
-
-template <typename T> __device__ __forceinline__ float fast_exp(float x);
-template <> __device__ __forceinline__ float fast_exp<float>(float x) { return expf(x); }
-template <> __device__ __forceinline__ float fast_exp<bf16_t>(float x) { return __expf(x); }
-
-__device__ __forceinline__ f32x4 load4_guard(const float *p, int i, int n, bool vec) {
-  if (vec) return (i < n) ? dm_load4(p + i) : (f32x4){0.f, 0.f, 0.f, 0.f};
-  f32x4 r;
-#pragma unroll
-  for (int e = 0; e < 4; ++e) r[e] = (i + e < n) ? p[i + e] : 0.f;
-  return r;
-}
 
 struct AttnParams {
   const void *qkv;
@@ -142,39 +34,6 @@
     }
   }
   return bv;
-}
-template <typename T>
-__device__ __forceinline__ f32x4 score_tile(const u32x4 (&fa)[AL<T>::KBD], const char *img, const f32x4 bv,
-                                            int N, int row, float scale, int lane, int kt) {
-  using L = AL<T>;
-  const int g = lane >> 4, li = lane & 15;
-  f32x4 a = {0.f, 0.f, 0.f, 0.f};
-#pragma unroll
-  for (int kb = 0; kb < L::KBD; ++kb) mma<T>(a, fa[kb], frag_row<T>(img, kt * 16 + li, kb, lane));
-  const int col = kt * 16 + 4 * g;
-#pragma unroll
-  for (int r = 0; r < 4; ++r) a[r] = (row < N && col + r < N) ? a[r] * scale + bv[r] : -INFINITY;
-  return a;
-}
-
-template <typename T> __device__ __forceinline__ u32x4 pack_tiles(const f32x4 (&tl)[AL<T>::TPB]) {
-  if constexpr (sizeof(T) == 2) {
-    bf16x8 r = {(bf16_t)tl[0][0], (bf16_t)tl[0][1], (bf16_t)tl[0][2], (bf16_t)tl[0][3],
-                (bf16_t)tl[1][0], (bf16_t)tl[1][1], (bf16_t)tl[1][2], (bf16_t)tl[1][3]};
-    return __builtin_bit_cast(u32x4, r);
-  } else {
-    return __builtin_bit_cast(u32x4, tl[0]);
-  }
-}
-
-template <typename T, int NB>
-__device__ __forceinline__ void contract_frags(f32x4 (&o)[4], const u32x4 (&f)[NB], const char *img, int lane) {
-#pragma unroll
-  for (int m = 0; m < NB; ++m) {
-#pragma unroll
-    for (int dt = 0; dt < 4; ++dt) mma<T>(o[dt], f[m], frag_tr<T>(img, dt * 16, m, lane));
-    if ((m & 1) == 1) __builtin_amdgcn_sched_barrier(0);
-  }
 }
 
 template <typename T, int NKT, bool FAST>
diff --git a/deepmerge_amd/csrc/dm_attention_reg.h b/deepmerge_amd/csrc/dm_attention_reg.h
--- /dev/null
+++ b/deepmerge_amd/csrc/dm_attention_reg.h
@@ -0,0 +1,150 @@
+#pragma once
+#include "dm_common.h"
+#include "dm_mfma.h"
+
+namespace {
+
+constexpr int HD = 64;
+constexpr int QB = 64;
+
+template <typename T> struct AL {
+  static constexpr int RB = HD * (int)sizeof(T);
+  static constexpr int CPRW = RB / 16;
+  static constexpr int KBD = RB / 64;
+  static constexpr int EPC = 16 / (int)sizeof(T);
+  static constexpr int TPB = (sizeof(T) == 2) ? 2 : 1;
+};
+
+template <typename T> __device__ __forceinline__ int swz(int row);
+template <> __device__ __forceinline__ int swz<bf16_t>(int row) {
+  const int t0 = (row >> 1) & 1, t1 = (row >> 2) & 1, t2 = (row >> 3) & 1;
+  return ((t1 ^ t2) << 2) | (t0 << 1) | t1;
+}
+template <> __device__ __forceinline__ int swz<float>(int row) { return row & 15; }
+
+template <typename T> __device__ __forceinline__ int img_off(int row, int chunk) {
+  return row * AL<T>::RB + ((chunk ^ swz<T>(row)) << 4);
+}
+
+template <typename T, int NT = 256>
+__device__ __forceinline__ void tile_to_lds(char *lds, const T *g, long long ld, int nvalid, int nrows, int t) {
+  using L = AL<T>;
+  const int c = t % L::CPRW;
+  constexpr int RPI = NT / L::CPRW;
+  for (int row = t / L::CPRW; row < nrows; row += RPI) {
+    u32x4 v = {0u, 0u, 0u, 0u};
+    if (row < nvalid) v = *reinterpret_cast<const u32x4 *>(g + (long long)row * ld + c * L::EPC);
+    *reinterpret_cast<u32x4 *>(lds + img_off<T>(row, c)) = v;
+  }
+}
+
+template <typename T> __device__ __forceinline__ u32x4 frag_row(const char *lds, int row, int kb, int lane) {
+  return *reinterpret_cast<const u32x4 *>(lds + img_off<T>(row, kb * 4 + (lane >> 4)));
+}
+template <typename T> __device__ __forceinline__ u32x4 frag_tr(const char *lds, int d0, int m, int lane);
+template <> __device__ __forceinline__ u32x4 frag_tr<bf16_t>(const char *lds, int d0, int m, int lane) {
+  const int g = lane >> 4, q = (lane >> 2) & 3, p = lane & 3;
+  const int d = d0 + 4 * p;
+  u32x4 out;
+#pragma unroll
+  for (int half = 0; half < 2; ++half) {
+    const int k = 32 * m + 4 * g + 16 * half + q;
+    const u32x2 w = dm_ds_read_tr16(lds + img_off<bf16_t>(k, d >> 3) + ((d & 7) << 1));
+    out[2 * half] = w[0];
+    out[2 * half + 1] = w[1];
+  }
+  return out;
+}
+template <> __device__ __forceinline__ u32x4 frag_tr<float>(const char *lds, int d0, int m, int lane) {
+  const int g = lane >> 4, d = d0 + (lane & 15);
+  u32x4 out;
+#pragma unroll
+  for (int j = 0; j < 4; ++j) {
+    const int k = 16 * m + 4 * g + j;
+    out[j] = *reinterpret_cast<const unsigned int *>(lds + img_off<float>(k, d >> 2) + ((d & 3) << 2));
+  }
+  return out;
+}
+template <typename T> __device__ __forceinline__ u32x4 gl_frag(const T *rowp, bool valid, int kb, int lane) {
+  u32x4 v = {0u, 0u, 0u, 0u};
+  if (valid) v = *reinterpret_cast<const u32x4 *>(rowp + (kb * 4 + (lane >> 4)) * AL<T>::EPC);
+  return v;
+}
+
+template <typename T, int NKT> __device__ __forceinline__ u32x4 acc_frag(const f32x4 (&s)[NKT], int m) {
+  if constexpr (sizeof(T) == 2) {
+    const f32x4 lo = s[2 * m], hi = s[2 * m + 1];
+    bf16x8 r = {(bf16_t)lo[0], (bf16_t)lo[1], (bf16_t)lo[2], (bf16_t)lo[3], (bf16_t)hi[0], (bf16_t)hi[1], (bf16_t)hi[2], (bf16_t)hi[3]};
+    return __builtin_bit_cast(u32x4, r);
+  } else {
+    return __builtin_bit_cast(u32x4, s[m]);
+  }
+}
+
+template <typename T, int NKT>
+__device__ __forceinline__ void contract_tokens(f32x4 (&o)[4], const f32x4 (&s)[NKT], const char *img, int lane) {
+#pragma unroll
+  for (int m = 0; m < NKT / AL<T>::TPB; ++m) {
+    const u32x4 fp = acc_frag<T, NKT>(s, m);
+#pragma unroll
+    for (int dt = 0; dt < 4; ++dt) mma<T>(o[dt], fp, frag_tr<T>(img, dt * 16, m, lane));
+    if ((m & 1) == 1) __builtin_amdgcn_sched_barrier(0);
+  }
+}
+
+__device__ __forceinline__ float row_max(float v) {
+  v = fmaxf(v, __shfl_xor(v, 16, 64));
+  return fmaxf(v, __shfl_xor(v, 32, 64));
+}
+__device__ __forceinline__ float row_sum(float v) {
+  v += __shfl_xor(v, 16, 64);
+  return v + __shfl_xor(v, 32, 64);
+}
+
+template <typename T> __device__ __forceinline__ float fast_exp(float x);
+template <> __device__ __forceinline__ float fast_exp<float>(float x) { return expf(x); }
+template <> __device__ __forceinline__ float fast_exp<bf16_t>(float x) { return __expf(x); }
+
+__device__ __forceinline__ f32x4 load4_guard(const float *p, int i, int n, bool vec) {
+  if (vec) return (i < n) ? dm_load4(p + i) : (f32x4){0.f, 0.f, 0.f, 0.f};
+  f32x4 r;
+#pragma unroll
+  for (int e = 0; e < 4; ++e) r[e] = (i + e < n) ? p[i + e] : 0.f;
+  return r;
+}
+
+template <typename T>
+__device__ __forceinline__ f32x4 score_tile(const u32x4 (&fa)[AL<T>::KBD], const char *img, const f32x4 bv,
+                                            int N, int row, float scale, int lane, int kt) {
+  using L = AL<T>;
+  const int g = lane >> 4, li = lane & 15;
+  f32x4 a = {0.f, 0.f, 0.f, 0.f};
+#pragma unroll
+  for (int kb = 0; kb < L::KBD; ++kb) mma<T>(a, fa[kb], frag_row<T>(img, kt * 16 + li, kb, lane));
+  const int col = kt * 16 + 4 * g;
+#pragma unroll
+  for (int r = 0; r < 4; ++r) a[r] = (row < N && col + r < N) ? a[r] * scale + bv[r] : -INFINITY;
+  return a;
+}
+
+template <typename T> __device__ __forceinline__ u32x4 pack_tiles(const f32x4 (&tl)[AL<T>::TPB]) {
+  if constexpr (sizeof(T) == 2) {
+    bf16x8 r = {(bf16_t)tl[0][0], (bf16_t)tl[0][1], (bf16_t)tl[0][2], (bf16_t)tl[0][3],
+                (bf16_t)tl[1][0], (bf16_t)tl[1][1], (bf16_t)tl[1][2], (bf16_t)tl[1][3]};
+    return __builtin_bit_cast(u32x4, r);
+  } else {
+    return __builtin_bit_cast(u32x4, tl[0]);
+  }
+}
+
+template <typename T, int NB>
+__device__ __forceinline__ void contract_frags(f32x4 (&o)[4], const u32x4 (&f)[NB], const char *img, int lane) {
+#pragma unroll
+  for (int m = 0; m < NB; ++m) {
+#pragma unroll
+    for (int dt = 0; dt < 4; ++dt) mma<T>(o[dt], f[m], frag_tr<T>(img, dt * 16, m, lane));
+    if ((m & 1) == 1) __builtin_amdgcn_sched_barrier(0);
+  }
+}
+
+}
diff --git a/deepmerge_amd/csrc/dm_attention_small.hip b/deepmerge_amd/csrc/dm_attention_small.hip
--- /dev/null
+++ b/deepmerge_amd/csrc/dm_attention_small.hip
@@ -0,0 +1,416 @@
+#include <algorithm>
+
+#include "dm_common.h"
+#include "dm_mfma.h"
+#include "dm_attention_reg.h"
+#include "dm_prof.h"
+
+namespace {
+
+struct SmallParams {
+  const bf16_t *qkv;
+  const float *table;
+  const int *index;
+  const int *csr_pos, *csr_off;
+  bf16_t *out;
+  const bf16_t *dout;
+  float *lse;
+  bf16_t *dqkv;
+  float *partial;
+  int B, N, H, n_bins, chunks;
+  float scale;
+};
+
+template <int NKT, int WPS> struct SG {
+  static constexpr int NK = NKT * 16;
+  static constexpr int IMG = NK * 128;
+  static constexpr int SLOTS = 4 / WPS;
+  static constexpr int NT = WPS * 64;
+  static constexpr int LD = NK + 4;
+  static constexpr int FWD_LDS = SLOTS * 2 * IMG + NK * LD * 4;
+  static constexpr int BWD_LDS = SLOTS * 4 * IMG + NK * LD * 4 + SLOTS * NK * 4;
+};
+
+template <int NK>
+__device__ __forceinline__ void build_plane(float *plane, const SmallParams &p, int h, int t) {
+  constexpr int IT = NK * NK / 256, LD = NK + 4;
+  const int N = p.N, NN = N * N;
+  const float rn = 1.0f / (float)N;
+  int bin[IT];
+#pragma unroll
+  for (int it = 0; it < IT; ++it) bin[it] = (t + it * 256 < NN) ? p.index[t + it * 256] : 0;
+  float v[IT];
+#pragma unroll
+  for (int it = 0; it < IT; ++it) v[it] = p.table[(long long)min(max(bin[it], 0), p.n_bins - 1) * p.H + h];
+#pragma unroll
+  for (int it = 0; it < IT; ++it) {
+    const int ij = t + it * 256;
+    if (ij < NN) {
+      const int i = (int)(((float)ij + 0.5f) * rn);
+      plane[i * LD + ij - i * N] = v[it];
+    }
+  }
+}
+__device__ __forceinline__ void chunk_range(const SmallParams &p, int chunk, int &b0, int &b1) {
+  b0 = (int)((long long)chunk * p.B / p.chunks);
+  b1 = (int)((long long)(chunk + 1) * p.B / p.chunks);
+}
+
+template <int NKT, int WPS>
+__global__ __launch_bounds__(256) void small_fwd_kernel(const SmallParams p) {
+  using T = bf16_t;
+  using G = SG<NKT, WPS>;
+  using L = AL<T>;
+  extern __shared__ __attribute__((aligned(16))) char smem[];
+  float *plane = reinterpret_cast<float *>(smem + G::SLOTS * 2 * G::IMG);
+  const int t = threadIdx.x, lane = t & 63, wave = t >> 6, g = lane >> 4, li = lane & 15;
+  const int slot = wave / WPS, ws = wave % WPS, ts = t - slot * G::NT;
+  const int h = blockIdx.x, chunk = blockIdx.y;
+  const int N = p.N, H = p.H;
+  char *kimg = smem + slot * 2 * G::IMG, *vimg = kimg + G::IMG;
+  const bool has_bias = p.table != nullptr;
+  if (has_bias) build_plane<G::NK>(plane, p, h, t);
+  const long long tok_stride = 3LL * H * HD;
+  const int q = ws * 16 + li;
+  int b0, b1;
+  chunk_range(p, chunk, b0, b1);
+  for (int bb = b0; bb < b1; bb += G::SLOTS) {
+    const int b = bb + slot;
+    const bool act = b < b1;
+    const T *base = p.qkv + (long long)b * N * tok_stride + (long long)h * HD;
+    __syncthreads();
+    u32x4 fq[L::KBD];
+    if (act) {
+      tile_to_lds<T, G::NT>(kimg, base + (long long)H * HD, tok_stride, N, G::NK, ts);
+      tile_to_lds<T, G::NT>(vimg, base + 2LL * H * HD, tok_stride, N, G::NK, ts);
+#pragma unroll
+      for (int kb = 0; kb < L::KBD; ++kb) fq[kb] = gl_frag<T>(base + (long long)q * tok_stride, q < N, kb, lane);
+    }
+    __syncthreads();
+    if (!act) continue;
+
+    f32x4 s[NKT];
+#pragma unroll
+    for (int kt = 0; kt < NKT; ++kt) {
+      const int col = kt * 16 + 4 * g;
+      f32x4 bv = {0.f, 0.f, 0.f, 0.f};
+      if (has_bias && q < N && col < N) bv = dm_load4(plane + q * G::LD + col);
+      s[kt] = score_tile<T>(fq, kimg, bv, N, q, p.scale, lane, kt);
+    }
+    float m = -INFINITY;
+#pragma unroll
+    for (int kt = 0; kt < NKT; ++kt)
+#pragma unroll
+      for (int r = 0; r < 4; ++r) m = fmaxf(m, s[kt][r]);
+    m = row_max(m);
+    const float msafe = (m == -INFINITY) ? 0.f : m;
+    float l = 0.f;
+#pragma unroll
+    for (int kt = 0; kt < NKT; ++kt)
+#pragma unroll
+      for (int r = 0; r < 4; ++r) {
+        const float e = fast_exp<T>(s[kt][r] - msafe);
+        s[kt][r] = e;
+        l += e;
+      }
+    l = row_sum(l);
+    const float inv = (l > 0.f) ? 1.f / l : 0.f;
+    if (g == 0 && q < N) p.lse[((long long)b * H + h) * N + q] = msafe + logf(l);
+#pragma unroll
+    for (int kt = 0; kt < NKT; ++kt) s[kt] *= inv;
+
+    f32x4 o[4];
+#pragma unroll
+    for (int dt = 0; dt < 4; ++dt) o[dt] = (f32x4){0.f, 0.f, 0.f, 0.f};
+    contract_tokens<T, NKT>(o, s, vimg, lane);
+    if (q < N) {
+      T *orow = p.out + ((long long)b * N + q) * H * HD + (long long)h * HD;
+#pragma unroll
+      for (int dt = 0; dt < 4; ++dt) dm_store4(orow + dt * 16 + 4 * g, o[dt]);
+    }
+  }
+}
+
+template <int NKT, int WPS>
+__global__ __launch_bounds__(256) void small_bwd_kernel(const SmallParams p) {
+  using T = bf16_t;
+  using G = SG<NKT, WPS>;
+  using L = AL<T>;
+  constexpr int NB = NKT / L::TPB;
+  extern __shared__ __attribute__((aligned(16))) char smem[];
+  float *plane = reinterpret_cast<float *>(smem + G::SLOTS * 4 * G::IMG);
+  const int t = threadIdx.x, lane = t & 63, wave = t >> 6, g = lane >> 4, li = lane & 15;
+  const int slot = wave / WPS, ws = wave % WPS, ts = t - slot * G::NT;
+  float *dlt = plane + G::NK * G::LD + slot * G::NK;
+  const int h = blockIdx.x, chunk = blockIdx.y;
+  const int N = p.N, H = p.H;
+  char *qimg = smem + slot * 4 * G::IMG, *kimg = qimg + G::IMG, *vimg = kimg + G::IMG, *doimg = vimg + G::IMG;
+  const bool has_bias = p.table != nullptr;
+  const bool want_bins = p.partial != nullptr;
+  if (has_bias) build_plane<G::NK>(plane, p, h, t);
+  const long long tok_stride = 3LL * H * HD, o_stride = (long long)H * HD;
+  const int row = ws * 16 + li;
+  const bool rok = row < N;
+  f32x4 hacc[NKT];
+#pragma unroll
+  for (int kt = 0; kt < NKT; ++kt) hacc[kt] = (f32x4){0.f, 0.f, 0.f, 0.f};
+  int b0, b1;
+  chunk_range(p, chunk, b0, b1);
+  const int n_pos = want_bins ? min(p.csr_off[p.n_bins], N * N) : 0;
+
+  for (int bb = b0; bb < b1; bb += G::SLOTS) {
+    const int b = bb + slot;
+    const bool act = b < b1;
+    const T *base = p.qkv + (long long)b * N * tok_stride + (long long)h * HD;
+    const long long orow = ((long long)b * N + row) * o_stride + (long long)h * HD;
+    const float *lse_b = p.lse + ((long long)b * H + h) * N;
+    __syncthreads();
+    float dl = 0.f, lse = 0.f;
+    if (act) {
+      tile_to_lds<T, G::NT>(qimg, base, tok_stride, N, G::NK, ts);
+      tile_to_lds<T, G::NT>(kimg, base + (long long)H * HD, tok_stride, N, G::NK, ts);
+      tile_to_lds<T, G::NT>(vimg, base + 2LL * H * HD, tok_stride, N, G::NK, ts);
+      tile_to_lds<T, G::NT>(doimg, p.dout + (long long)b * N * o_stride + (long long)h * HD, o_stride, N, G::NK, ts);
+      if (rok) {
+        const T *Og = p.out + orow, *dOg = p.dout + orow;
+#pragma unroll
+        for (int c = 0; c < 4; ++c) {
+          const f32x4 a = dm_load4(Og + 16 * g + 4 * c), d = dm_load4(dOg + 16 * g + 4 * c);
+          dl += (a[0] * d[0] + a[1] * d[1]) + (a[2] * d[2] + a[3] * d[3]);
+        }
+      }
+      dl = row_sum(dl);
+      if (g == 0) dlt[row] = dl;
+      lse = rok ? lse_b[row] : 0.f;
+    }
+    __syncthreads();
+    if (!act) continue;
+
+    {
+      u32x4 fq[L::KBD], fdo[L::KBD];
+#pragma unroll
+      for (int kb = 0; kb < L::KBD; ++kb) {
+        fq[kb] = frag_row<T>(qimg, row, kb, lane);
+        fdo[kb] = frag_row<T>(doimg, row, kb, lane);
+      }
+      u32x4 fds[NB];
+#pragma unroll
+      for (int m = 0; m < NB; ++m) {
+        f32x4 tl[L::TPB];
+#pragma unroll
+        for (int u = 0; u < L::TPB; ++u) {
+          const int kt = m * L::TPB + u, col = kt * 16 + 4 * g;
+          f32x4 bv = {0.f, 0.f, 0.f, 0.f};
+          if (has_bias && rok && col < N) bv = dm_load4(plane + row * G::LD + col);
+          const f32x4 sc = score_tile<T>(fq, kimg, bv, N, row, p.scale, lane, kt);
+          f32x4 a = {0.f, 0.f, 0.f, 0.f};
+#pragma unroll
+          for (int kb = 0; kb < L::KBD; ++kb) mma<T>(a, fdo[kb], frag_row<T>(vimg, kt * 16 + li, kb, lane));
+          f32x4 dsv;
+#pragma unroll
+          for (int r = 0; r < 4; ++r) dsv[r] = fast_exp<T>(sc[r] - lse) * (a[r] - dl);
+          if (want_bins) hacc[kt] += dsv;
+          tl[u] = dsv;
+        }
+        fds[m] = pack_tiles<T>(tl);
+        asm volatile("" : "+v"(fds[m]));
+        __builtin_amdgcn_sched_barrier(0);
+      }
+      f32x4 o[4];
+#pragma unroll
+      for (int dt = 0; dt < 4; ++dt) o[dt] = (f32x4){0.f, 0.f, 0.f, 0.f};
+      contract_frags<T, NB>(o, fds, kimg, lane);
+      if (rok) {
+        T *dq = p.dqkv + ((long long)b * N + row) * tok_stride + (long long)h * HD;
+#pragma unroll
+        for (int dt = 0; dt < 4; ++dt) dm_store4(dq + dt * 16 + 4 * g, o[dt] * p.scale);
+      }
+    }
+
+    {
+      u32x4 fk[L::KBD], fvv[L::KBD];
+#pragma unroll
+      for (int kb = 0; kb < L::KBD; ++kb) {
+        fk[kb] = frag_row<T>(kimg, row, kb, lane);
+        fvv[kb] = frag_row<T>(vimg, row, kb, lane);
+      }
+      u32x4 fpt[NB], fds[NB];
+#pragma unroll
+      for (int m = 0; m < NB; ++m) {
+        f32x4 tp[L::TPB], td[L::TPB];
+#pragma unroll
+        for (int u = 0; u < L::TPB; ++u) {
+          const int qt = m * L::TPB + u, q0 = qt * 16 + 4 * g;
+          f32x4 bv = {0.f, 0.f, 0.f, 0.f};
+          if (has_bias && rok) {
+#pragma unroll
+            for (int r = 0; r < 4; ++r) bv[r] = (q0 + r < N) ? plane[(q0 + r) * G::LD + row] : 0.f;
+          }
+          const f32x4 lcur = load4_guard(lse_b, q0, N, true);
+          const f32x4 dcur = (q0 < N) ? dm_load4(dlt + q0) : (f32x4){0.f, 0.f, 0.f, 0.f};
+          const f32x4 sc = score_tile<T>(fk, qimg, bv, N, row, p.scale, lane, qt);
+          f32x4 a = {0.f, 0.f, 0.f, 0.f};
+#pragma unroll
+          for (int kb = 0; kb < L::KBD; ++kb) mma<T>(a, fvv[kb], frag_row<T>(doimg, qt * 16 + li, kb, lane));
+#pragma unroll
+          for (int r = 0; r < 4; ++r) {
+            const float pv = (q0 + r < N) ? fast_exp<T>(sc[r] - lcur[r]) : 0.f;
+            tp[u][r] = pv;
+            td[u][r] = pv * (a[r] - dcur[r]);
+          }
+        }
+        fpt[m] = pack_tiles<T>(tp);
+        fds[m] = pack_tiles<T>(td);
+        asm volatile("" : "+v"(fpt[m]), "+v"(fds[m]));
+        __builtin_amdgcn_sched_barrier(0);
+      }
+      f32x4 o[4];
+      T *dk = p.dqkv + ((long long)b * N + row) * tok_stride + (long long)H * HD + (long long)h * HD;
+      T *dvp = dk + (long long)H * HD;
+#pragma unroll
+      for (int dt = 0; dt < 4; ++dt) o[dt] = (f32x4){0.f, 0.f, 0.f, 0.f};
+      contract_frags<T, NB>(o, fpt, doimg, lane);
+      if (rok) {
+#pragma unroll
+        for (int dt = 0; dt < 4; ++dt) dm_store4(dvp + dt * 16 + 4 * g, o[dt]);
+      }
+#pragma unroll
+      for (int dt = 0; dt < 4; ++dt) o[dt] = (f32x4){0.f, 0.f, 0.f, 0.f};
+      contract_frags<T, NB>(o, fds, qimg, lane);
+      if (rok) {
+#pragma unroll
+        for (int dt = 0; dt < 4; ++dt) dm_store4(dk + dt * 16 + 4 * g, o[dt] * p.scale);
+      }
+    }
+  }
+
+  if (!want_bins) return;
+  const int NN = N * N;
+  float *ds = reinterpret_cast<float *>(smem);
+  int *pos = reinterpret_cast<int *>(smem) + G::NK * G::NK;
+  __syncthreads();
+  {
+    constexpr int IT = G::NK * G::NK / 256;
+    int pv[IT];
+#pragma unroll
+    for (int it = 0; it < IT; ++it) pv[it] = (t + it * 256 < n_pos) ? p.csr_pos[t + it * 256] : 0;
+#pragma unroll
+    for (int it = 0; it < IT; ++it)
+      if (t + it * 256 < n_pos) pos[t + it * 256] = pv[it];
+  }
+#pragma unroll
+  for (int s = 0; s < G::SLOTS; ++s) {
+    if (slot == s && rok) {
+#pragma unroll
+      for (int kt = 0; kt < NKT; ++kt) {
+        const int col = kt * 16 + 4 * g;
+        if (col < N) {
+          float *d = ds + row * N + col;
+          dm_store4(d, s == 0 ? hacc[kt] : dm_load4(d) + hacc[kt]);
+        }
+      }
+    }
+    __syncthreads();
+  }
+  float *out = p.partial + ((long long)chunk * H + h) * p.n_bins;
+  for (int bin = t; bin < p.n_bins; bin += 256) {
+    const int beg = min(max(p.csr_off[bin], 0), n_pos), end = min(max(p.csr_off[bin + 1], beg), n_pos);
+    float acc = 0.f;
+#pragma unroll 4
+    for (int j = beg; j < end; ++j) {
+      const int at = pos[j];
+      acc += ((unsigned)at < (unsigned)NN) ? ds[at] : 0.f;
+    }
+    out[bin] = acc;
+  }
+}
+
+__global__ __launch_bounds__(256) void small_reduce_kernel(const float *__restrict__ partial, float *__restrict__ dtable, int chunks, int H,
+                                                           int n_bins, int accumulate) {
+  const int i = blockIdx.x * 256 + threadIdx.x;
+  if (i >= n_bins * H) return;
+  const int bin = i / H, h = i - bin * H;
+  const float *src = partial + (long long)h * n_bins + bin;
+  const long long step = (long long)H * n_bins;
+  float acc = 0.f;
+#pragma unroll 8
+  for (int c = 0; c < chunks; ++c) acc += src[c * step];
+  dtable[i] = accumulate ? dtable[i] + acc : acc;
+}
+
+int small_chunks(int B, int H) { return std::min(B, std::max(1, 512 / H)); }
+
+template <int NKT, int WPS> bool launch_small(bool bwd, const SmallParams &p, hipStream_t s) {
+  using G = SG<NKT, WPS>;
+  const void *fn = bwd ? reinterpret_cast<const void *>(&small_bwd_kernel<NKT, WPS>) : reinterpret_cast<const void *>(&small_fwd_kernel<NKT, WPS>);
+  const int lds = bwd ? G::BWD_LDS : G::FWD_LDS;
+  if (lds > 64 * 1024) {
+    static const bool ok = hipFuncSetAttribute(fn, hipFuncAttributeMaxDynamicSharedMemorySize, G::BWD_LDS) == hipSuccess;
+    if (!ok) return false;
+  }
+  const dim3 grid(p.H, p.chunks);
+  if (bwd) hipLaunchKernelGGL((small_bwd_kernel<NKT, WPS>), grid, dim3(256), lds, s, p);
+  else hipLaunchKernelGGL((small_fwd_kernel<NKT, WPS>), grid, dim3(256), lds, s, p);
+  return true;
+}
+bool dispatch_small(bool bwd, const SmallParams &p, hipStream_t s) {
+  if (p.N == 16) return launch_small<2, 1>(bwd, p, s);
+  if (p.N == 32) return launch_small<2, 2>(bwd, p, s);
+  return launch_small<4, 4>(bwd, p, s);
+}
+
+}
+
+extern "C" int32_t dm_attention_small_ok(int32_t B, int32_t N, int32_t H, int32_t D, int32_t dtype, int32_t n_bins) {
+  return B > 0 && B <= (1 << 24) && H > 0 && H <= 65535 && D == HD && dtype == DM_BF16 && N >= 16 && N <= 64 && N % 16 == 0 && n_bins >= 0 &&
+                 n_bins <= (1 << 20) ? 1 : 0;
+}
+
+extern "C" int32_t dm_attention_small_chunks(int32_t B, int32_t N, int32_t H) {
+  (void)N;
+  return B > 0 && H > 0 ? small_chunks(B, H) : 0;
+}
+
+extern "C" int dm_attention_small_fwd(const void *qkv, const float *table, const int32_t *index32, void *out, float *lse, int32_t B, int32_t N,
+                                      int32_t H, int32_t D, int32_t n_bins, float scale, void *stream) {
+  DM_REQUIRE(dm_attention_small_ok(B, N, H, D, DM_BF16, n_bins), DM_ERR_UNSUPPORTED,
+             "dm_attention_small_fwd: shape not taken (B=%d N=%d H=%d D=%d n_bins=%d); use dm_attention_fwd", B, N, H, D, n_bins);
+  DM_REQUIRE(qkv && out && lse && (!table || (index32 && n_bins > 0)), DM_ERR_BAD_SHAPE, "dm_attention_small_fwd: null pointer");
+  DM_REQUIRE(dm_aligned16(qkv) && dm_aligned16(out), DM_ERR_BAD_ALIGN, "dm_attention_small_fwd: qkv/out must be 16-byte aligned");
+  hipStream_t s = reinterpret_cast<hipStream_t>(stream);
+  {
+    DmProfScope prof("attn_fwd_bf16", s, 4.0 * B * H * (double)N * N * HD, 2.0 * 4.0 * B * H * (double)N * HD);
+    SmallParams p{};
+    p.qkv = reinterpret_cast<const bf16_t *>(qkv); p.table = table; p.index = index32; p.out = reinterpret_cast<bf16_t *>(out); p.lse = lse;
+    p.B = B; p.N = N; p.H = H; p.n_bins = n_bins; p.chunks = small_chunks(B, H); p.scale = scale;
+    DM_REQUIRE(dispatch_small(false, p, s), DM_ERR_HIP, "dm_attention_small_fwd: kernel could not be configured");
+  }
+  DM_LAUNCH_CHECK("dm_attention_small_fwd");
+  return DM_OK;
+}
+
+extern "C" int dm_attention_small_bwd(const void *qkv, const float *table, const int32_t *index32, const int32_t *csr_pos, const int32_t *csr_off,
+                                      const void *out, const void *dout, const float *lse, void *dqkv, float *partial, float *dtable,
+                                      int32_t accumulate, int32_t B, int32_t N, int32_t H, int32_t D, int32_t n_bins, float scale, void *stream) {
+  DM_REQUIRE(dm_attention_small_ok(B, N, H, D, DM_BF16, n_bins), DM_ERR_UNSUPPORTED,
+             "dm_attention_small_bwd: shape not taken (B=%d N=%d H=%d D=%d n_bins=%d); use dm_attention_bwd", B, N, H, D, n_bins);
+  DM_REQUIRE(qkv && out && dout && lse && dqkv && (!table || (index32 && n_bins > 0)), DM_ERR_BAD_SHAPE, "dm_attention_small_bwd: null pointer");
+  DM_REQUIRE(!dtable || (table && csr_pos && csr_off && partial), DM_ERR_BAD_SHAPE,
+             "dm_attention_small_bwd: a table gradient needs the table, the CSR inverse of its index and the partial rows");
+  DM_REQUIRE(dm_aligned16(qkv) && dm_aligned16(out) && dm_aligned16(dout) && dm_aligned16(dqkv) && dm_aligned16(lse), DM_ERR_BAD_ALIGN,
+             "dm_attention_small_bwd: tensors must be 16-byte aligned");
+  hipStream_t s = reinterpret_cast<hipStream_t>(stream);
+  {
+    DmProfScope prof("attn_bwd_bf16", s, 10.0 * B * H * (double)N * N * HD, 2.0 * 8.0 * B * H * (double)N * HD);
+    SmallParams p{};
+    p.qkv = reinterpret_cast<const bf16_t *>(qkv); p.table = table; p.index = index32; p.csr_pos = csr_pos; p.csr_off = csr_off;
+    p.out = reinterpret_cast<bf16_t *>(const_cast<void *>(out)); p.dout = reinterpret_cast<const bf16_t *>(dout);
+    p.lse = const_cast<float *>(lse); p.dqkv = reinterpret_cast<bf16_t *>(dqkv); p.partial = dtable ? partial : nullptr;
+    p.B = B; p.N = N; p.H = H; p.n_bins = n_bins; p.chunks = small_chunks(B, H); p.scale = scale;
+    DM_REQUIRE(dispatch_small(true, p, s), DM_ERR_HIP, "dm_attention_small_bwd: kernel could not be configured");
+    if (dtable)
+      hipLaunchKernelGGL(small_reduce_kernel, dim3((n_bins * H + 255) / 256), dim3(256), 0, s, partial, dtable, p.chunks, H, n_bins, accumulate);
+  }
+  DM_LAUNCH_CHECK("dm_attention_small_bwd");
+  return DM_OK;
+}
diff --git a/deepmerge_amd/ops.py b/deepmerge_amd/ops.py
--- a/deepmerge_amd/ops.py
+++ b/deepmerge_amd/ops.py
@@ -484,6 +484,7 @@
 
 _SPLIT_ATTENTION = os.environ.get("DM_ATTN_X3", "1") != "0"
 _INKERNEL_TABLE = os.environ.get("DM_ATTN_TABLE_IN_KERNEL", "1") != "0"
+_SMALL_MAX_TOKENS = {"0": 0, "1": 32}.get(os.environ.get("DM_ATTN_SMALL", "1"), 64)
 
 
 class _AttnRoute:
@@ -497,6 +498,9 @@
             self.kind, self.cube = "split", cube
         elif cube is not None and _INKERNEL_TABLE and relpos_inkernel(B, N, H, D, cube, dtype):
             self.kind, self.cube = "table", cube
+        elif (dtype == torch.bfloat16 and N <= _SMALL_MAX_TOKENS and (table is None or index32 is not None)
+              and attention_small_ok(B, N, H, D, dtype, 0 if table is None else table.shape[0])):
+            self.kind = "small"
 
 
 def _attention_forward(qkv, table, index32, route: _AttnRoute, B, N, H, D, scale, out_pair: bool = False):
@@ -506,11 +510,14 @@
         return r[0], r[1], (r[2], r[3]), (r[4] if out_pair else None)
     if route.kind == "table":
         return attention_fwd_relpos(qkv, table, route.cube, B, N, H, D, scale) + ((None, None), None)
+    if route.kind == "small":
+        return attention_small_fwd(qkv, table, index32, B, N, H, D, scale) + ((None, None), None)
     keep = (None, None) if table is None else relpos_bias_gather(table, index32, N, transposed=True)
     return attention_fwd(qkv, keep[0], B, N, H, D, scale) + (keep, None)
 
 
 def _attention_backward(route: _AttnRoute, qkv, keep, table, out, dout, lse, index32, n_bins, B, N, H, D, scale, pair: bool = False):
+    assert route.kind != "small"
     table = None if (table is None or route.kind == "dense") else table.contiguous()
     if route.kind == "split":
         return attention_bwd_split(keep[0], keep[1], table, route.cube, out, dout, lse, B, N, H, D, scale, index32, n_bins or 0, pair=pair)
@@ -586,6 +593,46 @@
              dhi.data_ptr(), dlo.data_ptr(), lse.data_ptr(), dqkv.data_ptr(), delta.data_ptr(), _ptr(slab),
              B, N, H, D, scale, _stream()), "dm_attention_split_bwd")
     return (Planes(dqkv) if pair else dqkv), slab, info
+
+
+def attention_small_ok(B: int, N: int, H: int, D: int, dtype: torch.dtype, n_bins: int) -> bool:
+    return bool(_lib.lib().dm_attention_small_ok(B, N, H, D, DM_BF16 if dtype == torch.bfloat16 else DM_F32, n_bins))
+
+
+def _small_table_check(who: str, table, index32, N: int, H: int) -> int:
+    if table is None:
+        return 0
+    if (table.dtype != torch.float32 or not table.is_contiguous() or table.dim() != 2 or table.shape[1] != H or index32 is None
+            or index32.dtype != torch.int32 or not index32.is_contiguous() or index32.numel() != N * N):
+        raise ValueError(f"{who}: table must be contiguous fp32 [n_bins, H] and index32 contiguous int32 [N, N]")
+    return table.shape[0]
+
+
+def attention_small_fwd(qkv: torch.Tensor, table: Optional[torch.Tensor], index32: Optional[torch.Tensor], B: int, N: int, H: int, D: int,
+                        scale: float):
+    _need_cuda(qkv, table, index32)
+    n_bins = _small_table_check("attention_small_fwd", table, index32, N, H)
+    out = torch.empty((B, N, H * D), dtype=qkv.dtype, device=qkv.device)
+    lse = torch.empty((B, H, N), dtype=torch.float32, device=qkv.device)
+    check(_lib.lib().dm_attention_small_fwd(qkv.data_ptr(), _ptr(table), _ptr(index32 if n_bins else None), out.data_ptr(), lse.data_ptr(),
+                                            B, N, H, D, n_bins, scale, _stream()), "dm_attention_small_fwd")
+    return out, lse
+
+
+def attention_small_bwd(qkv, table, index32, out, dout, lse, B, N, H, D, scale, dtable=None, accumulate=False):
+    _need_cuda(qkv, table, index32, out, dout, lse, dtable)
+    n_bins = _small_table_check("attention_small_bwd", table, index32, N, H)
+    dqkv = torch.empty_like(qkv)
+    pos = off = partial = None
+    if dtable is not None:
+        if not n_bins or dtable.dtype != torch.float32 or not dtable.is_contiguous() or dtable.numel() != n_bins * H:
+            raise ValueError("attention_small_bwd: dtable must be contiguous fp32 [n_bins, H] next to a table")
+        pos, off = relpos_index_csr(index32, n_bins)
+        partial = torch.empty((_lib.lib().dm_attention_small_chunks(B, N, H), H, n_bins), dtype=torch.float32, device=qkv.device)
+    check(_lib.lib().dm_attention_small_bwd(qkv.data_ptr(), _ptr(table), _ptr(index32 if n_bins else None), _ptr(pos), _ptr(off),
+                                            out.data_ptr(), dout.data_ptr(), lse.data_ptr(), dqkv.data_ptr(), _ptr(partial), _ptr(dtable),
+                                            int(accumulate), B, N, H, D, n_bins, scale, _stream()), "dm_attention_small_bwd")
+    return dqkv
 
 
 def relpos_index_csr(index32: torch.Tensor, n_bins: int):
@@ -1192,6 +1239,11 @@
         qkv, out, lse, k0, k1, index32, table = ctx.saved_tensors
         want_table = n_bins is not None and ctx.needs_input_grad[1]
         dout = dout.contiguous().float() if ctx.route.kind == "split" else _as_operand(dout, qkv.dtype)
+        if ctx.route.kind == "small":
+            dtable = torch.empty((n_bins, H), dtype=torch.float32, device=out.device) if want_table else None
+            dqkv = attention_small_bwd(qkv, None if table is None else table.contiguous(), index32, out, dout, lse, B, N, H, D, scale,
+                                       dtable=dtable)
+            return dqkv, dtable, None, None, None, None, None, None
         dqkv, slab, info = _attention_backward(ctx.route, qkv, (k0, k1), table, out, dout, lse, index32 if want_table else None, n_bins,
                                                B, N, H, D, scale)
         dtable = None
@@ -1639,11 +1691,18 @@
         keep = ctx.split_imgs if ctx.route.kind == "split" else (bias, bias_t)
         ctx.split_imgs = None
         want_table = P["table"] is not None
-        dqkv, slab, info = _attention_backward(ctx.route, qkv, keep, P["table"].detach() if want_table else None, o, do.view(B, N, Cc), lse,
-                                               index32 if want_table else None, n_bins, B, N, heads, D, scale, pair=planes)
-        if want_table:
-            t = slots["table"] = _GradSlot(P["table"], (n_bins, heads), dev)
-            relpos_bias_scatter(slab, t.out, B, heads, info, n_bins, accumulate=t.acc())
+        if ctx.route.kind == "small":
+            t = None
+            if want_table:
+                t = slots["table"] = _GradSlot(P["table"], (n_bins, heads), dev)
+            dqkv = attention_small_bwd(qkv, P["table"].detach().contiguous() if want_table else None, index32, o, do.view(B, N, Cc), lse,
+                                       B, N, heads, D, scale, dtable=t.out if t else None, accumulate=bool(t and t.acc()))
+        else:
+            dqkv, slab, info = _attention_backward(ctx.route, qkv, keep, P["table"].detach() if want_table else None, o, do.view(B, N, Cc), lse,
+                                                   index32 if want_table else None, n_bins, B, N, heads, D, scale, pair=planes)
+            if want_table:
+                t = slots["table"] = _GradSlot(P["table"], (n_bins, heads), dev)
+                relpos_bias_scatter(slab, t.out, B, heads, info, n_bins, accumulate=t.acc())
         dqkv = linear_grads("qkv", dqkv if isinstance(dqkv, Planes) else dqkv.view(M, 3 * Cc), y1, 3 * Cc, Cc, pair=True)
         dy1 = torch.empty((M, Cc), dtype=dtype, device=dev)
         gemm(DM_NN, dqkv, wq, dy1, M, Cc, 3 * Cc, lda=3 * Cc, ldb=Cc, ldc=Cc)
diff --git a/include/deepmerge_hip.h b/include/deepmerge_hip.h
--- a/include/deepmerge_hip.h
+++ b/include/deepmerge_hip.h
@@ -89,6 +89,14 @@
                                 int32_t H, int32_t D, float scale, void *stream);
 int32_t dm_attention_bwd_batch_chunks(int32_t B, int32_t N, int32_t H, int32_t dtype);
 
+int32_t dm_attention_small_ok(int32_t B, int32_t N, int32_t H, int32_t D, int32_t dtype, int32_t n_bins);
+int32_t dm_attention_small_chunks(int32_t B, int32_t N, int32_t H);
+int dm_attention_small_fwd(const void *qkv, const float *table, const int32_t *index32, void *out, float *lse, int32_t B, int32_t N,
+                           int32_t H, int32_t D, int32_t n_bins, float scale, void *stream);
+int dm_attention_small_bwd(const void *qkv, const float *table, const int32_t *index32, const int32_t *csr_pos, const int32_t *csr_off,
+                           const void *out, const void *dout, const float *lse, void *dqkv, float *partial, float *dtable,
+                           int32_t accumulate, int32_t B, int32_t N, int32_t H, int32_t D, int32_t n_bins, float scale, void *stream);
+
 int dm_relpos_bias_gather(const float *table, const int32_t *index, float *bias, float *bias_t,
                           int32_t N, int32_t H, int32_t n_bins, void *stream);
 int dm_relpos_bias_reduce(float *dbias_slab, const int32_t *positions, const int32_t *offsets, float *dtable,
```

Measured after the change: 6576 pairs/s, median of 2. Within noise of the previous version (+0.2%).
